# shz9/viprs

Hardware: AMD Instinct MI355X
Metric: SNP-updates/sec/E-step (1M SNPs, ~1700 LD blocks) (higher is better)
Workload: dtype f32

## Files before the change

### viprs_amd/csrc/abi_estep.hip

```cpp
#include "internal.h"

#include <type_traits>

using namespace viprs;

namespace {

__global__ void sweep_prologue_kernel(int32_t* counters, int n_counters, unsigned long long* skipped,
                                      unsigned long long* granules, int64_t n_granules) {
    const int64_t i = (int64_t)blockIdx.x * blockDim.x + threadIdx.x;
    if (i < n_counters) counters[i] = 0;
    if (i == 0) { skipped[0] = 0ull; skipped[1] = 0ull; }
    for (int64_t k = i; k < n_granules; k += (int64_t)gridDim.x * blockDim.x) granules[k] = 0ull;
}

hipError_t clear_stale_skip_count(viprs_plan* P) {
    if (!P->skip_count_in_place) return hipSuccess;
    P->skip_count_in_place = false;
    return hipMemsetAsync(P->d_skipped.p, 0, sizeof(unsigned long long), P->stream);
}

int sweep_prologue(viprs_plan* P, int n_models) {
    P->skip_count_in_place = true;
    const int64_t ng = P->n_granule_rows * kPanel * std::max(1, n_models);
    if (P->d_granules.n < (size_t)ng) {
        HIP_TRY(hipStreamSynchronize(P->stream));
        HIP_TRY(P->d_granules.alloc((size_t)ng));
    }
    const unsigned grid = (unsigned)std::max<int64_t>(1, std::min<int64_t>((ng + 255) / 256, 1024));
    sweep_prologue_kernel<<<grid, 256, 0, P->stream>>>(P->d_counters.p, kPlanCounters, P->d_skipped.p, P->d_granules.p, ng);
    HIP_TRY(hipGetLastError());
    return VIPRS_OK;
}

template <typename T>
EStepArgs<T> make_args(viprs_state* S, double dq) {
    viprs_plan* P = S->plan;
    EStepArgs<T> A{};
    A.skipped = P->d_skipped.p;
    A.lb = P->d_lb.p;
    A.rowstart = P->d_ip.p;
    A.rowlen = P->d_rowlen.p;
    A.ld_rows = P->d_ld_raw.p;
    A.ld_dense = P->d_ld_dense.p;
    A.ld_zero_off = P->dense_elems;
    A.std_beta = (const T*)S->f[VIPRS_FIELD_STD_BETA].p;
    A.u_logs = (const T*)S->f[VIPRS_FIELD_U_LOGS].p;
    A.shvt = (const T*)S->f[VIPRS_FIELD_SQRT_HALF_VAR_TAU].p;
    A.mu_mult = (const T*)S->f[VIPRS_FIELD_MU_MULT].p;
    A.log_null_pi = (const T*)S->f[VIPRS_FIELD_LOG_NULL_PI].p;
    A.var_gamma = (T*)S->f[VIPRS_FIELD_VAR_GAMMA].p;
    A.var_mu = (T*)S->f[VIPRS_FIELD_VAR_MU].p;
    A.eta = (T*)S->f[VIPRS_FIELD_ETA].p;
    A.q = (T*)S->f[VIPRS_FIELD_Q].p;
    A.eta_diff = (T*)S->f[VIPRS_FIELD_ETA_DIFF].p;
    A.eta_out = (T*)S->eta_out.p;
    A.q_out = (T*)S->q_out.p;
    A.granules = P->d_granules.p;
    A.granule_rows = P->n_granule_rows;
    A.error = P->d_error.p;
    A.dq = (T)dq;
    A.low_memory = P->low_memory;
    A.width = S->width;
    A.m = P->m;
    return A;
}

template <typename U> constexpr int ld_code();
template <> constexpr int ld_code<int8_t>() { return VIPRS_LD_I8; }
template <> constexpr int ld_code<int16_t>() { return VIPRS_LD_I16; }
template <> constexpr int ld_code<int32_t>() { return VIPRS_LD_I32; }
template <> constexpr int ld_code<int64_t>() { return VIPRS_LD_I64; }
template <> constexpr int ld_code<float>() { return VIPRS_LD_F32; }
template <> constexpr int ld_code<double>() { return VIPRS_LD_F64; }

template <typename... Us, typename F>
int for_ld_type(int ld_dtype, const char* otherwise, F&& f) {
    int rc = VIPRS_OK;
    const bool found = ((ld_dtype == ld_code<Us>() && ((rc = f(Us{})), true)) || ...);
    return found ? rc : fail(VIPRS_EINVAL, otherwise);
}

template <typename U>
int launch_grid_chunks(viprs_state* S, const EStepArgs<float>& A) {
    viprs_plan* P = S->plan;
    const int64_t lists_per_chunk = (int64_t)S->n_groups * kGroupListStride;
    for (int off = 0; off < A.n_active; off += kGridModels) {
        EStepArgs<float> Ac = A;
        Ac.active = A.active + off;
        Ac.n_active = std::min(kGridModels, A.n_active - off);
        if (A.group_cols) Ac.group_lists = S->d_group_lists.p + (off / kGridModels) * lists_per_chunk;
        int rc = off > 0 ? sweep_prologue(P, 1) : VIPRS_OK;
        if (rc == VIPRS_OK) rc = launch_grid_mfma<U>(P, Ac);
        if (rc != VIPRS_OK) return rc;
    }
    return VIPRS_OK;
}

template <typename T>
int launch_family(viprs_state* S, const EStepArgs<T>& A, int family, int model, bool dense) {
    viprs_plan* P = S->plan;
    if (family == kFamNone) return VIPRS_OK;
    if (family == kFamGeneric)
        return for_ld_type<int8_t, int16_t, int32_t, int64_t, float, double>(P->ld_dtype, "bad LD dtype", [&](auto u) {
            return launch_generic<T, decltype(u)>(P, A, model, dense); });
    if constexpr (std::is_same<T, double>::value) {
        if (family == kFamTileF64)
            return for_ld_type<int8_t, int16_t, int32_t, int64_t, float, double>(P->ld_dtype, "bad LD dtype", [&](auto u) {
                return launch_tile_f64<decltype(u)>(P, A, model, dense); });
    } else {
        if (family == kFamPanel)
            return for_ld_type<float, int8_t, int16_t>(P->ld_dtype, kDenseLdTypeError, [&](auto u) {
                return model == kPanelElasticNet ? launch_panel_enet<decltype(u)>(P, A) : launch_panel<decltype(u)>(P, A, model); });
        if (family == kFamBand)
            return for_ld_type<float, int8_t, int16_t>(P->ld_dtype, kBandLdTypeError, [&](auto u) {
                return model == kBandElasticNet ? launch_band_enet<decltype(u)>(P, A) : launch_band<decltype(u)>(P, A, model); });
        if (family == kFamGridBatched)
            return for_ld_type<float, int8_t, int16_t>(P->ld_dtype, kDenseLdTypeError, [&](auto u) {
                return launch_grid_chunks<decltype(u)>(S, A); });
    }
    return fail(VIPRS_EINVAL, "kernel family without an instantiation for the state precision");
}

template <typename T>
int launch_route(viprs_state* S, const SweepRoute& r, double dq, const int32_t* d_active, int n_active) {
    viprs_plan* P = S->plan;
    EStepArgs<T> A = make_args<T>(S, dq);
    A.active = d_active;
    A.n_active = n_active;
    if (S->model_kind == VIPRS_MODEL_GRID && !S->group_cols_h.empty()) {
        A.blk_group = S->d_blk_group.p;
        A.group_cols = S->d_group_cols.p;
    }
    int rc = launch_family<T>(S, A, r.dense_family, r.dense_model, true);
    if (rc != VIPRS_OK) return rc;
    rc = P->timing.dense_done();
    if (rc != VIPRS_OK) return rc;
    return launch_family<T>(S, A, r.ragged_family, r.ragged_model, false);
}

bool band_ok(const viprs_plan* P) {
    const char* f = getenv("VIPRS_BAND");
    if (f && !atoi(f)) return false;
    if (P->ld_dtype != VIPRS_LD_F32 && P->ld_dtype != VIPRS_LD_I8 && P->ld_dtype != VIPRS_LD_I16) return false;
    return band_ring_panels(P) <= kBandMaxRingPanels;
}

bool use_grid_mfma(const viprs_plan* P, int width) {
    if ((int64_t)P->m * std::max(1, width) >= (1LL << 31)) return false;
    if (P->grid_mfma >= 0) return P->grid_mfma != 0;
    return (int64_t)P->dense_h.size() * 8 >= (int64_t)P->n_cu * 3;
}

int run_route(viprs_state* S, const SweepRoute& r, double dq, const int32_t* d_active, int n_active) {
    viprs_plan* P = S->plan;
    int rc = VIPRS_OK;
    if (r.prologue) rc = sweep_prologue(P, r.prologue_per_model ? n_active : 1);
    else HIP_TRY(clear_stale_skip_count(P));
    if (rc != VIPRS_OK) return rc;
    P->math_used = 0;
    rc = P->timing.open(r.whole_sweep_events, r.dense_bracketed);
    if (rc != VIPRS_OK) return rc;
    if (r.dense_bracketed && r.start_event_by_launcher) P->timing.arm();
    else if (r.dense_bracketed) { rc = P->timing.start(); if (rc != VIPRS_OK) return rc; }
    rc = S->float_dtype == VIPRS_F32 ? launch_route<float>(S, r, dq, d_active, n_active)
                                     : launch_route<double>(S, r, dq, d_active, n_active);
    if (rc != VIPRS_OK) { P->timing.abandon(); return rc; }
    return P->timing.close();
}

int run_sweep(viprs_state* S, double dq, const int32_t* d_active, int n_active) {
    static_assert(kGenSpikeSlab == VIPRS_MODEL_SPIKE_SLAB && kGenMixture == VIPRS_MODEL_MIXTURE && kGenGrid == VIPRS_MODEL_GRID, "");
    viprs_plan* P = S->plan;
    HIP_TRY(hipSetDevice(P->device));
    const SweepConfig c{S->float_dtype, S->model_kind, S->width, P->ld_dtype, !P->dense_h.empty(), !P->ragged_h.empty(), band_ok(P),
                        use_grid_mfma(P, S->width), getenv("VIPRS_F64_ROW_BY_ROW") != nullptr};
    SweepRoute r;
    std::string err;
    const int rc = sweep_route(c, r, err);
    if (rc != VIPRS_OK) return fail(rc, err);
    return run_route(S, r, dq, d_active, n_active);
}

int group_mask_prepare(viprs_state* S, const int32_t* active, int n_active) {
    viprs_plan* P = S->plan;
    if (S->float_dtype != VIPRS_F32)
        return fail(VIPRS_EUNSUPPORTED, "grid state with a (group, column) mask: float64 states are not supported");
    if (!P->ragged_h.empty())
        return fail(VIPRS_EUNSUPPORTED, "grid state with a (group, column) mask: ragged / banded LD blocks are not supported "
                                        "(the generic and band kernels take no mask)");
    const int n_chunks = (n_active + kGridModels - 1) / kGridModels;
    std::vector<int32_t> lists((size_t)n_chunks * S->n_groups * kGroupListStride, 0);
    for (int k = 0; k < n_chunks; ++k) {
        const int lo = k * kGridModels, hi = std::min(n_active, lo + kGridModels);
        for (int g = 0; g < S->n_groups; ++g) {
            int32_t* l = lists.data() + ((size_t)k * S->n_groups + g) * kGroupListStride;
            int cnt = 0;
            for (int i = lo; i < hi; ++i)
                if (S->group_cols_h[(size_t)g * S->width + active[i]]) l[1 + cnt++] = active[i];
            l[0] = cnt;
            for (int t = cnt; t < kGridModels; ++t) l[1 + t] = cnt > 0 ? l[cnt] : active[lo];
        }
    }
    HIP_TRY(hipStreamSynchronize(P->stream));
    if (S->d_group_lists.n < lists.size()) HIP_TRY(S->d_group_lists.alloc(lists.size()));
    HIP_TRY(hipMemcpy(S->d_group_lists.p, lists.data(), lists.size() * sizeof(int32_t), hipMemcpyHostToDevice));
    if (S->blk_group_gen != P->dense_gen || S->d_blk_group.n < P->dense_h.size()) {
        std::vector<int32_t> map(std::max<size_t>(1, P->dense_h.size()), 0);
        for (size_t k = 0; k < P->dense_h.size(); ++k)
            map[k] = (int32_t)(std::upper_bound(S->group_start.begin(), S->group_start.end(), (int64_t)P->dense_h[k].start) -
                               S->group_start.begin()) - 1;
        HIP_TRY(S->d_blk_group.alloc(map.size()));
        HIP_TRY(hipMemcpy(S->d_blk_group.p, map.data(), map.size() * sizeof(int32_t), hipMemcpyHostToDevice));
        S->blk_group_gen = P->dense_gen;
    }
    return VIPRS_OK;
}

int active_list_check(const viprs_state* S, const int32_t*& active, int& n_active, std::vector<int32_t>& all) {
    if (!active) {
        all.resize((size_t)S->width);
        for (int g = 0; g < S->width; ++g) all[(size_t)g] = g;
        active = all.data();
        n_active = S->width;
    }
    for (int i = 0; i < n_active; ++i)
        if (active[i] < 0 || active[i] >= S->width) return fail(VIPRS_EINVAL, "active_model_idx out of range");
    return VIPRS_OK;
}

int active_list_upload(viprs_state* S, const int32_t* active, int n_active) {
    if (S->d_active.n < (size_t)n_active) HIP_TRY(S->d_active.alloc((size_t)std::max(n_active, S->width)));
    HIP_TRY(hipMemcpyAsync(S->d_active.p, active, sizeof(int32_t) * (size_t)n_active, hipMemcpyHostToDevice, S->plan->stream));
    HIP_TRY(hipStreamSynchronize(S->plan->stream));
    return VIPRS_OK;
}

void route_fields(const SweepRoute& r, int* route) {
    const int out[VIPRS_ROUTE_COUNT] = {r.dense_family, r.dense_model, r.ragged_family, r.ragged_model, r.prologue,
                                        r.prologue_per_model, r.start_event_by_launcher, r.whole_sweep_events, r.dense_bracketed};
    std::copy(out, out + VIPRS_ROUTE_COUNT, route);
}

}

extern "C" {

int viprs_state_e_step(viprs_state* S, double dq_scale, const int32_t* active, int n_active, int sync) {
    if (!S) return fail(VIPRS_EINVAL, "null state");
    int rc;
    switch (S->model_kind) {
        case VIPRS_MODEL_SPIKE_SLAB: case VIPRS_MODEL_MIXTURE: rc = run_sweep(S, dq_scale, nullptr, 0); break;
        case VIPRS_MODEL_GRID: {
            std::vector<int32_t> all;
            rc = active_list_check(S, active, n_active, all);
            if (rc != VIPRS_OK) return rc;
            if (n_active == 0) return VIPRS_OK;
            HIP_TRY(hipSetDevice(S->plan->device));
            if (!S->group_cols_h.empty()) {
                rc = group_mask_prepare(S, active, n_active);
                if (rc != VIPRS_OK) return rc;
            }
            rc = active_list_upload(S, active, n_active);
            if (rc != VIPRS_OK) return rc;
            rc = run_sweep(S, dq_scale, S->d_active.p, n_active);
            break;
        }
        default: return fail(VIPRS_EINVAL, "bad model kind");
    }
    if (rc != VIPRS_OK) return rc;
    if (sync) HIP_TRY(hipStreamSynchronize(S->plan->stream));
    return VIPRS_OK;
}

int viprs_state_enet_sweep(viprs_state* S, double dq_scale, const int32_t* active, int n_active, int sync) {
    if (!S) return fail(VIPRS_EINVAL, "null state");
    if (S->model_kind == VIPRS_MODEL_MIXTURE) return fail(VIPRS_EINVAL, "elastic-net sweep: not defined for a mixture state");
    if (S->model_kind != VIPRS_MODEL_SPIKE_SLAB && S->model_kind != VIPRS_MODEL_GRID) return fail(VIPRS_EINVAL, "bad model kind");
    if (S->float_dtype != VIPRS_F32)
        return fail(VIPRS_EUNSUPPORTED, "elastic-net sweep: float64 states are not supported (the kernels are float32)");
    const bool grid = S->model_kind == VIPRS_MODEL_GRID;
    if (grid && !S->group_cols_h.empty())
        return fail(VIPRS_EUNSUPPORTED, "elastic-net sweep: a grid state under a (group, column) mask is not supported");
    viprs_plan* P = S->plan;
    std::vector<int32_t> all;
    if (grid) {
        const int rc = active_list_check(S, active, n_active, all);
        if (rc != VIPRS_OK) return rc;
    } else {
        active = nullptr;
        n_active = 0;
    }
    SweepRoute r;
    std::string err;
    int rc = enet_route(grid, P->ld_dtype, !P->dense_h.empty(), !P->ragged_h.empty(), band_ok(P), r, err);
    if (rc != VIPRS_OK) return fail(rc, err);
    if (grid && n_active == 0) return VIPRS_OK;
    HIP_TRY(hipSetDevice(P->device));
    if (grid) {
        rc = active_list_upload(S, active, n_active);
        if (rc != VIPRS_OK) return rc;
    }
    rc = run_route(S, r, dq_scale, grid ? S->d_active.p : nullptr, n_active);
    if (rc != VIPRS_OK) return rc;
    if (sync) HIP_TRY(hipStreamSynchronize(P->stream));
    return VIPRS_OK;
}

int viprs_enet_route(int grid, int ld_dtype, int dense, int ragged, int band_ok, int* route) {
    if (!route) return fail(VIPRS_EINVAL, "null argument");
    SweepRoute r;
    std::string err;
    const int rc = enet_route(grid != 0, ld_dtype, dense != 0, ragged != 0, band_ok != 0, r, err);
    if (rc != VIPRS_OK) return fail(rc, err);
    route_fields(r, route);
    return VIPRS_OK;
}

static int one_shot(viprs_plan* P, int float_dtype, int model_kind, int width, const void* const (&host)[VIPRS_FIELD_COUNT],
                    double dq, const int32_t* active, int n_active) {
    viprs_state* S = P->scratch;
    if (!S || S->float_dtype != float_dtype || S->model_kind != model_kind || S->width != width) {
        delete P->scratch;
        P->scratch = nullptr;
        int rc = viprs_state_create(&P->scratch, P, float_dtype, model_kind, width);
        if (rc != VIPRS_OK) return rc;
        S = P->scratch;
    }
    const size_t fs = float_size(S->float_dtype);
    HIP_TRY(hipSetDevice(P->device));
    for (int f : {VIPRS_FIELD_STD_BETA, VIPRS_FIELD_LOG_NULL_PI, VIPRS_FIELD_U_LOGS, VIPRS_FIELD_SQRT_HALF_VAR_TAU, VIPRS_FIELD_MU_MULT,
                  VIPRS_FIELD_VAR_GAMMA, VIPRS_FIELD_VAR_MU, VIPRS_FIELD_ETA, VIPRS_FIELD_Q, VIPRS_FIELD_ETA_DIFF}) {
        const size_t bytes = S->field_elems(f) * fs;
        if (bytes == 0) continue;
        if (!host[f]) return fail(VIPRS_EINVAL, "null buffer");
        HIP_TRY(hipMemcpyAsync(S->f[f].p, host[f], bytes, hipMemcpyHostToDevice, P->stream));
    }
    int rc = viprs_state_e_step(S, dq, active, n_active, 0);
    if (rc != VIPRS_OK) return rc;
    for (int f : {VIPRS_FIELD_VAR_GAMMA, VIPRS_FIELD_VAR_MU, VIPRS_FIELD_ETA, VIPRS_FIELD_Q, VIPRS_FIELD_ETA_DIFF})
        HIP_TRY(hipMemcpyAsync(const_cast<void*>(host[f]), S->f[f].p, S->field_elems(f) * fs, hipMemcpyDeviceToHost, P->stream));
    HIP_TRY(hipStreamSynchronize(P->stream));
    return check_device_error(P);
}

int viprs_e_step(viprs_plan* P, int float_dtype, const void* std_beta, void* var_gamma, void* var_mu, void* eta,
                 void* q, void* eta_diff, const void* u_logs, const void* shvt, const void* mu_mult,
                 double dq_scale, int threads, int low_memory) {
    (void)threads;
    if (!P) return fail(VIPRS_EINVAL, "null plan");
    if ((low_memory != 0) != (P->low_memory != 0))
        return fail(VIPRS_EINVAL, "low_memory differs from the value the plan was created with");
    if (P->m == 0) return VIPRS_OK;
    const void* const host[] = {std_beta, u_logs, shvt, mu_mult, nullptr, var_gamma, var_mu, eta, q, eta_diff};
    return one_shot(P, float_dtype, VIPRS_MODEL_SPIKE_SLAB, 1, host, dq_scale, nullptr, 0);
}

int viprs_e_step_mixture(viprs_plan* P, int float_dtype, int K, const void* std_beta, void* var_gamma, void* var_mu,
                         void* eta, void* q, void* eta_diff, const void* log_null_pi, const void* u_logs,
                         const void* shvt, const void* mu_mult, double dq_scale, int threads, int low_memory) {
// ... 86 lines not shown
```

### viprs_amd/csrc/abi_plan.hip

```cpp
#include "internal.h"
#include <chrono>

using namespace viprs;

namespace {
thread_local std::string g_err;
viprs::BuildFlagsRegistrar tu_build_flags_(VIPRS_TU_BUILD_FLAGS);
}

namespace viprs {
int fail(int code, const std::string& msg) {
    g_err = msg;
    return code;
}
SchedConfig& sched_config() {
    static SchedConfig c;
    return c;
}
static std::string& build_flags_registry() {
    static std::string s;
    return s;
}
void register_build_flags(const char* flags) {
    std::string& all = build_flags_registry();
    const std::string f(flags ? flags : "");
    size_t i = 0;
    while (i < f.size()) {
        while (i < f.size() && f[i] == ' ') ++i;
        size_t j = i;
        while (j < f.size() && f[j] != ' ') ++j;
        if (j > i) {
            const std::string name = f.substr(i, j - i);
            if ((" " + all + " ").find(" " + name + " ") == std::string::npos) all += (all.empty() ? "" : " ") + name;
        }
        i = j;
    }
}
}

namespace {

template <typename U>
__global__ void repack_dense_kernel(const U* __restrict__ src, const int64_t* __restrict__ ip, U* __restrict__ dst,
                                    const BlockDesc* __restrict__ blocks, int upper) {
    const BlockDesc bd = blocks[blockIdx.y];
    const int b = bd.size;
    for (int r = blockIdx.x; r < b; r += gridDim.x) {
        const int64_t rs = ip[bd.start + r];
        U* __restrict__ drow = dst + bd.ld_off + (int64_t)r * bd.stride;
        if (upper) {
            for (int c = r + 1 + threadIdx.x; c < b; c += blockDim.x) drow[c] = src[rs + (c - r - 1)];
        } else {
            for (int c = threadIdx.x; c < b; c += blockDim.x) drow[c] = src[rs + c];
        }
    }
}

template <typename U>
__global__ __launch_bounds__(256) void mirror_lower_kernel(U* __restrict__ dense, const BlockDesc* __restrict__ blocks, int fill) {
    __shared__ U t[kPanel][kPanel + 1];
    const BlockDesc bd = blocks[blockIdx.y];
    const int b = bd.size, np = (b + kPanel - 1) / kPanel;
    U* __restrict__ base = dense + bd.ld_off;
    const int tx = threadIdx.x & 63, ty = threadIdx.x >> 6;
    const int n_pairs = np * (np + 1) / 2;
    for (int item = blockIdx.x; item < n_pairs; item += gridDim.x) {
        int I = 0, rem = item;
        while (rem >= np - I) { rem -= np - I; ++I; }
        const int J = I + rem;
        if (fill) {
            for (int r = ty; r < kPanel; r += 4) {
                const int row = I * kPanel + r, col = J * kPanel + tx;
                t[r][tx] = (row < b && col < b && col > row) ? base[(int64_t)row * bd.stride + col] : (U)0;
            }
        }
        __syncthreads();
        for (int r = ty; r < kPanel; r += 4) {
            const int row = J * kPanel + r, col = I * kPanel + tx;
            if (row < b && col < row) base[(int64_t)row * bd.stride + col] = fill ? t[tx][r] : (U)0;
        }
        __syncthreads();
    }
}

template <typename U>
__global__ void expand_symmetric_kernel(const U* __restrict__ up, const int64_t* __restrict__ ipu,
                                        const int32_t* __restrict__ lb, const int64_t* __restrict__ ip,
                                        U* __restrict__ out, int64_t m, U diag) {
    for (int64_t j = blockIdx.x; j < m; j += gridDim.x) {
        const int64_t o = ip[j];
        const int len = (int)(ip[j + 1] - o);
        const int64_t c0 = lb[j];
        const int64_t uj = ipu[j];
        for (int p = threadIdx.x; p < len; p += blockDim.x) {
            const int64_t c = c0 + p;
            U v = diag;
            if (c > j) v = up[uj + (c - j - 1)];
            else if (c < j) v = up[ipu[c] + (j - c - 1)];
            out[o + p] = v;
        }
    }
}

template <typename U>
static hipError_t launch_expand(const void* up, const int64_t* ipu, const int32_t* lb, const int64_t* ip, void* out,
                                int64_t m, double diag) {
    const unsigned grid = (unsigned)std::min<int64_t>(m, 1 << 16);
    expand_symmetric_kernel<U><<<grid, 256>>>((const U*)up, ipu, lb, ip, (U*)out, m, (U)diag);
    return hipGetLastError();
}

}

namespace viprs { void team_launch_forget(const viprs_plan* P); }
viprs_plan::~viprs_plan() {
    viprs::team_launch_forget(this);
    delete scratch;
    if (ev_fork) (void)hipEventDestroy(ev_fork);
    if (ev_join) (void)hipEventDestroy(ev_join);
    if (side_stream) (void)hipStreamDestroy(side_stream);
    if (stream) (void)hipStreamDestroy(stream);
}

struct ExpandSource {
    std::vector<int64_t> ip_upper;
    const void* data = nullptr;
    double diag = 1.0;
};

static int widen_indptr(int64_t m, const void* indptr, int indptr_dtype, std::vector<int64_t>& ip64) {
    ip64.assign((size_t)m + 1, 0);
    if (indptr_dtype == VIPRS_IP_I64) {
        if (m > 0) std::memcpy(ip64.data(), indptr, sizeof(int64_t) * ((size_t)m + 1));
    } else if (indptr_dtype == VIPRS_IP_I32) {
        const int32_t* p = static_cast<const int32_t*>(indptr);
        for (int64_t i = 0; i <= m && m > 0; ++i) ip64[(size_t)i] = p[i];
    } else {
        return fail(VIPRS_EINVAL, "bad indptr dtype code");
    }
    return VIPRS_OK;
}

static int plan_create_impl(viprs_plan** out, int64_t m, const int32_t* lb, const std::vector<int64_t>& ip64,
                            const void* ld_data, int ld_dtype, int low_memory, int device, const ExpandSource* ex,
                            const std::function<int(void*)>* fill = nullptr) {
    const size_t es = ld_elem_size(ld_dtype);
    std::unique_ptr<viprs_plan> P(new viprs_plan());
    P->m = m;
    if (const char* f = getenv("VIPRS_GRID_MFMA")) P->grid_mfma = atoi(f);
    {
        SchedConfig c;
        auto env = [](const char* name) -> const char* { const char* f = getenv(name); return (f && *f) ? f : nullptr; };
        if (const char* f = env("VIPRS_LARGE_BLOCK")) c.large_block = atoi(f);
        if (const char* f = env("VIPRS_MEDIUM_BLOCK")) c.medium_block = atoi(f);
        if (const char* f = env("VIPRS_TEAM0")) { c.class_team[0] = std::max(1, atoi(f)); c.team_env = true; }
        if (const char* f = env("VIPRS_TEAM1")) { c.class_team[1] = std::max(1, atoi(f)); c.team_env = true; }
        if (const char* f = getenv("VIPRS_BOTTOM_MOD")) c.bottom_mod = std::max(0, atoi(f));
        sched_config() = c;
    }
    P->low_memory = low_memory != 0;
    P->ld_dtype = ld_dtype;
    P->device = device;
    std::string err;
    int rc = plan_blocks(m, lb, ip64.data(), low_memory != 0, P->blocks, err);
    if (rc != VIPRS_OK) return fail(rc, err);
    P->nnz = m > 0 ? ip64[(size_t)m] : 0;
    if (P->nnz > 0 && !ld_data && !ex && !fill) return fail(VIPRS_EINVAL, "ld_data is null");

    HIP_TRY(hipSetDevice(device));
    (void)hipGetLastError();
    hipDeviceProp_t prop;
    HIP_TRY(hipGetDeviceProperties(&prop, device));
    P->n_cu = prop.multiProcessorCount;
    HIP_TRY(hipStreamCreateWithFlags(&P->stream, hipStreamNonBlocking));
    rc = P->timing.create(P->stream);
    if (rc != VIPRS_OK) return rc;

    bool panel_ld = (ld_dtype == VIPRS_LD_F32 || ld_dtype == VIPRS_LD_I8 || ld_dtype == VIPRS_LD_I16);
    if (const char* f = getenv("VIPRS_NO_DENSE")) panel_ld = panel_ld && !atoi(f);
    int64_t dense_off = 0;
    for (const Block& b : P->blocks) {
        BlockDesc d;
        d.start = (int32_t)b.start;
        d.size = (int32_t)(b.end - b.start);
        d.kind = b.kind;
        d.stride = 0;
        d.ld_off = 0;
        d.gr_off = 0;
        d.band_left = d.band_right = 0;
        constexpr int kMaxDenseBlock = 13184;
        static_assert(kMaxDenseBlock % kPanel == 0, "whole panels");
        static_assert(PanelLds(kMaxDenseBlock + 2 * kStrip, true, false).total_floats() <= 160 * 1024 / 4, "the symmetric form fits one workgroup");
        const bool dense = panel_ld && (b.kind == VIPRS_BLOCK_DENSE_SYM || b.kind == VIPRS_BLOCK_DENSE_UPPER) &&
                           d.size <= kMaxDenseBlock;
        if (dense) {
            d.stride = (d.size + kPanel - 1) / kPanel * kPanel;
            d.ld_off = dense_off;
            dense_off += (int64_t)d.size * d.stride;
            dense_off = (dense_off + 63) / 64 * 64;
            P->dense_h.push_back(d);
            P->max_dense = std::max(P->max_dense, d.size);
        } else {
            int64_t wl = 0, wr = 0;
            for (int64_t j = b.start; j < b.end; ++j) {
                const int64_t len = ip64[(size_t)j + 1] - ip64[(size_t)j];
                if (len <= 0) continue;
                wl = std::max<int64_t>(wl, j - lb[j]);
                wr = std::max<int64_t>(wr, lb[j] + len - 1 - j);
            }
            d.band_left = (int32_t)(wl / kPanel + 1);
            d.band_right = (int32_t)(wr / kPanel + 1);
            P->max_band_panels = std::max(P->max_band_panels, d.band_left + d.band_right + 2);
            P->ragged_h.push_back(d);
            P->max_ragged = std::max(P->max_ragged, d.size);
        }
    }
    P->dense_elems = dense_off;
    auto by_cost = [](const BlockDesc& a, const BlockDesc& b) {
        return a.size != b.size ? a.size > b.size : a.start < b.start;
    };
    std::sort(P->dense_h.begin(), P->dense_h.end(), by_cost);
    std::sort(P->ragged_h.begin(), P->ragged_h.end(), by_cost);
    {
        int i = 0, n = (int)P->dense_h.size();
        P->class_begin[0] = 0;
        while (i < n && P->dense_h[i].size >= sched_config().large_block) ++i;
        P->class_begin[1] = i;
        while (i < n && P->dense_h[i].size >= sched_config().medium_block) ++i;
        P->class_begin[2] = i;
        P->class_begin[3] = n;
        if (!sched_config().team_env && P->class_begin[1] > 0) {
            P->team0 = std::min(16, std::max(8, 4 * (int)(((int64_t)P->dense_h[0].size * (int64_t)es + 5999) / 6000)));
            const int64_t room = (int64_t)P->n_cu * 2 * 5 / 8;
            while (P->team0 > 4 && (int64_t)P->class_begin[1] * P->team0 > room) P->team0 -= 4;
        }
        int64_t rows = 0;
        for (int k = 0; k < P->class_begin[2]; ++k) {
            P->dense_h[(size_t)k].gr_off = rows;
            rows += (P->dense_h[(size_t)k].size + kPanel - 1) / kPanel;
        }
        P->n_granule_rows = rows;
    }

    HIP_TRY(P->d_counters.alloc(kPlanCounters));
    HIP_TRY(hipMemset(P->d_counters.p, 0, kPlanCounters * sizeof(int32_t)));
    HIP_TRY(hipDeviceSynchronize());
    HIP_TRY(P->d_error.alloc(1));
    HIP_TRY(hipMemset(P->d_error.p, 0, sizeof(int32_t)));
    HIP_TRY(P->d_skipped.alloc(2));
    HIP_TRY(hipMemset(P->d_skipped.p, 0, 2 * sizeof(unsigned long long)));
    if (m > 0) {
        HIP_TRY(P->d_lb.alloc((size_t)m));
        HIP_TRY(P->d_ip.alloc((size_t)m + 1));
        HIP_TRY(hipMemcpy(P->d_lb.p, lb, sizeof(int32_t) * (size_t)m, hipMemcpyHostToDevice));
        HIP_TRY(hipMemcpy(P->d_ip.p, ip64.data(), sizeof(int64_t) * ((size_t)m + 1), hipMemcpyHostToDevice));
        std::vector<int32_t> rowlen((size_t)m);
        for (int64_t j = 0; j < m; ++j) rowlen[(size_t)j] = (int32_t)(ip64[(size_t)j + 1] - ip64[(size_t)j]);
        HIP_TRY(P->d_rowlen.alloc((size_t)m));
        HIP_TRY(hipMemcpy(P->d_rowlen.p, rowlen.data(), sizeof(int32_t) * (size_t)m, hipMemcpyHostToDevice));
        if (!P->dense_h.empty()) {
            std::vector<int64_t> rs((size_t)m, 0);
            for (const BlockDesc& d : P->dense_h)
                for (int r = 0; r < d.size; ++r)
                    rs[(size_t)d.start + r] = d.ld_off + (int64_t)r * d.stride + (P->low_memory ? r + 1 : 0);
            HIP_TRY(P->d_rowstart_dense.alloc((size_t)m));
            HIP_TRY(hipMemcpy(P->d_rowstart_dense.p, rs.data(), sizeof(int64_t) * (size_t)m, hipMemcpyHostToDevice));
        }
    }
    if (P->nnz > 0) {
        HIP_TRY(P->d_ld_raw.alloc((size_t)P->nnz * es + 64));
        if (fill) {
            rc = (*fill)(P->d_ld_raw.p);
            if (rc != VIPRS_OK) return rc;
        } else if (!ex) {
            HIP_TRY(hipMemcpy(P->d_ld_raw.p, ld_data, (size_t)P->nnz * es, hipMemcpyHostToDevice));
        } else {
            const size_t nnz_u = (size_t)ex->ip_upper[(size_t)m];
            DevBuf<char> d_up;
            DevBuf<int64_t> d_ipu;
            HIP_TRY(d_up.alloc(std::max<size_t>(nnz_u, 1) * es));
            HIP_TRY(d_ipu.alloc((size_t)m + 1));
            if (nnz_u) HIP_TRY(hipMemcpy(d_up.p, ex->data, nnz_u * es, hipMemcpyHostToDevice));
            HIP_TRY(hipMemcpy(d_ipu.p, ex->ip_upper.data(), sizeof(int64_t) * ((size_t)m + 1), hipMemcpyHostToDevice));
            hipError_t e = hipSuccess;
            switch (ld_dtype) {
                case VIPRS_LD_I8:  e = launch_expand<int8_t>(d_up.p, d_ipu.p, P->d_lb.p, P->d_ip.p, P->d_ld_raw.p, m, ex->diag); break;
                case VIPRS_LD_I16: e = launch_expand<int16_t>(d_up.p, d_ipu.p, P->d_lb.p, P->d_ip.p, P->d_ld_raw.p, m, ex->diag); break;
                case VIPRS_LD_I32: e = launch_expand<int32_t>(d_up.p, d_ipu.p, P->d_lb.p, P->d_ip.p, P->d_ld_raw.p, m, ex->diag); break;
                case VIPRS_LD_I64: e = launch_expand<int64_t>(d_up.p, d_ipu.p, P->d_lb.p, P->d_ip.p, P->d_ld_raw.p, m, ex->diag); break;
                case VIPRS_LD_F32: e = launch_expand<float>(d_up.p, d_ipu.p, P->d_lb.p, P->d_ip.p, P->d_ld_raw.p, m, ex->diag); break;
                default:           e = launch_expand<double>(d_up.p, d_ipu.p, P->d_lb.p, P->d_ip.p, P->d_ld_raw.p, m, ex->diag); break;
            }
            HIP_TRY(e);
            HIP_TRY(hipDeviceSynchronize());
        }
    }
    if (P->n_granule_rows > 0) {
        HIP_TRY(P->d_granules.alloc((size_t)P->n_granule_rows * kPanel));
        HIP_TRY(hipMemset(P->d_granules.p, 0, sizeof(unsigned long long) * P->d_granules.n));
        HIP_TRY(hipDeviceSynchronize());
    }
    if (!P->dense_h.empty()) {
        HIP_TRY(P->d_dense.alloc(P->dense_h.size()));
        HIP_TRY(hipMemcpy(P->d_dense.p, P->dense_h.data(), sizeof(BlockDesc) * P->dense_h.size(), hipMemcpyHostToDevice));
        int max_stride = 0;
        for (const BlockDesc& d : P->dense_h) max_stride = std::max(max_stride, d.stride);
        const size_t bytes = ((size_t)P->dense_elems + 4 * kStrip + (size_t)kPanel * max_stride) * es;
        HIP_TRY(P->d_ld_dense.alloc(bytes));
        HIP_TRY(hipMemset(P->d_ld_dense.p, 0, bytes));
        dim3 grid(64, (unsigned)P->dense_h.size());
        const int upper = P->low_memory;
        switch (ld_dtype) {
            case VIPRS_LD_F32:
                repack_dense_kernel<float><<<grid, 256>>>((const float*)P->d_ld_raw.p, P->d_ip.p, (float*)P->d_ld_dense.p, P->d_dense.p, upper);
                break;
            case VIPRS_LD_I8:
                repack_dense_kernel<int8_t><<<grid, 256>>>((const int8_t*)P->d_ld_raw.p, P->d_ip.p, (int8_t*)P->d_ld_dense.p, P->d_dense.p, upper);
                break;
            case VIPRS_LD_I16:
                repack_dense_kernel<int16_t><<<grid, 256>>>((const int16_t*)P->d_ld_raw.p, P->d_ip.p, (int16_t*)P->d_ld_dense.p, P->d_dense.p, upper);
                break;
            default: break;
        }
        HIP_TRY(hipGetLastError());
        HIP_TRY(hipDeviceSynchronize());
    }
    if (!P->ragged_h.empty()) {
        HIP_TRY(P->d_ragged.alloc(P->ragged_h.size()));
        HIP_TRY(hipMemcpy(P->d_ragged.p, P->ragged_h.data(), sizeof(BlockDesc) * P->ragged_h.size(), hipMemcpyHostToDevice));
    } else {
        HIP_TRY(P->d_ld_raw.alloc(0));
    }
    P->dense_all_h = P->dense_h;
    P->ragged_all_h = P->ragged_h;
    std::copy(P->class_begin, P->class_begin + 4, P->class_begin_all);
    if (!P->dense_h.empty()) {
        HIP_TRY(P->d_dense_all.alloc(P->dense_h.size()));
        HIP_TRY(hipMemcpy(P->d_dense_all.p, P->dense_h.data(), sizeof(BlockDesc) * P->dense_h.size(), hipMemcpyHostToDevice));
    }
    HIP_TRY(hipDeviceSynchronize());
    *out = P.release();
    return VIPRS_OK;
}

namespace viprs {
int ensure_upper_storage(viprs_plan* P, bool mirrored) {
    P->unmirrored_wanted = !mirrored;
    if (!P->low_memory || P->dense_all_h.empty() || (P->mirror != 0) == mirrored) return VIPRS_OK;
    int max_np = 0;
    for (const BlockDesc& d : P->dense_all_h) max_np = std::max(max_np, (d.size + kPanel - 1) / kPanel);
    const dim3 grid((unsigned)std::min(max_np * (max_np + 1) / 2, 512), (unsigned)P->dense_all_h.size());
    switch (P->ld_dtype) {
        case VIPRS_LD_F32: mirror_lower_kernel<float><<<grid, 256, 0, P->stream>>>((float*)P->d_ld_dense.p, P->d_dense_all.p, mirrored ? 1 : 0); break;
        case VIPRS_LD_I8: mirror_lower_kernel<int8_t><<<grid, 256, 0, P->stream>>>((int8_t*)P->d_ld_dense.p, P->d_dense_all.p, mirrored ? 1 : 0); break;
        case VIPRS_LD_I16: mirror_lower_kernel<int16_t><<<grid, 256, 0, P->stream>>>((int16_t*)P->d_ld_dense.p, P->d_dense_all.p, mirrored ? 1 : 0); break;
        default: return fail(VIPRS_EINVAL, "dense blocks with unsupported LD dtype");
    }
    HIP_TRY(hipGetLastError());
    P->mirror = mirrored ? 1 : 0;
    return VIPRS_OK;
}

namespace {
std::mutex g_gate_mutex;
std::map<int, hipEvent_t> g_gate_event;
std::map<int, const viprs_plan*> g_gate_plan;
}
double host_clock_ms() {
    return std::chrono::duration<double, std::milli>(std::chrono::steady_clock::now().time_since_epoch()).count();
}
int team_launch_gate(viprs_plan* P) {
    std::lock_guard<std::mutex> lock(g_gate_mutex);
    auto it = g_gate_event.find(P->device);
    auto last = g_gate_plan.find(P->device);
    if (it != g_gate_event.end() && (last == g_gate_plan.end() || last->second != P))
        HIP_TRY(hipStreamWaitEvent(P->stream, it->second, 0));
    return VIPRS_OK;
}
void team_launch_forget(const viprs_plan* P) {
    std::lock_guard<std::mutex> lock(g_gate_mutex);
    auto last = g_gate_plan.find(P->device);
    if (last != g_gate_plan.end() && last->second == P) g_gate_plan.erase(last);
}
int team_launch_done(viprs_plan* P) {
    std::lock_guard<std::mutex> lock(g_gate_mutex);
    auto it = g_gate_event.find(P->device);
    if (it == g_gate_event.end()) {
        hipEvent_t e = nullptr;
        HIP_TRY(hipEventCreateWithFlags(&e, hipEventDisableTiming));
        it = g_gate_event.emplace(P->device, e).first;
    }
    HIP_TRY(hipEventRecord(it->second, P->stream));
    g_gate_plan[P->device] = P;
    return VIPRS_OK;
}
int plan_create_generated(viprs_plan** out, int64_t m, const int32_t* lb, const std::vector<int64_t>& ip64, int ld_dtype,
                          int low_memory, int device, const std::function<int(void*)>& fill) {
    return plan_create_impl(out, m, lb, ip64, nullptr, ld_dtype, low_memory, device, nullptr, &fill);
}
}

extern "C" {

const char* viprs_last_error(void) { return g_err.c_str(); }
const char* viprs_version(void) { return "viprs_amd 0.1.0 (gfx950)"; }
const char* viprs_build_flags(void) { return build_flags_registry().c_str(); }

int viprs_device_count(int* count) {
    if (!count) return fail(VIPRS_EINVAL, "count is null");
    int n = 0;
    hipError_t e = hipGetDeviceCount(&n);
    if (e != hipSuccess) { *count = 0; return fail(VIPRS_EDEVICE, hipGetErrorString(e)); }
    *count = n;
    return VIPRS_OK;
}

int viprs_host_fingerprint(const void* data, int64_t n_bytes, uint64_t* out) {
    if (!out || n_bytes < 0 || (n_bytes > 0 && !data)) return fail(VIPRS_EINVAL, "bad argument");
    const unsigned char* b = static_cast<const unsigned char*>(data);
    uint64_t h = 0x9e3779b97f4a7c15ull ^ (uint64_t)n_bytes;
    auto mix = [&](const unsigned char* p, int64_t n) {
        int64_t i = 0;
        for (; i + 8 <= n; i += 8) {
            uint64_t w;
            std::memcpy(&w, p + i, 8);
            h = (h ^ w) * 0xff51afd7ed558ccdull;
            h ^= h >> 32;
        }
        for (; i < n; ++i) { h = (h ^ p[i]) * 0x100000001b3ull; }
    };
    constexpr int64_t kEdge = 4096, kSamples = 256, kWin = 64;
    if (n_bytes <= 2 * kEdge + kSamples * kWin) {
        mix(b, n_bytes);
    } else {
        mix(b, kEdge);
        mix(b + n_bytes - kEdge, kEdge);
        const int64_t step = (n_bytes - kWin) / kSamples;
        for (int64_t k = 0; k < kSamples; ++k) mix(b + k * step, kWin);
    }
    *out = h;
    return VIPRS_OK;
}

int viprs_check_blas_support(void) { return 0; }
int viprs_check_omp_support(void) { return 0; }

int viprs_plan_blocks(int64_t m, const int32_t* lb, const void* indptr, int indptr_dtype, int low_memory,
                      int64_t* n_blocks, int64_t* block_start, int32_t* block_kind) {
    if (!n_blocks || !block_start) return fail(VIPRS_EINVAL, "null output");
    if (m > 0 && (!lb || !indptr)) return fail(VIPRS_EINVAL, "null LD index array");
    std::vector<int64_t> ip64;
    const int64_t* ip = nullptr;
    if (indptr_dtype == VIPRS_IP_I64) {
        ip = static_cast<const int64_t*>(indptr);
    } else if (indptr_dtype == VIPRS_IP_I32) {
        const int32_t* p = static_cast<const int32_t*>(indptr);
        ip64.assign(p, p + m + 1);
        ip = ip64.data();
    } else {
        return fail(VIPRS_EINVAL, "bad indptr dtype code");
    }
    std::vector<Block> blocks;
    std::string err;
    int rc = plan_blocks(m, lb, ip, low_memory != 0, blocks, err);
    if (rc != VIPRS_OK) return fail(rc, err);
    *n_blocks = (int64_t)blocks.size();
    for (size_t i = 0; i < blocks.size(); ++i) {
        block_start[i] = blocks[i].start;
        if (block_kind) block_kind[i] = blocks[i].kind;
    }
    block_start[blocks.size()] = m;
    return VIPRS_OK;
}

int viprs_plan_create(viprs_plan** out, int64_t m, const int32_t* lb, const void* indptr, int indptr_dtype,
                      const void* ld_data, int ld_dtype, int low_memory, int device) {
    if (!out) return fail(VIPRS_EINVAL, "plan output is null");
    *out = nullptr;
    if (ld_elem_size(ld_dtype) == 0) return fail(VIPRS_EINVAL, "bad LD dtype code");
    if (m < 0 || m > INT32_MAX) return fail(VIPRS_EINVAL, "m out of range");
    if (m > 0 && (!lb || !indptr)) return fail(VIPRS_EINVAL, "null LD index array");
    std::vector<int64_t> ip64;
    int rc = widen_indptr(m, indptr, indptr_dtype, ip64);
    if (rc != VIPRS_OK) return rc;
    return plan_create_impl(out, m, lb, ip64, ld_data, ld_dtype, low_memory, device, nullptr);
}

int viprs_plan_create_expanded(viprs_plan** out, int64_t m, const void* upper_indptr, int indptr_dtype,
                               const void* upper_data, int ld_dtype, double diag_value, int device) {
    if (!out) return fail(VIPRS_EINVAL, "plan output is null");
    *out = nullptr;
    if (ld_elem_size(ld_dtype) == 0) return fail(VIPRS_EINVAL, "bad LD dtype code");
    if (m < 0 || m > INT32_MAX) return fail(VIPRS_EINVAL, "m out of range");
    if (m > 0 && !upper_indptr) return fail(VIPRS_EINVAL, "null LD index array");
    ExpandSource ex;
    int rc = widen_indptr(m, upper_indptr, indptr_dtype, ex.ip_upper);
    if (rc != VIPRS_OK) return rc;
    ex.data = upper_data;
    ex.diag = diag_value;
    if (m > 0 && ex.ip_upper[(size_t)m] > 0 && !upper_data) return fail(VIPRS_EINVAL, "ld_data is null");
    std::vector<int32_t> lb((size_t)m, 0);
    std::vector<int64_t> ip((size_t)m + 1, 0);
    int64_t first = 0, prev_reach = -1;
    for (int64_t j = 0; j < m; ++j) {
        const int64_t len = ex.ip_upper[(size_t)j + 1] - ex.ip_upper[(size_t)j];
        if (len < 0) return fail(VIPRS_EINVAL, "ld_indptr is not non-decreasing");
        const int64_t reach = j + len;
        if (reach >= m) return fail(VIPRS_EINVAL, "an upper-triangular LD row runs past the last SNP");
        if (reach < prev_reach) return fail(VIPRS_EINVAL, "the upper-triangular windows do not mirror into contiguous symmetric windows");
        prev_reach = reach;
        while (first < j && first + (ex.ip_upper[(size_t)first + 1] - ex.ip_upper[(size_t)first]) < j) ++first;
        lb[(size_t)j] = (int32_t)first;
        ip[(size_t)j + 1] = ip[(size_t)j] + (j - first) + 1 + len;
    }
    return plan_create_impl(out, m, lb.data(), ip, nullptr, ld_dtype, 0, device, &ex);
}

int viprs_plan_get_windows(const viprs_plan* P, int32_t* left_bound, int64_t* indptr) {
    if (!P || !left_bound || !indptr) return fail(VIPRS_EINVAL, "null argument");
    HIP_TRY(hipSetDevice(P->device));
    indptr[0] = 0;
    if (P->m > 0) {
        HIP_TRY(hipMemcpy(left_bound, P->d_lb.p, sizeof(int32_t) * (size_t)P->m, hipMemcpyDeviceToHost));
        HIP_TRY(hipMemcpy(indptr, P->d_ip.p, sizeof(int64_t) * ((size_t)P->m + 1), hipMemcpyDeviceToHost));
    }
    return VIPRS_OK;
}
int viprs_plan_destroy(viprs_plan* plan) {
    if (!plan) return VIPRS_OK;
    (void)hipSetDevice(plan->device);
    delete plan;
    return VIPRS_OK;
}

int viprs_plan_info(const viprs_plan* P, int key, int64_t* value) {
// ... 82 lines not shown
```

### viprs_amd/csrc/abi_state.hip

```cpp
#include "internal.h"

using namespace viprs;

namespace {

template <typename T>
__global__ void reset_state_kernel(T* var_gamma, T* var_mu, int64_t n_wide, T* eta, T* q, T* eta_diff, int64_t n_vec,
                                   T pi) {
    const int64_t i = (int64_t)blockIdx.x * blockDim.x + threadIdx.x;
    if (i < n_wide) { var_gamma[i] = pi; var_mu[i] = (T)0; }
    if (i < n_vec) { eta[i] = (T)0; q[i] = (T)0; eta_diff[i] = (T)0; }
}


struct PrepRow {
    int64_t i0, i1, off;
    double logit_pi, log_tau_beta, sigma_eps, tau_beta, one_plus_lambda;
};

template <typename T, bool GRID>
__global__ void prep_kernel(const double* __restrict__ n, PrepRow one, const PrepRow* __restrict__ rows,
                            T* __restrict__ mu_mult, T* __restrict__ u_logs, T* __restrict__ shvt,
                            double* __restrict__ var_tau) {
    PrepRow r;
    if (rows) r = rows[blockIdx.y];
    else r = one;
    for (int64_t i = r.i0 + (int64_t)blockIdx.x * blockDim.x + threadIdx.x; i < r.i1; i += (int64_t)gridDim.x * blockDim.x) {
        const double vt = n[i] * r.one_plus_lambda / r.sigma_eps + r.tau_beta;
        mu_mult[r.off + i] = (T)(n[i] / (vt * r.sigma_eps));
        u_logs[r.off + i] = (T)(r.logit_pi + 0.5 * (r.log_tau_beta - log(vt)));
        if (GRID) {
            shvt[r.off + i] = (T)(0.5 * vt);
        } else {
            shvt[r.off + i] = (T)sqrt(0.5 * vt);
            var_tau[i] = vt;
        }
    }
}

constexpr int kMixResidentK = 8;
constexpr int kMixSums(int K) { return 7 + 6 * K; }
struct MixPrepRow {
    int64_t i0, i1;
    double log_null_pi, sigma_eps, one_plus_lambda;
    double logit_pi[kMixResidentK], log_tau[kMixResidentK], tau[kMixResidentK];
};

template <typename T>
__device__ __forceinline__ void prep_mixture_body(const double* __restrict__ n, int K, const MixPrepRow& r, T* __restrict__ mu_mult,
                                                  T* __restrict__ u_logs, T* __restrict__ shvt, T* __restrict__ lnp,
                                                  double* __restrict__ var_tau) {
    for (int64_t i = r.i0 + (int64_t)blockIdx.x * blockDim.x + threadIdx.x; i < r.i1; i += (int64_t)gridDim.x * blockDim.x) {
        lnp[i] = (T)r.log_null_pi;
        for (int k = 0; k < K; ++k) {
            const double vt = n[i] * r.one_plus_lambda / r.sigma_eps + r.tau[k];
            var_tau[i * K + k] = vt;
            mu_mult[i * K + k] = (T)(n[i] / (vt * r.sigma_eps));
            u_logs[i * K + k] = (T)(r.logit_pi[k] + 0.5 * (r.log_tau[k] - log(vt)));
            shvt[i * K + k] = (T)sqrt(0.5 * vt);
        }
    }
}
template <typename T>
__global__ void prep_mixture_kernel(const double* __restrict__ n, int K, MixPrepRow one, const MixPrepRow* __restrict__ rows,
                                    T* __restrict__ mu_mult, T* __restrict__ u_logs, T* __restrict__ shvt,
                                    T* __restrict__ lnp, double* __restrict__ var_tau) {
    if (rows) prep_mixture_body(n, K, rows[blockIdx.y], mu_mult, u_logs, shvt, lnp, var_tau);
    else prep_mixture_body(n, K, one, mu_mult, u_logs, shvt, lnp, var_tau);
}

constexpr int kSumsBlock = 256;
constexpr int kNSums = VIPRS_N_SUMS;
__host__ __device__ inline int sums_blocks(int64_t count) {
    const int64_t nb = (count + kSumsBlock - 1) / kSumsBlock;
    return (int)(nb < 1024 ? nb : 1024);
}
__host__ __device__ inline int grid_sums_blocks(int64_t count) {
    const int64_t nb = (count + kSumsBlock - 1) / kSumsBlock;
    return (int)(nb < 256 ? nb : 256);
}

struct SumsRow {
    int64_t i0, i1, off;
    int nb;
    int weighted;
    int form_vt;
    double vt[3];
    double one_plus_lambda;
};

template <typename T>
__device__ __forceinline__ void sums_body(int64_t i0, int64_t i1, int nb, int bx, const T* __restrict__ gam,
                                          const T* __restrict__ mu, const T* __restrict__ eta, const T* __restrict__ q,
                                          const T* __restrict__ ed, const T* __restrict__ beta,
                                          const double* __restrict__ var_tau, double one_plus_lambda,
                                          const double* __restrict__ weight, double* __restrict__ out,
                                          const double* __restrict__ n_snp = nullptr, double p_lam1 = 0.0, double p_sig = 1.0,
                                          double p_tau = 0.0) {
    __shared__ double red[kNSums][kSumsBlock];
    double acc[kNSums];
#pragma unroll
    for (int k = 0; k < kNSums; ++k) acc[k] = 0.0;
    const double lo = 1e-15, hi = 1.0 - 1e-15;
    for (int64_t i = i0 + (int64_t)bx * kSumsBlock + threadIdx.x; i < i1; i += (int64_t)nb * kSumsBlock) {
        const double g = (double)gam[i], mud = (double)mu[i];
        const double vt = n_snp ? n_snp[i] * p_lam1 / p_sig + p_tau : var_tau[i];
        const double zeta = g * (mud * mud + 1.0 / vt);
        acc[0] += weight ? g * weight[i] : g;
        acc[1] += zeta;
        acc[2] += one_plus_lambda * zeta + (double)(q[i] * eta[i]);
        acc[3] += (double)beta[i] * (double)eta[i];
        acc[4] += (double)eta[i] * (double)eta[i];
        const double gc = fmin(fmax(g, lo), hi), ng = fmin(fmax(1.0 - g, lo), hi);
        acc[5] += gc * log(gc);
        acc[6] += ng * log(ng);
        acc[7] += gc;
        acc[8] += ng;
        acc[9] += gc * log(vt);
        acc[10] = fmax(acc[10], fabs((double)ed[i]));
    }
#pragma unroll
    for (int k = 0; k < kNSums; ++k) red[k][threadIdx.x] = acc[k];
    __syncthreads();
    for (int s = kSumsBlock / 2; s > 0; s >>= 1) {
        if ((int)threadIdx.x < s) {
#pragma unroll
            for (int k = 0; k < kNSums - 1; ++k) red[k][threadIdx.x] += red[k][threadIdx.x + s];
            red[kNSums - 1][threadIdx.x] = fmax(red[kNSums - 1][threadIdx.x], red[kNSums - 1][threadIdx.x + s]);
        }
        __syncthreads();
    }
    if (threadIdx.x < kNSums) out[threadIdx.x] = red[threadIdx.x][0];
}

template <typename T>
__global__ __launch_bounds__(kSumsBlock) void sums_kernel(SumsRow one, const SumsRow* __restrict__ rows,
                                                          const T* __restrict__ gam, const T* __restrict__ mu,
                                                          const T* __restrict__ eta, const T* __restrict__ q,
                                                          const T* __restrict__ ed, const T* __restrict__ beta,
                                                          const double* __restrict__ var_tau, const double* __restrict__ n_snp,
                                                          const double* __restrict__ weight, double* __restrict__ partials) {
    SumsRow r;
    if (rows) r = rows[blockIdx.y];
    else r = one;
    if ((int)blockIdx.x >= r.nb) return;
    sums_body<T>(r.i0, r.i1, r.nb, (int)blockIdx.x, gam + r.off, mu + r.off, eta + r.off, q + r.off, ed + r.off, beta,
                 r.form_vt ? nullptr : var_tau, r.one_plus_lambda, r.weighted ? weight : nullptr,
                 partials + ((int64_t)blockIdx.y * gridDim.x + blockIdx.x) * kNSums, r.form_vt ? n_snp : nullptr, r.vt[0],
                 r.vt[1], r.vt[2]);
}

template <typename T>
__device__ __forceinline__ void sums_mixture_body(int64_t i0, int64_t i1, int nb, int bx, int K, const T* __restrict__ gam,
                                                  const T* __restrict__ mu, const T* __restrict__ eta,
                                                  const T* __restrict__ q, const T* __restrict__ ed,
                                                  const T* __restrict__ beta, const double* __restrict__ var_tau,
                                                  const double* __restrict__ log_var_tau0, double one_plus_lambda,
                                                  double* __restrict__ partials) {
    constexpr int NMAX = kMixSums(kMixResidentK);
    const int N = kMixSums(K);
    double acc[NMAX];
#pragma unroll
    for (int k = 0; k < NMAX; ++k) acc[k] = 0.0;
    const double lo = 1e-15, hi = 1.0 - 1e-15;
    for (int64_t i = i0 + (int64_t)bx * kSumsBlock + threadIdx.x; i < i1; i += (int64_t)nb * kSumsBlock) {
        double zeta = 0.0, gsum = 0.0;
#pragma unroll
        for (int k = 0; k < kMixResidentK; ++k) {
            if (k < K) {
                const double g = (double)gam[i * K + k], mud = (double)mu[i * K + k], vt = var_tau[i * K + k];
                const double z = g * (mud * mud + 1.0 / vt);
                zeta += z;
                gsum += g;
                const double gc = fmin(fmax(g, lo), hi);
                acc[6 + 0 * kMixResidentK + k] += g;
                acc[6 + 1 * kMixResidentK + k] += z;
                acc[6 + 2 * kMixResidentK + k] += gc * log(gc);
                acc[6 + 3 * kMixResidentK + k] += gc;
                acc[6 + 4 * kMixResidentK + k] += gc * log_var_tau0[i * K + k];
                acc[6 + 5 * kMixResidentK + k] += gc * (mud * mud + 1.0 / vt);
            }
        }
        acc[0] += zeta;
        acc[1] += one_plus_lambda * zeta + (double)(q[i] * eta[i]);
        acc[2] += (double)beta[i] * (double)eta[i];
        acc[3] += (double)eta[i] * (double)eta[i];
        const double ng = fmin(fmax(1.0 - gsum, lo), hi);
        acc[4] += ng * log(ng);
        acc[5] += ng;
        acc[NMAX - 1] = fmax(acc[NMAX - 1], fabs((double)ed[i]));
    }
    __shared__ double red[NMAX][kSumsBlock / 64];
    const int lane = threadIdx.x & 63, wave = threadIdx.x >> 6;
#pragma unroll
    for (int k = 0; k < NMAX; ++k) {
        double a = acc[k];
        for (int off = 32; off > 0; off >>= 1) {
            const double o = __shfl_xor(a, off, 64);
            a = (k == NMAX - 1) ? fmax(a, o) : a + o;
        }
        if (lane == 0) red[k][wave] = a;
    }
    __syncthreads();
    if ((int)threadIdx.x < N) {
        const int nidx = threadIdx.x;
        int src;
        if (nidx < 6) src = nidx;
        else if (nidx == N - 1) src = NMAX - 1;
        else src = 6 + ((nidx - 6) / K) * kMixResidentK + (nidx - 6) % K;
        double a = red[src][0];
        for (int w = 1; w < kSumsBlock / 64; ++w) a = (src == NMAX - 1) ? fmax(a, red[src][w]) : a + red[src][w];
        partials[nidx] = a;
    }
}

template <typename T>
__global__ __launch_bounds__(kSumsBlock) void sums_mixture_kernel(int K, SumsRow one, const SumsRow* __restrict__ rows,
                                                                  const T* __restrict__ gam, const T* __restrict__ mu,
                                                                  const T* __restrict__ eta, const T* __restrict__ q,
                                                                  const T* __restrict__ ed, const T* __restrict__ beta,
                                                                  const double* __restrict__ var_tau,
                                                                  const double* __restrict__ log_var_tau0,
                                                                  double* __restrict__ partials) {
    SumsRow r;
    if (rows) r = rows[blockIdx.y];
    else r = one;
    if ((int)blockIdx.x >= r.nb) return;
    sums_mixture_body<T>(r.i0, r.i1, r.nb, (int)blockIdx.x, K, gam, mu, eta, q, ed, beta, var_tau, log_var_tau0,
                         r.one_plus_lambda, partials + ((int64_t)blockIdx.y * gridDim.x + blockIdx.x) * kMixSums(K));
}

constexpr int kNEnetSums = VIPRS_N_ENET_SUMS;
__global__ __launch_bounds__(kSumsBlock) void enet_sums_kernel(SumsRow one, const SumsRow* __restrict__ rows,
                                                               const float* __restrict__ eta, const float* __restrict__ q,
                                                               const float* __restrict__ ed, const float* __restrict__ beta,
                                                               const float* __restrict__ pen, double* __restrict__ partials) {
    SumsRow r;
    if (rows) r = rows[blockIdx.y];
    else r = one;
    if ((int)blockIdx.x >= r.nb) return;
    __shared__ double red[kNEnetSums][kSumsBlock];
    double acc[kNEnetSums];
#pragma unroll
    for (int k = 0; k < kNEnetSums; ++k) acc[k] = 0.0;
    for (int64_t i = r.i0 + (int64_t)blockIdx.x * kSumsBlock + threadIdx.x; i < r.i1; i += (int64_t)r.nb * kSumsBlock) {
        const double e = (double)eta[r.off + i];
        acc[0] += (double)beta[i] * e;
        acc[1] += (double)q[r.off + i] * e;
        acc[2] += e * e;
        acc[3] += (double)pen[r.off + i] * fabs(e);
        acc[4] += e != 0.0 ? 1.0 : 0.0;
        acc[5] = fmax(acc[5], fabs((double)ed[r.off + i]));
    }
#pragma unroll
    for (int k = 0; k < kNEnetSums; ++k) red[k][threadIdx.x] = acc[k];
    __syncthreads();
    for (int s = kSumsBlock / 2; s > 0; s >>= 1) {
        if ((int)threadIdx.x < s) {
#pragma unroll
            for (int k = 0; k < kNEnetSums - 1; ++k) red[k][threadIdx.x] += red[k][threadIdx.x + s];
            red[kNEnetSums - 1][threadIdx.x] = fmax(red[kNEnetSums - 1][threadIdx.x], red[kNEnetSums - 1][threadIdx.x + s]);
        }
        __syncthreads();
    }
    if (threadIdx.x < kNEnetSums)
        partials[((int64_t)blockIdx.y * gridDim.x + blockIdx.x) * kNEnetSums + threadIdx.x] = red[threadIdx.x][0];
}

__global__ void sums_final_kernel(const double* __restrict__ partials, int stride, int n_sums, SumsRow one,
                                  const SumsRow* __restrict__ rows, double* __restrict__ out) {
    int nb;
    if (rows) nb = rows[blockIdx.y].nb;
    else nb = one.nb;
    partials += (int64_t)blockIdx.y * stride * n_sums;
    const int k = blockIdx.x, lane = threadIdx.x;
    const bool is_max = (k == n_sums - 1);
    double a = 0.0;
    for (int b = lane; b < nb; b += 64) {
        const double v = partials[(int64_t)b * n_sums + k];
        a = is_max ? fmax(a, v) : a + v;
    }
    for (int off = 32; off > 0; off >>= 1) {
        const double o = __shfl_xor(a, off, 64);
        a = is_max ? fmax(a, o) : a + o;
    }
    if (lane == 0) out[(int64_t)blockIdx.y * n_sums + k] = a;
}

}

extern "C" {

int viprs_state_create(viprs_state** out, viprs_plan* plan, int float_dtype, int model_kind, int width) {
    if (!out || !plan) return fail(VIPRS_EINVAL, "null argument");
    *out = nullptr;
    if (float_size(float_dtype) == 0) return fail(VIPRS_EINVAL, "bad float dtype code");
    if (model_kind < VIPRS_MODEL_SPIKE_SLAB || model_kind > VIPRS_MODEL_GRID) return fail(VIPRS_EINVAL, "bad model kind");
    if (model_kind == VIPRS_MODEL_SPIKE_SLAB) width = 1;
    if (width < 1) return fail(VIPRS_EINVAL, "width must be >= 1");
    HIP_TRY(hipSetDevice(plan->device));
    (void)hipGetLastError();
    std::unique_ptr<viprs_state> S(new viprs_state());
    S->plan = plan;
    S->device = plan->device;
    S->float_dtype = float_dtype;
    S->model_kind = model_kind;
    S->width = width;
    if (plan->n_granule_rows > 0) {
        HIP_TRY(S->eta_out.alloc(S->field_elems(VIPRS_FIELD_ETA) * float_size(float_dtype)));
        HIP_TRY(S->q_out.alloc(S->field_elems(VIPRS_FIELD_ETA) * float_size(float_dtype)));
    }
    for (int k = 0; k < VIPRS_FIELD_COUNT; ++k) {
        const size_t bytes = S->field_elems(k) * float_size(float_dtype);
        HIP_TRY(S->f[k].alloc(bytes));
        if (bytes) HIP_TRY(hipMemsetAsync(S->f[k].p, 0, bytes, plan->stream));
    }
    HIP_TRY(hipStreamSynchronize(plan->stream));
    *out = S.release();
    return VIPRS_OK;
}

int viprs_state_destroy(viprs_state* S) {
    if (!S) return VIPRS_OK;
    (void)hipSetDevice(S->device);
    delete S;
    return VIPRS_OK;
}

int viprs_state_upload(viprs_state* S, int field, const void* host) {
    if (!S || field < 0 || field >= VIPRS_FIELD_COUNT) return fail(VIPRS_EINVAL, "bad state/field");
    const size_t bytes = S->field_elems(field) * float_size(S->float_dtype);
    if (bytes == 0) return VIPRS_OK;
    if (!host) return fail(VIPRS_EINVAL, "host buffer is null");
    HIP_TRY(hipSetDevice(S->plan->device));
    HIP_TRY(hipMemcpyAsync(S->f[field].p, host, bytes, hipMemcpyHostToDevice, S->plan->stream));
    HIP_TRY(hipStreamSynchronize(S->plan->stream));
    return VIPRS_OK;
}

int viprs_state_download(viprs_state* S, int field, void* host) {
    if (!S || field < 0 || field >= VIPRS_FIELD_COUNT) return fail(VIPRS_EINVAL, "bad state/field");
    const size_t bytes = S->field_elems(field) * float_size(S->float_dtype);
    if (bytes == 0) return VIPRS_OK;
    if (!host) return fail(VIPRS_EINVAL, "host buffer is null");
    HIP_TRY(hipSetDevice(S->plan->device));
    HIP_TRY(hipMemcpyAsync(host, S->f[field].p, bytes, hipMemcpyDeviceToHost, S->plan->stream));
    HIP_TRY(hipStreamSynchronize(S->plan->stream));
    return check_device_error(S->plan);
}

int viprs_state_reset(viprs_state* S, double pi) {
    if (!S) return fail(VIPRS_EINVAL, "null state");
    viprs_plan* P = S->plan;
    HIP_TRY(hipSetDevice(P->device));
    const int64_t n_wide = (int64_t)S->field_elems(VIPRS_FIELD_VAR_GAMMA);
    const int64_t n_vec = (int64_t)S->field_elems(VIPRS_FIELD_ETA);
    const int64_t n = std::max(n_wide, n_vec);
    if (n == 0) return VIPRS_OK;
    const unsigned grid = (unsigned)((n + 255) / 256);
    if (S->float_dtype == VIPRS_F32)
        reset_state_kernel<float><<<grid, 256, 0, P->stream>>>(
            (float*)S->f[VIPRS_FIELD_VAR_GAMMA].p, (float*)S->f[VIPRS_FIELD_VAR_MU].p, n_wide,
            (float*)S->f[VIPRS_FIELD_ETA].p, (float*)S->f[VIPRS_FIELD_Q].p, (float*)S->f[VIPRS_FIELD_ETA_DIFF].p, n_vec,
            (float)pi);
    else
        reset_state_kernel<double><<<grid, 256, 0, P->stream>>>(
            (double*)S->f[VIPRS_FIELD_VAR_GAMMA].p, (double*)S->f[VIPRS_FIELD_VAR_MU].p, n_wide,
            (double*)S->f[VIPRS_FIELD_ETA].p, (double*)S->f[VIPRS_FIELD_Q].p, (double*)S->f[VIPRS_FIELD_ETA_DIFF].p, n_vec,
            pi);
    HIP_TRY(hipGetLastError());
    return VIPRS_OK;
}

}

namespace viprs {
int check_device_error(viprs_plan* P) {
    int32_t e = 0;
    HIP_TRY(hipMemcpy(&e, P->d_error.p, sizeof(e), hipMemcpyDeviceToHost));
    if (e != 0) {
        HIP_TRY(hipMemsetAsync(P->d_error.p, 0, sizeof(e), P->stream));
        HIP_TRY(hipStreamSynchronize(P->stream));
        return fail(VIPRS_EDEVICE, "E-step kernel: a team hand-off timed out (results of this sweep are invalid)");
    }
    return VIPRS_OK;
}
}

static size_t prep_row_bytes(const viprs_state* S) {
    return S->model_kind == VIPRS_MODEL_MIXTURE ? sizeof(MixPrepRow) : sizeof(PrepRow);
}
static SumsRow* sums_staging(const viprs_state* S) {
    return reinterpret_cast<SumsRow*>(S->h_rows + S->rows_cap * prep_row_bytes(S));
}

static int row_buffers(viprs_state* S, int n) {
    if ((size_t)n <= S->rows_cap) return VIPRS_OK;
    viprs_plan* P = S->plan;
    const size_t cap = std::max<size_t>((size_t)n, (size_t)std::max(1, S->n_groups) *
                                                       (S->model_kind == VIPRS_MODEL_GRID ? S->width : 1));
    HIP_TRY(hipStreamSynchronize(P->stream));
    HIP_TRY(S->d_prep_rows.alloc(cap * prep_row_bytes(S)));
    HIP_TRY(S->d_sum_rows.alloc(cap * sizeof(SumsRow)));
    if (S->h_rows) HIP_TRY(hipHostFree(S->h_rows));
    S->h_rows = nullptr;
    S->rows_cap = 0;
    HIP_TRY(hipHostMalloc(reinterpret_cast<void**>(&S->h_rows), cap * (prep_row_bytes(S) + sizeof(SumsRow)),
                          hipHostMallocDefault));
    S->rows_cap = cap;
    return VIPRS_OK;
}

template <typename Row>
static int prep_staging(viprs_state* S, int n, Row** h) {
    const int rc = row_buffers(S, n);
    if (rc != VIPRS_OK) return rc;
    if (!S->ev_prep) HIP_TRY(hipEventCreateWithFlags(&S->ev_prep, hipEventDisableTiming));
    else HIP_TRY(hipEventSynchronize(S->ev_prep));
    *h = reinterpret_cast<Row*>(S->h_rows);
    return VIPRS_OK;
}

template <typename Row>
static dim3 prep_grid(int n, const Row* rows) {
    int64_t longest = 0;
    for (int i = 0; i < n; ++i) longest = std::max(longest, rows[i].i1 - rows[i].i0);
    return dim3((unsigned)std::max<int64_t>(1, (longest + 255) / 256), (unsigned)n);
}

static int prep_launch(viprs_state* S, int n, const PrepRow* one) {
    viprs_plan* P = S->plan;
    const PrepRow* h = one ? one : reinterpret_cast<const PrepRow*>(S->h_rows);
    const PrepRow* rows = one ? nullptr : reinterpret_cast<const PrepRow*>(S->d_prep_rows.p);
    if (!one) HIP_TRY(hipMemcpyAsync(S->d_prep_rows.p, h, n * sizeof(PrepRow), hipMemcpyHostToDevice, P->stream));
    const dim3 grid = prep_grid(n, h);
    const bool g = S->model_kind == VIPRS_MODEL_GRID;
#define VIPRS_PREP_ARGS(T)                                                                                                    \
    S->d_n.p, *h, rows, (T*)S->f[VIPRS_FIELD_MU_MULT].p, (T*)S->f[VIPRS_FIELD_U_LOGS].p,                                     \
        (T*)S->f[VIPRS_FIELD_SQRT_HALF_VAR_TAU].p, S->d_var_tau.p
    if (S->float_dtype == VIPRS_F32 && g) prep_kernel<float, true><<<grid, 256, 0, P->stream>>>(VIPRS_PREP_ARGS(float));
    else if (S->float_dtype == VIPRS_F32) prep_kernel<float, false><<<grid, 256, 0, P->stream>>>(VIPRS_PREP_ARGS(float));
    else if (g) prep_kernel<double, true><<<grid, 256, 0, P->stream>>>(VIPRS_PREP_ARGS(double));
    else prep_kernel<double, false><<<grid, 256, 0, P->stream>>>(VIPRS_PREP_ARGS(double));
#undef VIPRS_PREP_ARGS
    HIP_TRY(hipGetLastError());
    if (!one) HIP_TRY(hipEventRecord(S->ev_prep, P->stream));
    return VIPRS_OK;
}

static int prep_mixture_launch(viprs_state* S, int n, const MixPrepRow* one) {
    viprs_plan* P = S->plan;
    const int K = S->width;
    if (S->d_var_tau.n < (size_t)P->m * K) {
        HIP_TRY(hipStreamSynchronize(P->stream));
        HIP_TRY(S->d_var_tau.alloc((size_t)P->m * K));
    }
    const MixPrepRow* h = one ? one : reinterpret_cast<const MixPrepRow*>(S->h_rows);
    const MixPrepRow* rows = one ? nullptr : reinterpret_cast<const MixPrepRow*>(S->d_prep_rows.p);
    if (!one) HIP_TRY(hipMemcpyAsync(S->d_prep_rows.p, h, n * sizeof(MixPrepRow), hipMemcpyHostToDevice, P->stream));
    const dim3 grid = prep_grid(n, h);
    if (S->float_dtype == VIPRS_F32)
        prep_mixture_kernel<float><<<grid, 256, 0, P->stream>>>(
            S->d_n.p, K, *h, rows, (float*)S->f[VIPRS_FIELD_MU_MULT].p, (float*)S->f[VIPRS_FIELD_U_LOGS].p,
            (float*)S->f[VIPRS_FIELD_SQRT_HALF_VAR_TAU].p, (float*)S->f[VIPRS_FIELD_LOG_NULL_PI].p, S->d_var_tau.p);
    else
        prep_mixture_kernel<double><<<grid, 256, 0, P->stream>>>(
            S->d_n.p, K, *h, rows, (double*)S->f[VIPRS_FIELD_MU_MULT].p, (double*)S->f[VIPRS_FIELD_U_LOGS].p,
            (double*)S->f[VIPRS_FIELD_SQRT_HALF_VAR_TAU].p, (double*)S->f[VIPRS_FIELD_LOG_NULL_PI].p, S->d_var_tau.p);
    HIP_TRY(hipGetLastError());
    if (!one) HIP_TRY(hipEventRecord(S->ev_prep, P->stream));
    return VIPRS_OK;
}

static SumsRow sums_row(const viprs_state* S, int64_t i0, int64_t i1, int64_t col, double one_plus_lambda, bool weighted,
                        const double* vt) {
    SumsRow r{};
    r.i0 = i0;
    r.i1 = i1;
    r.off = col * S->plan->m;
    r.nb = vt ? grid_sums_blocks(i1 - i0) : sums_blocks(i1 - i0);
    r.weighted = weighted;
    r.one_plus_lambda = one_plus_lambda;
    if (vt) {
        r.form_vt = 1;
        for (int k = 0; k < 3; ++k) r.vt[k] = vt[k];
    }
    return r;
}

static int sums_buffers(viprs_state* S, size_t partials, size_t total) {
    if (S->d_partials.n < partials) HIP_TRY(S->d_partials.alloc(partials));
    if (S->d_sums.n < total) HIP_TRY(S->d_sums.alloc(total));
    if (S->h_sums_cap < total + 1) {
        if (S->h_sums) HIP_TRY(hipHostFree(S->h_sums));
        S->h_sums = nullptr;
        S->h_sums_cap = 0;
        HIP_TRY(hipHostMalloc(reinterpret_cast<void**>(&S->h_sums), (total + 1) * sizeof(double), hipHostMallocDefault));
        S->h_sums_cap = total + 1;
    }
    return VIPRS_OK;
}

enum { kSumsSpikeSlabOrGrid = 0, kSumsMixture = 1, kSumsElasticNet = 2 };

static int sums_enqueue(viprs_state* S, int family, int n, int n_sums, const SumsRow* one) {
    const bool mixture = family == kSumsMixture;
    viprs_plan* P = S->plan;
    HIP_TRY(hipSetDevice(P->device));
    const size_t total = (size_t)n * n_sums;
    const SumsRow* h = one ? one : sums_staging(S);
    int nb = 1;
    for (int i = 0; P->m > 0 && i < n; ++i) nb = std::max(nb, h[i].nb);
    int rc = sums_buffers(S, (size_t)nb * total, total);
    if (rc != VIPRS_OK) return rc;
    if (P->m == 0) {
        HIP_TRY(hipMemsetAsync(S->d_sums.p, 0, total * sizeof(double), P->stream));
    } else {
        const SumsRow* rows = one ? nullptr : reinterpret_cast<const SumsRow*>(S->d_sum_rows.p);
        if (!one) HIP_TRY(hipMemcpyAsync(S->d_sum_rows.p, h, n * sizeof(SumsRow), hipMemcpyHostToDevice, P->stream));
        const dim3 grid((unsigned)nb, (unsigned)n);
#define VIPRS_SUMS_ARGS(T)                                                                                                     \
    *h, rows, (const T*)S->f[VIPRS_FIELD_VAR_GAMMA].p, (const T*)S->f[VIPRS_FIELD_VAR_MU].p, (const T*)S->f[VIPRS_FIELD_ETA].p, \
        (const T*)S->f[VIPRS_FIELD_Q].p, (const T*)S->f[VIPRS_FIELD_ETA_DIFF].p, (const T*)S->f[VIPRS_FIELD_STD_BETA].p,       \
        S->d_var_tau.p
        if (family == kSumsElasticNet)
            enet_sums_kernel<<<grid, kSumsBlock, 0, P->stream>>>(
                *h, rows, (const float*)S->f[VIPRS_FIELD_ETA].p, (const float*)S->f[VIPRS_FIELD_Q].p,
                (const float*)S->f[VIPRS_FIELD_ETA_DIFF].p, (const float*)S->f[VIPRS_FIELD_STD_BETA].p,
                (const float*)S->f[VIPRS_FIELD_ENET_PENALTY].p, S->d_partials.p);
        else if (mixture && S->float_dtype == VIPRS_F32)
            sums_mixture_kernel<float><<<grid, kSumsBlock, 0, P->stream>>>(S->width, VIPRS_SUMS_ARGS(float), S->d_log_var_tau0.p,
                                                                           S->d_partials.p);
        else if (mixture)
            sums_mixture_kernel<double><<<grid, kSumsBlock, 0, P->stream>>>(S->width, VIPRS_SUMS_ARGS(double),
                                                                            S->d_log_var_tau0.p, S->d_partials.p);
        else if (S->float_dtype == VIPRS_F32)
            sums_kernel<float><<<grid, kSumsBlock, 0, P->stream>>>(VIPRS_SUMS_ARGS(float), S->d_n.p, S->d_weight.p,
                                                                   S->d_partials.p);
        else
            sums_kernel<double><<<grid, kSumsBlock, 0, P->stream>>>(VIPRS_SUMS_ARGS(double), S->d_n.p, S->d_weight.p,
                                                                    S->d_partials.p);
#undef VIPRS_SUMS_ARGS
        HIP_TRY(hipGetLastError());
        sums_final_kernel<<<dim3((unsigned)n_sums, (unsigned)n), 64, 0, P->stream>>>(S->d_partials.p, nb, n_sums, *h, rows,
                                                                                     S->d_sums.p);
        HIP_TRY(hipGetLastError());
    }
    if (S->comm) {
        rc = comm_reduce_on_stream(S->comm, S->d_sums.p, (int)total, n_sums, P->stream);
        if (rc != VIPRS_OK) return rc;
    }
    HIP_TRY(hipMemcpyAsync(S->h_sums, S->d_sums.p, total * sizeof(double), hipMemcpyDeviceToHost, P->stream));
    HIP_TRY(hipMemcpyAsync(S->h_sums + total, P->d_error.p, sizeof(int32_t), hipMemcpyDeviceToHost, P->stream));
    S->sums_total = total;
    S->sums_pending = true;
    S->sums_empty = false;
    return VIPRS_OK;
}

static int sums_nothing(viprs_state* S, bool mixture, int n, int n_sums) {
    if (S->plan->m == 0 && n > 0 && S->comm) return sums_enqueue(S, mixture, n, n_sums, nullptr);
    S->sums_total = (size_t)n * n_sums;
    S->sums_pending = false;
    S->sums_empty = true;
    return VIPRS_OK;
}

static int sums_collect(viprs_state* S, double* out, const char* begin, size_t room = SIZE_MAX) {
    const size_t n = std::min(S->sums_total, room);
    if (S->sums_empty) {
        for (size_t k = 0; k < n; ++k) out[k] = 0.0;
        return VIPRS_OK;
    }
    if (!S->sums_pending) return fail(VIPRS_EINVAL, std::string("no device sums in flight (") + begin + ")");
    viprs_plan* P = S->plan;
    HIP_TRY(hipSetDevice(P->device));
    HIP_TRY(hipStreamSynchronize(P->stream));
    S->sums_pending = false;
    for (size_t k = 0; k < n; ++k) out[k] = S->h_sums[k];
    int32_t e = 0;
    memcpy(&e, S->h_sums + S->sums_total, sizeof(e));
    return e != 0 ? check_device_error(P) : VIPRS_OK;
}

extern "C" {

int viprs_state_synchronize(viprs_state* S) {
    if (!S) return fail(VIPRS_EINVAL, "null state");
    HIP_TRY(hipSetDevice(S->plan->device));
    HIP_TRY(hipStreamSynchronize(S->plan->stream));
    return check_device_error(S->plan);
}

int viprs_state_set_n_per_snp(viprs_state* S, const double* n) {
    if (!S || !n) return fail(VIPRS_EINVAL, "null argument");
    viprs_plan* P = S->plan;
    HIP_TRY(hipSetDevice(P->device));
    const size_t m = (size_t)P->m;
    if (m == 0) return VIPRS_OK;
    HIP_TRY(S->d_n.alloc(m));
    HIP_TRY(S->d_var_tau.alloc(m));
    HIP_TRY(hipMemcpyAsync(S->d_n.p, n, m * sizeof(double), hipMemcpyHostToDevice, P->stream));
    HIP_TRY(hipMemsetAsync(S->d_var_tau.p, 0, m * sizeof(double), P->stream));
    HIP_TRY(hipStreamSynchronize(P->stream));
    return VIPRS_OK;
}

int viprs_state_set_snp_weights(viprs_state* S, const double* w) {
    if (!S) return fail(VIPRS_EINVAL, "null argument");
    viprs_plan* P = S->plan;
    HIP_TRY(hipSetDevice(P->device));
    const size_t m = (size_t)P->m;
    if (!w || m == 0) { HIP_TRY(S->d_weight.alloc(0)); return VIPRS_OK; }
    HIP_TRY(S->d_weight.alloc(m));
// ... 562 lines not shown
```

### viprs_amd/csrc/estep_band.h

```cpp
#pragma once
#include "panel_loads.h"
#include "panel_models.h"

namespace viprs {

constexpr int kBandWaves = 8;
constexpr int kBandStagers = 2;
constexpr int kBandIdleWave = 4;
constexpr int kBandUpdaters = kBandWaves - 2 - kBandStagers;
constexpr int kBandTargets = 2;

__host__ __device__ constexpr int band_lds_floats(int ring_panels) {
    return ring_panels * kPanel + 2 * kPanel + 4 * kPanel * kPanel;
}

struct BandRows {
    int rs_lo, rs_hi, lb, len;
};
__device__ __forceinline__ BandRows band_rows(const EStepArgs<float>& A, int64_t s0, int b, int panel, int lane) {
    const int row = panel * kPanel + lane;
    const bool ok = row < b;
    const int64_t rs = ok ? A.rowstart[s0 + row] : 0;
    BandRows d;
    d.rs_lo = (int)(unsigned)(rs & 0xffffffffll);
    d.rs_hi = (int)(rs >> 32);
    d.lb = ok ? A.lb[s0 + row] - (int)s0 : 0;
    d.len = ok ? A.rowlen[s0 + row] : 0;
    return d;
}
__device__ __forceinline__ int64_t band_rowstart(const BandRows& d, int r) {
    return ((int64_t)__builtin_amdgcn_readlane(d.rs_hi, r) << 32) | (int64_t)(unsigned)__builtin_amdgcn_readlane(d.rs_lo, r);
}

template <typename U>
__device__ __forceinline__ void band_stage_tiles(const U* __restrict__ ld, const BandRows& dT, const BandRows& dD, int cp,
                                                 float* __restrict__ dstT, float* __restrict__ dstD, int sw, int lane) {
    constexpr int RPW = (2 * kPanel + kBandStagers - 1) / kBandStagers;
    const int c = cp * kPanel + lane;
    float v[RPW];
    unsigned long long okm = 0;
#pragma unroll
    for (int i = 0; i < RPW; ++i) {
        const int t = min(sw + i * kBandStagers, 2 * kPanel - 1);
        const bool inT = t < kPanel;
        const int r = t & (kPanel - 1);
        const int len = inT ? __builtin_amdgcn_readlane(dT.len, r) : __builtin_amdgcn_readlane(dD.len, r);
        const int off = c - (inT ? __builtin_amdgcn_readlane(dT.lb, r) : __builtin_amdgcn_readlane(dD.lb, r));
        const int64_t rs = inT ? band_rowstart(dT, r) : band_rowstart(dD, r);
        v[i] = static_cast<float>(ld[rs + max(0, min(off, len - 1))]);
        okm |= (off >= 0 && off < len) ? (1ull << i) : 0ull;
    }
    asm volatile("" ::: "memory");
#pragma unroll
    for (int i = 0; i < RPW; ++i) {
        const int t = sw + i * kBandStagers;
        if (t < 2 * kPanel) {
            float* __restrict__ dst = (t < kPanel) ? dstT : dstD;
            dst[(t & (kPanel - 1)) * kPanel + lane] = ((okm >> i) & 1ull) ? v[i] : 0.0f;
        }
    }
}

template <typename U, int NT>
__device__ __forceinline__ void band_strip(const U* __restrict__ ld, const BandRows& d, const int (&c)[NT], float avec,
                                           float (&qv)[NT]) {
    constexpr int DEPTH = 64 / NT;
#pragma unroll
    for (int g = 0; g < kPanel / DEPTH; ++g) {
        float x[NT][DEPTH];
        unsigned okm[NT];
#pragma unroll
        for (int n = 0; n < NT; ++n) okm[n] = 0;
#pragma unroll
        for (int k = 0; k < DEPTH; ++k) {
            const int r = g * DEPTH + k;
            const int len = __builtin_amdgcn_readlane(d.len, r);
            const int lb = __builtin_amdgcn_readlane(d.lb, r);
            const U* __restrict__ row = ld + band_rowstart(d, r);
#pragma unroll
            for (int n = 0; n < NT; ++n) {
                const int off = c[n] - lb;
                x[n][k] = static_cast<float>(row[max(0, min(off, len - 1))]);
                okm[n] |= (off >= 0 && off < len) ? (1u << k) : 0u;
            }
        }
        asm volatile("" ::: "memory");
#pragma unroll
        for (int k = 0; k < DEPTH; ++k) {
            const float a = rl(avec, g * DEPTH + k);
#pragma unroll
            for (int n = 0; n < NT; ++n) qv[n] = __builtin_fmaf(((okm[n] >> k) & 1u) ? x[n][k] : 0.0f, a, qv[n]);
        }
    }
}

template <bool EXACT = true>
struct MixtureSerialModel : MixtureModel<EXACT> {
    static constexpr bool kLaneParallel = false;
};

template <typename U, typename MODEL, bool SYM>
__global__ __launch_bounds__(64 * kBandWaves) void estep_band_kernel(EStepArgs<float> A0, int ring_panels) {
    static_assert(!MODEL::kLaneParallel, "band kernel: lane-per-SNP model policies only");
    extern __shared__ __attribute__((aligned(16))) float band_smem[];
    __shared__ int s_blk;
    ExpTab tab;
    tab.init();
    const int tid = threadIdx.x, lane = tid & 63;
    const int wave = __builtin_amdgcn_readfirstlane(tid >> 6);
    const int RM = ring_panels - 1;
    float* __restrict__ lq = band_smem;
    float* __restrict__ la = lq + ring_panels * kPanel;
    float* __restrict__ lT = la + 2 * kPanel;
    float* __restrict__ lD = lT + 2 * kPanel * kPanel;
    const U* __restrict__ ld = static_cast<const U*>(A0.ld_rows);
    const int n_models = max(A0.n_active, 1);
    const float dq = A0.dq;
    unsigned long long my_skipped = 0;

    for (;;) {
        if (tid == 0) s_blk = atomicAdd(A0.counter, 1);
        __syncthreads();
        const int item = s_blk;
        __syncthreads();
        if (item >= A0.n_blocks * n_models) break;
        const int blk = item / n_models, model_slot = item - blk * n_models;
        const EStepArgs<float> A = select_model(A0, model_slot);
        const BlockDesc bd = A.blocks[blk];
        const int64_t s0 = bd.start;
        const int b = bd.size;
        const int WL = bd.band_left, WR = bd.band_right;
        const int np = (b + kPanel - 1) / kPanel;

        for (int i = tid; i < min(WR, np) * kPanel; i += 64 * kBandWaves)
            lq[((i >> 6) & RM) * kPanel + (i & 63)] = (i < b) ? A.q[s0 + i] : 0.0f;
        BandRows d_prev{}, d_cur{}, d_next{};
        if (wave > 0) {
            d_cur = band_rows(A, s0, b, 0, lane);
            d_next = band_rows(A, s0, b, 1, lane);
            if (wave <= kBandStagers) band_stage_tiles<U>(ld, d_cur, d_cur, 0, lT, lD, wave - 1, lane);
        }
        __syncthreads();

        float a_prev = 0.0f;
        typename MODEL::In nxt_in{};
        if (wave == 0) nxt_in = MODEL::load(A, s0 + (lane < b ? lane : 0), lane < b);

        for (int p = 0; p < np + (SYM ? 1 : 0); ++p) {
            if (wave == 0) {
                if (p < np) {
                    const int r0 = p * kPanel;
                    const int nrows = min(kPanel, b - r0);
                    const int64_t j = s0 + r0 + lane;
                    const bool live = lane < nrows;
                    const typename MODEL::In in = nxt_in;
                    {
                        const int rn = r0 + kPanel + lane;
                        const bool ln = rn < b;
                        nxt_in = MODEL::load(A, s0 + (ln ? rn : 0), ln);
                    }
                    float* __restrict__ slot = lq + (p & RM) * kPanel + lane;
                    float qc = *slot;
                    const float* __restrict__ Dt = lD + (p & 1) * kPanel * kPanel + lane;
                    float drow[kPanel];
#pragma unroll
                    for (int k = 0; k < kChainPrefetch; ++k) drow[k] = Dt[k * kPanel];
                    if (p > 0) {
                        const float* __restrict__ T = lT + (p & 1) * kPanel * kPanel;
#pragma unroll
                        for (int k = 0; k < kPanel; ++k) qc = __builtin_fmaf(T[k * kPanel + lane], rl(a_prev, k), qc);
                    }
                    float qcap_v = 0.0f;
#pragma unroll
                    for (int jj = 0; jj < kPanel; ++jj) {
                        if (jj + kChainPrefetch < kPanel) drow[jj + kChainPrefetch] = Dt[(jj + kChainPrefetch) * kPanel];
                        float d;
                        const bool upd = MODEL::template update<kLookupLane>(in, qc, tab, d, jj) && live;
                        const float a_lane = upd ? dq * d : 0.0f;
                        int l = lane;
                        asm volatile("" : "+v"(l));
                        const bool me = (l == jj);
                        qcap_v = me ? qc : qcap_v;
                        qc = __builtin_fmaf(drow[jj], rl(a_lane, jj), qc);
                        if (SYM) qc = (me && upd) ? qc - d : qc;
                    }
                    bool skipped_lane;
                    a_prev = MODEL::template finish<false>(A, j, in, qcap_v, tab, live, true, skipped_lane);
                    my_skipped += __popcll(__ballot(skipped_lane));
                    la[(p & 1) * kPanel + lane] = a_prev;
                    *slot = qc;
                    if (!SYM && live) A.q[j] = qc;
                }
            } else {
                const BandRows d_fetch = band_rows(A, s0, b, p + 2, lane);
                if (wave <= kBandStagers) {
                    if (p + 1 < np)
                        band_stage_tiles<U>(ld, d_cur, d_next, p + 1, lT + ((p + 1) & 1) * kPanel * kPanel,
                                            lD + ((p + 1) & 1) * kPanel * kPanel, wave - 1, lane);
                } else if (p > 0) {
                    const int uw = (wave == kBandIdleWave) ? kBandUpdaters : wave - 1 - kBandStagers - (wave > kBandIdleWave ? 1 : 0);
                    const int pp = p - 1;
                    const float avec = la[(pp & 1) * kPanel + lane];
                    const bool any_a = __ballot(avec != 0.0f) != 0;
                    const int first = SYM ? max(0, pp - WL) : p + 1;
                    const int last = min(np - 1, pp + WR);
                    const int n_targets = last - first + 1 - ((SYM && p < np) ? 2 : (SYM ? 1 : 0));
                    const int n_upd = (n_targets > kBandUpdaters * kBandTargets) ? kBandUpdaters + 1 : kBandUpdaters;
                    for (int t0 = uw * kBandTargets; t0 < n_targets && uw < n_upd; t0 += n_upd * kBandTargets) {
                        int cp[kBandTargets], c[kBandTargets];
                        float qv[kBandTargets];
#pragma unroll
                        for (int n = 0; n < kBandTargets; ++n) {
                            int x = first + t0 + n;
                            if (SYM && x >= pp) x += 2;
                            cp[n] = (t0 + n < n_targets) ? x : -1;
                            c[n] = (cp[n] >= 0) ? cp[n] * kPanel + lane : -(1 << 28);
                            qv[n] = (cp[n] >= 0) ? lq[(cp[n] & RM) * kPanel + lane] : 0.0f;
                        }
                        if (any_a) band_strip<U, kBandTargets>(ld, d_prev, c, avec, qv);
#pragma unroll
                        for (int n = 0; n < kBandTargets; ++n) {
                            if (cp[n] < 0) continue;
                            lq[(cp[n] & RM) * kPanel + lane] = qv[n];
                            if (SYM && p == min(cp[n] + WL + 1, np) && c[n] < b) A.q[s0 + c[n]] = qv[n];
                        }
                    }
                    if (SYM && p == np && uw == 0 && pp * kPanel + lane < b)
                        A.q[s0 + pp * kPanel + lane] = lq[(pp & RM) * kPanel + lane];
                }
                d_prev = d_cur;
                d_cur = d_next;
                d_next = d_fetch;
                if (wave == 1) {
                    const int cn = p + WR;
                    if (cn < np) {
                        const int c = cn * kPanel + lane;
                        lq[(cn & RM) * kPanel + lane] = (c < b) ? A.q[s0 + c] : 0.0f;
                    }
                }
            }
            __syncthreads();
        }

    }
    if (lane == 0 && my_skipped) atomicAdd(A0.skipped, my_skipped);
}

template <typename U>
__global__ __launch_bounds__(256) void band_upper_epilogue_kernel(EStepArgs<float> A0) {
    const int n_models = max(A0.n_active, 1);
    const int blk = blockIdx.y / n_models, model_slot = blockIdx.y - blk * n_models;
    const EStepArgs<float> A = select_model(A0, model_slot);
    const BlockDesc bd = A.blocks[blk];
    const U* __restrict__ ld = static_cast<const U*>(A.ld_rows);
    for (int jj = blockIdx.x * 256 + threadIdx.x; jj < bd.size; jj += gridDim.x * 256) {
        const int64_t j = (int64_t)bd.start + jj;
        const U* __restrict__ row = ld + A.rowstart[j];
        const float* __restrict__ ed = A.eta_diff + A.lb[j];
        const int len = A.rowlen[j];
        float s = 0.0f;
        for (int i = 0; i < len; ++i) s = __builtin_fmaf(static_cast<float>(row[i]), ed[i], s);
        A.q[j] += A.dq * s;
    }
}

}
```

### viprs_amd/csrc/estep_panel.h

```cpp
#pragma once
#include <type_traits>

#include "device_math.h"
#include "kernels_common.h"
#include "panel_loads.h"
#include "panel_models.h"

#ifndef PANEL_MIN_WAVES
#define PANEL_MIN_WAVES 2
#endif

namespace viprs {

#ifdef VIPRS_SWEEP_TRACE
__device__ unsigned long long g_sweep_trace[1 << 15][4];
__device__ unsigned int g_sweep_trace_n;
#endif

#ifdef VIPRS_PANEL_PROFILE
#define PPROF(slot, cond) do { if (TEAM && item == 0 && member < 2 && lane == 0 && p < 64 && (cond)) s_pprof[p][slot] = (unsigned)wall_clock64(); } while (0)
#else
#define PPROF(slot, cond) do { } while (0)
#endif

template <typename U> __host__ __device__ constexpr int panel_cols() { return sizeof(U) == 4 ? 4 : 8; }
template <typename U> __host__ __device__ constexpr int panel_team_cols() {
#ifdef PANEL_TEAM_CPL_F32
    return sizeof(U) == 4 ? PANEL_TEAM_CPL_F32 : 4;
#else
    return sizeof(U) == 4 ? 2 : 4;
#endif
}

constexpr int kFormSym = 1, kFormMirror = 2;

template <typename U, typename MODEL, int FORM, int NW, bool TEAM, int CPL>
__device__ __forceinline__ void panel_role(const EStepArgs<float>& A0, const int qcap, float* __restrict__ smem, const int wg) {
    constexpr bool MIR = FORM == kFormMirror;
    constexpr bool SUMS = FORM != kFormSym;
    const PanelLds lds(qcap, MODEL::kLaneParallel && !is_wide_mixture<MODEL>::value, MIR);
    float* lq = smem + lds.q();
    float* la = smem + lds.a();
    float* lT = smem + lds.diag_tiles();
    float* lTo = smem + lds.offdiag_tile();
    float* lmx = smem + lds.mix();
    float* led = smem + lds.ed();
    float* ls = smem + lds.s();
#ifdef PANEL_TEAM_STRIP_DEPTH
    constexpr int kDepth = TEAM ? PANEL_TEAM_STRIP_DEPTH : kStripRowsInFlight;
#else
    constexpr int kDepth = TEAM ? (kPanel / RawRow<U, CPL>::kWords < kPanel ? kPanel / RawRow<U, CPL>::kWords : kPanel) : kStripRowsInFlight;
#endif
    __shared__ int s_blk;
    __shared__ int s_tdone;
    __shared__ int s_ddone;

    const int tid = threadIdx.x;
    const int wave = __builtin_amdgcn_readfirstlane(tid >> 6);
    const int lane = tid & 63;
    const U* __restrict__ ldd = static_cast<const U*>(A0.ld_dense);
    ExpTab tab;
    tab.init();
    unsigned long long my_skipped = 0;
    const float dq = A0.dq;
    const int n_models = max(1, A0.n_active);

    constexpr int kSW = kPanel * CPL;
    const int TS = TEAM ? A0.team_size : 1;
    const int team = TEAM ? wg / TS : 0;
    const int member = TEAM ? wg % TS : 0;
    int team_iter = 0;

    for (;;) {
        int item;
        if (TEAM) {
            item = team + team_iter * A0.n_teams;
            ++team_iter;
        } else {
            if (tid == 0) {
                int it = atomicAdd(A0.counter, 1);
                if (A0.bottom_mod > 0 && it < A0.n_blocks * n_models) {
                    const bool bottom = (wg % A0.bottom_mod) == A0.bottom_mod - 1;
                    it = bottom ? A0.n_blocks * n_models - 1 - atomicAdd(A0.counter + 2, 1) : atomicAdd(A0.counter + 1, 1);
                }
                s_blk = it;
            }
            __syncthreads();
            item = s_blk;
            __syncthreads();
        }
        if (item >= A0.n_blocks * n_models) break;
        const int blk = item / n_models, model_slot = item - blk * n_models;
        if constexpr (IsGridColumn<MODEL>::value) {
            if (A0.group_cols) {
                const int on = A0.group_cols[(int64_t)A0.blk_group[blk] * A0.width + A0.active[model_slot]];
                if (__builtin_amdgcn_readfirstlane(on) == 0) continue;
            }
        }
        const EStepArgs<float> A = select_model(A0, model_slot);

        const BlockDesc bd = A.blocks[blk];
        const int64_t s0 = bd.start;
        const int b = bd.size;
#ifdef VIPRS_SWEEP_TRACE
        const unsigned long long trace_t0 = wall_clock64();
#endif
        unsigned long long* __restrict__ gran =
            TEAM ? A.granules + ((int64_t)model_slot * A.granule_rows + bd.gr_off) * kPanel : nullptr;
        const int stride = bd.stride;
        const U* __restrict__ base = ldd + bd.ld_off;
        const int np = (b + kPanel - 1) / kPanel;
        const int bpad = np * kPanel;
        const int nstrips_all = (bpad + kSW - 1) / kSW;
        const int n_own = TEAM ? (nstrips_all - member + TS - 1) / TS : nstrips_all;
        auto own = [&](int c) { return !TEAM || ((c / kSW) % TS) == member; };
        auto loc = [&](int c) { return TEAM ? ((c / kSW) / TS) * kSW + (c % kSW) : c; };
        auto glob = [&](int li) { return TEAM ? ((li / kSW) * TS + member) * kSW + (li % kSW) : li; };

        for (int li = tid; li < (TEAM ? n_own * kSW : bpad) + kStrip; li += NW * 64) {
            const int c = glob(li);
            const bool in = (!TEAM || li < n_own * kSW) && c < b;
            lq[li] = in ? A.q[s0 + c] : 0.0f;
            if (SUMS) ls[li] = 0.0f;
        }
        if (tid == 0) { s_tdone = 0; s_ddone = 0; }
        for (int i = tid; i < kPanel * kPanel / 4; i += NW * 64) {
            const int row = i >> 4, tcol = (i & 15) * 4;
            *reinterpret_cast<float4*>(lT + row * kPanel + tcol) = load4<U>(base + (int64_t)min(row, b - 1) * stride + tcol);
        }
        __syncthreads();

        float a_prev = 0.0f;

        typename MODEL::In nxt_in{};
        if (wave == 0) {
            const bool live0 = lane < b;
            nxt_in = MODEL::load(A, s0 + (live0 ? lane : 0), live0);
        }

#ifdef VIPRS_PANEL_PROFILE
        __shared__ unsigned s_pprof[64][8];
#endif
        if (wave == 0) {
#ifdef PANEL_CHAIN_PRIO
        __builtin_amdgcn_s_setprio(PANEL_CHAIN_PRIO);
#endif
        for (int p = 0; p < np + 1; ++p) {
            PPROF(0, true);
            {
                if (p < np) {
                    const int r0 = p * kPanel;
                    const int nrows = min(kPanel, b - r0);
                    const int64_t j = s0 + r0 + lane;
                    const bool live = lane < nrows;
                    const typename MODEL::In in = nxt_in;
                    {
                        const int rn = r0 + kPanel + lane;
                        const bool ln = rn < b;
                        nxt_in = MODEL::load(A, s0 + (ln ? rn : 0), ln);
                    }

                    float qc;
                    float q_own = 0.0f;
                    if (own(r0)) qc = lq[loc(r0 + lane)];
                    else qc = (r0 + lane < b) ? A.q[s0 + r0 + lane] : 0.0f;
                    if (TEAM && p >= 2 && (((p * kPanel) / kSW) % TS) != member) {
                        unsigned long long g = 0;
#ifdef PANEL_TIMING_NO_HANDOFF_WAIT
                        if (false)
#endif
                        for (unsigned spins = 0;; ++spins) {
                            g = __hip_atomic_load(gran + (int64_t)p * kPanel + lane, __ATOMIC_RELAXED,
                                                  __HIP_MEMORY_SCOPE_AGENT);
                            if (__all((unsigned)(g >> 32) == A.tag_base + (unsigned)(p + 1))) break;
                            if (spins > (1u << 22)) {
                                if (lane == 0) atomicExch(A.error, 1);
                                break;
                            }
                            if ((spins & 1023u) == 1023u &&
                                __hip_atomic_load(A.error, __ATOMIC_RELAXED, __HIP_MEMORY_SCOPE_AGENT) != 0) break;
                            __builtin_amdgcn_s_sleep(8);
                        }
                        qc = __uint_as_float((unsigned)g);
                    }
                    PPROF(1, true);
                    if (p > 0) {
                        {
                            float trow[kPanel];
#pragma unroll
                            for (int k = 0; k < kPanel; ++k) trow[k] = lTo[k * kPanel + lane];
                            if constexpr (sizeof(U) < 4 || MODEL::kLaneParallel) {
                                const float4* __restrict__ av4 = reinterpret_cast<const float4*>(la + ((p - 1) & 1) * kPanel);
                                float4 av[kPanel / 4];
#pragma unroll
                                for (int i = 0; i < kPanel / 4; ++i) av[i] = av4[i];
#pragma unroll
                                for (int k = 0; k < kPanel; ++k) {
                                    const float4 t = av[k >> 2];
                                    const float ak = (k & 3) == 0 ? t.x : (k & 3) == 1 ? t.y : (k & 3) == 2 ? t.z : t.w;
                                    qc = __builtin_fmaf(trow[k], ak, qc);
                                }
                            } else {
#pragma unroll
                                for (int k = 0; k < kPanel; ++k) qc = __builtin_fmaf(trow[k], rl(a_prev, k), qc);
                            }
                        }
                    }

                    {
                        if (lane == 0) *reinterpret_cast<volatile int*>(&s_tdone) = p + 1;
                    }
                    PPROF(2, true);
                    if constexpr (is_wide_mixture<MODEL>::value) {
                        constexpr int KMAX = MODEL::kMax;
                        const int K = in.K;
                        const int kc = min(lane, K - 1);
                        const bool comp = lane < K;
                        float dvec = 0.0f, avec = 0.0f;
                        const int64_t jlast = s0 + b - 1;
                        auto cptr = [&](const float* __restrict__ arr, int jj) {
                            return arr + min(s0 + r0 + jj, jlast) * K + kc;
                        };
                        static_assert(kChainPrefetch == 16 && kPanel == 64, "window indexing");
                        float rmm[kChainPrefetch], rsv[kChainPrefetch], rul[kChainPrefetch];
                        float rvec = in.beta - qc;
                        const float* __restrict__ DtW = lT + (p & 1) * kPanel * kPanel + lane;
#pragma unroll
                        for (int k = 0; k < kChainPrefetch; ++k) {
                            rmm[k] = *cptr(A.mu_mult, k);
                            rsv[k] = *cptr(A.shvt, k);
                            rul[k] = *cptr(A.u_logs, k);
                        }
#pragma unroll 1
                        for (int g = 0; g < kPanel / kChainPrefetch; ++g) {
#pragma unroll
                        for (int k = 0; k < kChainPrefetch; ++k) {
                            const int jj = kChainPrefetch * g + k;
                            const float drow_jj = DtW[jj * kPanel];
                            const float cmm = rmm[k], csv = rsv[k], cul = rul[k];
                            {
                                rmm[k] = *cptr(A.mu_mult, jj + kChainPrefetch);
                                rsv[k] = *cptr(A.shvt, jj + kChainPrefetch);
                                rul[k] = *cptr(A.u_logs, jj + kChainPrefetch);
                            }
                            const float lnp = rl(in.lnp, jj), eta_old = rl(in.eta_old, jj);
                            const float r = rl(rvec, jj);
                            const float mu = cmm * r;
                            const float t = csv * mu;
                            float u = __builtin_fmaf(t, t, cul);
                            u = (lane == K) ? lnp : u;
                            float mx = dpp_max_shr<1>(u);
                            mx = dpp_max_shr<2>(mx);
                            mx = dpp_max_shr<4>(mx);
                            mx = dpp_max_shr<8>(mx);
                            const float m_lo = rl(mx, 15), m_hi = rl(mx, K);
                            mx = (K >= 16) ? fmaxf(m_lo, m_hi) : m_hi;
                            float e = expf_glibc_nonpos<kLookupPerLane>(u - mx, tab);
                            e = (lane <= K) ? e : 0.0f;
                            static_assert((KMAX + 1) % 8 == 0, "chunks of 8 terms");
                            float ssum = 0.0f;
#pragma unroll
                            for (int c = 0; c < (KMAX + 1) / 8; ++c) {
                                int et[8];
#pragma unroll
                                for (int i = 0; i < 8; ++i) et[i] = __builtin_amdgcn_readlane(__float_as_int(e), 8 * c + i);
                                pin_sgprs(et);
#pragma unroll
                                for (int i = 0; i < 8; ++i) ssum = (c == 0 && i == 0) ? __int_as_float(et[0]) : ssum + __int_as_float(et[i]);
                            }
                            const float gam = comp ? e / ssum : 0.0f;
                            float d = -eta_old;
#pragma unroll
                            for (int c = 0; c < (KMAX + 1) / 8; ++c) {
                                int gt[8];
                                float mb[8];
#pragma unroll
                                for (int i = 0; i < 8; ++i) {
                                    gt[i] = __builtin_amdgcn_readlane(__float_as_int(gam), 8 * c + i);
                                    mb[i] = rl(mu, 8 * c + i);
                                }
                                pin_sgprs(gt);
#pragma unroll
                                for (int i = 0; i < 8; ++i) d = __builtin_fmaf(__int_as_float(gt[i]), mb[i], d);
                            }
                            const bool livej = jj < nrows;
                            const float a = livej ? dq * d : 0.0f;
                            if (comp && livej && member == 0) {
                                const int64_t o = (s0 + r0 + jj) * K + lane;
                                A.var_mu[o] = mu;
                                A.var_gamma[o] = gam;
                            }
                            int l = lane;
                            asm volatile("" : "+v"(l));
                            const bool me = (l == jj);
                            dvec = me ? d : dvec;
                            avec = me ? a : avec;
                            if (MIR) q_own = me ? qc : q_own;
                            qc = __builtin_fmaf(drow_jj, a, qc);
                            rvec = in.beta - qc;
                            if (!MIR) qc = (me && livej) ? qc - d : qc;
                        }
                        }
                        if (member == 0 && live) {
                            A.eta_diff[j] = dvec;
                            if (TEAM) stage_store(A.eta_out + j, in.eta_old + dvec); else A.eta[j] = in.eta_old + dvec;
                        }
                        a_prev = avec;
                        if (SUMS) led[(p & 1) * kPanel + lane] = live ? dvec : 0.0f;
                    } else if constexpr (MODEL::kLaneParallel) {
                        const int K = in.K;
                        float* __restrict__ Lmm = lmx;
                        float* __restrict__ Lsv = lmx + kPanel * kPanelMaxK;
                        float* __restrict__ Lul = lmx + 2 * kPanel * kPanelMaxK;
                        float* __restrict__ Lmu = lmx + 3 * kPanel * kPanelMaxK;
                        float* __restrict__ Lga = lmx + 4 * kPanel * kPanelMaxK;
#pragma unroll
                        for (int k = 0; k < kPanelMaxK; ++k) {
                            if (k < K) {
                                Lmm[lane * K + k] = in.mm[k];
                                Lsv[lane * K + k] = in.sv[k];
                                Lul[lane * K + k] = in.ulog[k];
                            }
                        }
                        __builtin_amdgcn_wave_barrier();
                        const int kc = min(lane, K - 1);
                        float cmm = Lmm[kc], csv = Lsv[kc], cul = Lul[kc];
                        float dvec = 0.0f, avec = 0.0f;
                        auto run_panel = [&](auto rounds_c, auto k4_c) {
                        constexpr int ROUNDS = decltype(rounds_c)::value;
                        constexpr bool K4 = decltype(k4_c)::value;
                        float rvec = in.beta - qc;
                        static_assert(kChainPrefetch == 16 && kPanel == 64, "group indexing");
                        const float* __restrict__ Dt = lT + (p & 1) * kPanel * kPanel + lane;
#pragma unroll 1
                        for (int g = 0; g < kPanel / kChainPrefetch; ++g) {
#pragma unroll
                        for (int k = 0; k < kChainPrefetch; ++k) {
                            const int jj = kChainPrefetch * g + k;
                            const float drow_jj = Dt[jj * kPanel];
                            const int jn = (jj + 1 < kPanel) ? jj + 1 : jj;
                            const float nmm = Lmm[jn * K + kc], nsv = Lsv[jn * K + kc], nul = Lul[jn * K + kc];
                            const float lnp = rl(in.lnp, jj), eta_old = rl(in.eta_old, jj);
                            const float r = rl(rvec, jj);
                            const float mu = cmm * r;
                            const float t = csv * mu;
                            float u = __builtin_fmaf(t, t, cul);
                            u = (lane == K) ? lnp : u;
                            float mub[ROUNDS];
#pragma unroll
                            for (int i = 0; i < ROUNDS; ++i) mub[i] = rl(mu, i);
                            float mx;
                            if constexpr (K4) {
                                int ut[5];
#pragma unroll
                                for (int i = 0; i < 5; ++i) ut[i] = __builtin_amdgcn_readlane(__float_as_int(u), i);
                                pin_sgprs(ut);
                                mx = __int_as_float(ut[0]);
#pragma unroll
                                for (int i = 1; i <= 4; ++i) mx = fmaxf(mx, __int_as_float(ut[i]));
                            } else {
                                mx = dpp_max_shr<1>(u);
                                mx = dpp_max_shr<2>(mx);
                                mx = dpp_max_shr<4>(mx);
                                mx = dpp_max_shr<8>(mx);
                                mx = rl(mx, K);
                            }
                            const float e = softmax_exp<MODEL::kExact, kLookupPerLane>(u - mx, tab);
                            const float e_t = (K4 || lane <= K) ? e : 0.0f;
                            int et[ROUNDS + 1];
#pragma unroll
                            for (int i = 0; i <= ROUNDS; ++i) et[i] = __builtin_amdgcn_readlane(__float_as_int(e_t), i);
                            pin_sgprs(et);
                            float ssum = __int_as_float(et[0]);
#pragma unroll
                            for (int i = 1; i <= ROUNDS; ++i) ssum += __int_as_float(et[i]);
                            const float gam = softmax_div<MODEL::kExact>(e, ssum);
                            const float gam_t = (K4 || lane < K) ? gam : 0.0f;
                            int gt[ROUNDS];
#pragma unroll
                            for (int i = 0; i < ROUNDS; ++i) gt[i] = __builtin_amdgcn_readlane(__float_as_int(gam_t), i);
                            pin_sgprs(gt);
                            float d = -eta_old;
#pragma unroll
                            for (int i = 0; i < ROUNDS; ++i) d = __builtin_fmaf(__int_as_float(gt[i]), mub[i], d);
                            const bool livej = jj < nrows;
                            const float a = livej ? dq * d : 0.0f;
                            if (lane < K) {
                                Lmu[jj * K + lane] = mu;
                                Lga[jj * K + lane] = gam;
                            }
                            int l = lane;
                            asm volatile("" : "+v"(l));
                            const bool me = (l == jj);
                            dvec = me ? d : dvec;
                            avec = me ? a : avec;
                            if (MIR) q_own = me ? qc : q_own;
                            qc = __builtin_fmaf(drow_jj, a, qc);
                            rvec = in.beta - qc;
                            if (!MIR) qc = (me && livej) ? qc - d : qc;
                            cmm = nmm; csv = nsv; cul = nul;
                        }
                        }
                        };
                        if (K == 4) run_panel(std::integral_constant<int, 4>{}, std::true_type{});
                        else if (K < 4) run_panel(std::integral_constant<int, 4>{}, std::false_type{});
                        else run_panel(std::integral_constant<int, kPanelMaxK>{}, std::false_type{});
                        __builtin_amdgcn_wave_barrier();
                        if (member == 0) {
                            const int64_t o = (s0 + r0) * K;
                            for (int i = lane; i < nrows * K; i += 64) {
                                A.var_mu[o + i] = Lmu[i];
                                A.var_gamma[o + i] = Lga[i];
                            }
                            if (live) {
                                A.eta_diff[j] = dvec;
                                if (TEAM) stage_store(A.eta_out + j, in.eta_old + dvec); else A.eta[j] = in.eta_old + dvec;
                            }
                        }
                        a_prev = avec;
                        if (SUMS) led[(p & 1) * kPanel + lane] = live ? dvec : 0.0f;
                    } else {
                        float qcap_v = 0.0f;
                        const float* __restrict__ Dt = lT + (p & 1) * kPanel * kPanel + lane;
                        unsigned long long lane_bit = 1ull;
                        float qf = qc;
    #pragma unroll
                        for (int jj = 0; jj < kPanel; ++jj) {
                            const float dr = Dt[jj * kPanel];
                            const float d = MODEL::template delta<kLookupLane>(in, qf, tab, jj);
                            const float dz = (MODEL::kHasSkip && fabsf(d) < Eps<float>::value) ? 0.0f : d;
                            const float az = dq * dz;
                            const float sa = rl(az, jj);
                            const float sdz = rl(dz, jj);
                            qcap_v = sel_mask(qcap_v, qc, lane_bit);
                            qf = __builtin_fmaf(dr, sa, qc);
                            qc = !MIR ? sel_mask(qf, qf - sdz, lane_bit) : qf;
                            asm volatile("s_lshl_b64 %0, %0, 1" : "+s"(lane_bit) : : "scc");
                        }
                        q_own = qcap_v;

                        PPROF(3, true);
                        bool skipped_lane;
                        float d_lane = 0.0f;
                        a_prev = MODEL::template finish<TEAM>(A, j, in, qcap_v, tab, live, member == 0, skipped_lane, &d_lane);
                        my_skipped += __popcll(__ballot(skipped_lane));
                        if (SUMS) led[(p & 1) * kPanel + lane] = d_lane;
                    }
                    la[(p & 1) * kPanel + lane] = a_prev;
                    if (own(r0)) lq[loc(r0 + lane)] = MIR ? q_own : qc;
                    PPROF(4, true);
                }
            }
            __syncthreads();
        }
        } else {
        for (int p = 0; p < np + 1; ++p) {
            {
                const int uw = wave - 1;
                auto stage_tiles = [&]() {
                if (p + 1 < np) {
                    float* __restrict__ T = lT + ((p + 1) & 1) * kPanel * kPanel;
                    const int trow = lane >> 4, tcol = (lane & 15) * 4;
                    const int row_base = (p + 1) * kPanel;
                    constexpr int kGroups = (kPanel / 4 + NW - 2) / (NW - 1);
                    float4 v[kGroups];
#pragma unroll
                    for (int g = 0; g < kGroups; ++g) {
                        const int row = 4 * min(uw + g * (NW - 1), kPanel / 4 - 1) + trow;
                        v[g] = load4<U>(base + (int64_t)min(row_base + row, b - 1) * stride + (p + 1) * kPanel + tcol);
                    }
                    float4 w[kGroups];
                    {
#pragma unroll
                        for (int g = 0; g < kGroups; ++g) {
                            const int row = 4 * min(uw + g * (NW - 1), kPanel / 4 - 1) + trow;
                            w[g] = load4<U>(base + (int64_t)min(p * kPanel + row, b - 1) * stride + (p + 1) * kPanel + tcol);
                        }
                    }
                    if (MIR && p > 0) {
                        while (*reinterpret_cast<volatile int*>(&s_ddone) < p) __builtin_amdgcn_s_sleep(1);
                    }
#pragma unroll
                    for (int g = 0; g < kGroups; ++g) {
                        const int i = uw + g * (NW - 1);
                        if (i < kPanel / 4) *reinterpret_cast<float4*>(T + (4 * i + trow) * kPanel + tcol) = v[g];
                    }
                    {
                        while (*reinterpret_cast<volatile int*>(&s_tdone) < p + 1) __builtin_amdgcn_s_sleep(1);
#pragma unroll
                        for (int g = 0; g < kGroups; ++g) {
                            const int i = uw + g * (NW - 1);
                            if (i < kPanel / 4) *reinterpret_cast<float4*>(lTo + (4 * i + trow) * kPanel + tcol) = w[g];
                        }
                    }
                }
                };
                const int pp = p - 1;
                const int rr0 = pp * kPanel;
                const int last_row = min(kPanel, b - rr0) - 1;
                const float avec = p > 0 ? la[(pp & 1) * kPanel + lane] : 0.0f;
                const int nstrips = (bpad + kSW - 1) / kSW;
                const bool any_a = __ballot(avec != 0.0f) != 0;
                const float edvec = (MIR && p > 0) ? led[(pp & 1) * kPanel + lane] : 0.0f;
                const bool any_ed = MIR && __ballot(edvec != 0.0f) != 0;
                const int s_pri = ((p + 1) * kPanel) / kSW;
                const int n_mine = (nstrips - member + TS - 1) / TS;
                auto do_strip = [&](int k) {
                    int st = member + k * TS, kl = k;
                    if (TEAM) {
                        const int k_pri = (s_pri % TS == member) ? (s_pri - member) / TS : 0;
                        kl = (k + k_pri) % n_mine;
                        st = member + kl * TS;
                    }
                    const int c = st * kSW + CPL * lane;
                    float* __restrict__ lq_c = lq + (TEAM ? kl * kSW + CPL * lane : c);
                    const int cp = c >> 6;
#if defined(PANEL_TIMING_NO_SECOND_PASS) && PANEL_TIMING_NO_SECOND_PASS + 0 >= 2
                    const bool active = (c < b) && cp > p;
#else
                    const bool active = (c < b) && cp != pp && cp != p;
#endif
                    auto hand_off = [&]() {
                        if (TEAM && st == s_pri && p + 1 < np && p + 1 >= 2) {
                            __builtin_amdgcn_wave_barrier();
                            const float v = lq[loc((p + 1) * kPanel + lane)];
                            const unsigned long long g =
                                ((unsigned long long)(A.tag_base + (unsigned)(p + 2)) << 32) | (unsigned long long)__float_as_uint(v);
                            __hip_atomic_store(gran + (int64_t)(p + 1) * kPanel + lane, g, __ATOMIC_RELAXED,
                                               __HIP_MEMORY_SCOPE_AGENT);
                        }
                    };
                    if constexpr (MIR) {
                        const bool left = cp < pp;
                        float* __restrict__ tgt = left ? ls + (TEAM ? kl * kSW + CPL * lane : c) : lq_c;
                        const bool any_l = __ballot(active && left) != 0, any_r = __ballot(active && !left) != 0;
                        if (any_l && any_r) {
                            const float fvec = left ? 1.0f : dq;
                            if (any_ed && active) {
                                if (last_row == kPanel - 1)
                                    strip_update<U, CPL, true, kDepth, true>(base + (int64_t)rr0 * stride + c, stride, last_row, edvec, tgt, fvec);
                                else
                                    strip_update<U, CPL, false, kDepth, true>(base + (int64_t)rr0 * stride + c, stride, last_row, edvec, tgt, fvec);
                            }
                        } else {
                            float mvec = any_l ? edvec : avec;
                            asm volatile("" : "+v"(mvec));
                            if ((any_l ? any_ed : any_a) && active) {
                                if (last_row == kPanel - 1)
                                    strip_update<U, CPL, true, kDepth>(base + (int64_t)rr0 * stride + c, stride, last_row, mvec, tgt);
                                else
                                    strip_update<U, CPL, false, kDepth>(base + (int64_t)rr0 * stride + c, stride, last_row, mvec, tgt);
                            }
                        }
                        if (k == uw) PPROF(6, wave == 1);
                        hand_off();
                    } else {
                        if (any_a && active) {
                            if (last_row == kPanel - 1)
                                strip_update<U, CPL, true, kDepth>(base + (int64_t)rr0 * stride + c, stride, last_row, avec, lq_c);
                            else
                                strip_update<U, CPL, false, kDepth>(base + (int64_t)rr0 * stride + c, stride, last_row, avec, lq_c);
                        }
                        if (k == uw) PPROF(6, wave == 1);
                        hand_off();
                    }
                };
                if (MIR && p > 0 && uw == NW - 2) {
#ifdef PANEL_TIMING_NO_SECOND_PASS
                    if (false) {
#else
                    if (any_ed && own(rr0)) {
#endif
                        float* __restrict__ sp = ls + loc(rr0 + lane);
                        *sp = diag_lower_update(lT + (pp & 1) * kPanel * kPanel, edvec, *sp, lane);
                    }
                    if (lane == 0) *reinterpret_cast<volatile int*>(&s_ddone) = p;
                }
                stage_tiles();
                PPROF(5, wave == 1);
                if (p > 0) {
                    for (int k = uw; k < n_mine; k += NW - 1) do_strip(k);
                }
            }
            PPROF(7, wave == 1);
            __syncthreads();
        }
        }
#ifdef VIPRS_PANEL_PROFILE
        if (TEAM && item == 0 && member < 2 && tid == 0) {
            for (int p = 0; p < np && p < 64; p += (p < 4 || p > np - 4) ? 1 : 8) {
                const unsigned t = s_pprof[p][0];
                printf("m%d phase %2d @%7u: granule %4d T-apply %4d loop %5d replay %5d end %5d | upd: staged %5d pri %5d all %5d (x10ns)\n",
                       member, p, t - s_pprof[0][0], (int)(s_pprof[p][1] - t), (int)(s_pprof[p][2] - t), (int)(s_pprof[p][3] - t),
                       (int)(s_pprof[p][4] - t), (int)(s_pprof[p][4] - t), (int)(s_pprof[p][5] - t), (int)(s_pprof[p][6] - t),
                       (int)(s_pprof[p][7] - t));
            }
        }
#endif
        {
            for (int li = tid; li < (TEAM ? n_own * kSW : b); li += NW * 64) {
                const int i = glob(li);
                if (i < b) {
                    const float v = SUMS ? lq[li] + A.dq * ls[li] : lq[li];
                    if (TEAM) stage_store(A.q_out + s0 + i, v); else A.q[s0 + i] = v;
                }
            }
        }
        if (TEAM) {
            asm volatile("s_waitcnt vmcnt(0)" ::: "memory");
            __syncthreads();
            if (tid == 0) s_blk = (atomicAdd(A.arrive + item, 1) == TS - 1) ? 1 : 0;
            __syncthreads();
            const bool last = s_blk != 0;
            if (last) {
                for (int i = tid; i < b; i += NW * 64) {
                    A.eta[s0 + i] = __hip_atomic_load(A.eta_out + s0 + i, __ATOMIC_RELAXED, __HIP_MEMORY_SCOPE_AGENT);
                    A.q[s0 + i] = __hip_atomic_load(A.q_out + s0 + i, __ATOMIC_RELAXED, __HIP_MEMORY_SCOPE_AGENT);
                }
                if (tid == 0) atomicExch(A.arrive + item, 0);
            }
        }
        __syncthreads();
#ifdef VIPRS_SWEEP_TRACE
        if (tid == 0) {
            const unsigned k = atomicAdd(&g_sweep_trace_n, 1u);
            if (k < (1u << 15)) {
                g_sweep_trace[k][0] = ((unsigned long long)blockIdx.x << 32) | (unsigned)(TEAM ? 1 : 0);
                g_sweep_trace[k][1] = (unsigned long long)b;
                g_sweep_trace[k][2] = trace_t0;
                g_sweep_trace[k][3] = wall_clock64();
            }
        }
#endif
    }
    if (lane == 0 && my_skipped && member == 0) atomicAdd(A0.skipped, my_skipped);
}

struct SweepArgs {
    EStepArgs<float> cls[3];
    int32_t qcap[3];
    int32_t n_wg[2];
    int32_t narrow0;
    int32_t* done;
    unsigned long long* skipped_last;
};

template <typename U, typename MODEL, int FORM, int NW, int CPL>
__global__ __launch_bounds__(NW * 64, PANEL_MIN_WAVES) void estep_sweep_kernel(SweepArgs S) {
    extern __shared__ __attribute__((aligned(16))) float smem[];
    const int wg = blockIdx.x;
    const int team_cls = wg < S.n_wg[0] ? 0 : (wg < S.n_wg[0] + S.n_wg[1] ? 1 : 2);
    if (team_cls < 2) {
        constexpr bool kNarrowForm = FORM == kFormMirror && sizeof(U) < 4;
        constexpr int CPL_N = (MODEL::kLaneParallel || !kNarrowForm) ? CPL : panel_team_cols<U>();
        const int wg_t = wg - (team_cls ? S.n_wg[0] : 0);
        if (CPL_N != CPL && team_cls == 0 && S.narrow0)
            panel_role<U, MODEL, FORM, NW, true, CPL_N>(S.cls[0], S.qcap[0], smem, wg_t);
        else
            panel_role<U, MODEL, FORM, NW, true, CPL>(S.cls[team_cls], S.qcap[team_cls], smem, wg_t);
        __syncthreads();
    }
    if (S.cls[2].n_blocks > 0) panel_role<U, MODEL, FORM, NW, false, CPL>(S.cls[2], S.qcap[2], smem, wg);
    __syncthreads();
    if (threadIdx.x == 0) {
        if (atomicAdd(S.done, 1) == (int)gridDim.x - 1) {
            S.cls[2].counter[0] = 0; S.cls[2].counter[1] = 0; S.cls[2].counter[2] = 0;
            atomicExch(S.skipped_last, atomicExch(S.cls[2].skipped, 0ull));
            atomicExch(S.done, 0);
        }
    }
}

}
```

### viprs_amd/csrc/internal.h

```cpp
#pragma once
#include <hip/hip_runtime.h>

#include <algorithm>
#include <array>
#include <cstdlib>
#include <cstring>
#include <functional>
#include <map>
#include <memory>
#include <mutex>
#include <string>
#include <vector>

#include "../../include/viprs_hip.h"
#include "dev_buf.h"
#include "kernels_common.h"
#include "planner.h"
#include "sweep_route.h"

namespace viprs {

int fail(int code, const std::string& msg);

#define HIP_TRY(expr)                                                                        \
    do {                                                                                     \
        hipError_t _e = (expr);                                                              \
        if (_e != hipSuccess)                                                                \
            return ::viprs::fail(VIPRS_EDEVICE, std::string(#expr) + ": " + hipGetErrorString(_e)); \
    } while (0)

inline size_t ld_elem_size(int ld_dtype) {
    switch (ld_dtype) {
        case VIPRS_LD_I8: return 1;
        case VIPRS_LD_I16: return 2;
        case VIPRS_LD_I32: return 4;
        case VIPRS_LD_I64: return 8;
        case VIPRS_LD_F32: return 4;
        case VIPRS_LD_F64: return 8;
        default: return 0;
    }
}
inline size_t float_size(int t) { return t == VIPRS_F32 ? 4 : (t == VIPRS_F64 ? 8 : 0); }

struct SchedConfig {
    int large_block = 2304, medium_block = 1600;
    int class_team[3] = {8, 4, 1};
    int class_team_mix[3] = {8, 4, 1};
    bool team_env = false;
    int bottom_mod = 0;
};
SchedConfig& sched_config();
constexpr int kClassWaves[3] = {4, 4, 4};
constexpr int kPlanCounters = 32;

struct DevEvent {
    hipEvent_t e = nullptr;
    ~DevEvent() { if (e) (void)hipEventDestroy(e); }
};

struct EventBracket {
    DevEvent ev[2];
    bool timed = false;
    int start(hipStream_t s) {
        for (auto& e : ev)
            if (!e.e) HIP_TRY(hipEventCreate(&e.e));
        HIP_TRY(hipEventRecord(ev[0].e, s));
        return VIPRS_OK;
    }
    int stop(hipStream_t s) {
        HIP_TRY(hipEventRecord(ev[1].e, s));
        timed = true;
        return VIPRS_OK;
    }
    int elapsed(int device, double* ms, const char* nothing) {
        if (!timed) return fail(VIPRS_EINVAL, nothing);
        HIP_TRY(hipSetDevice(device));
        HIP_TRY(hipEventSynchronize(ev[1].e));
        float t = 0.f;
        HIP_TRY(hipEventElapsedTime(&t, ev[0].e, ev[1].e));
        *ms = (double)t;
        return VIPRS_OK;
    }
};

double host_clock_ms();

struct SweepTiming {
    static constexpr int kRing = 256;
    struct Slot {
        DevEvent ev[4];
        bool whole = false;
        bool dense = false;
        double t0 = 0.0, t1 = 0.0;
    };
    Slot ring[kRing];
    hipStream_t stream = nullptr;
    int64_t sweeps = 0;
    bool armed = false;

    Slot& slot(int64_t sweep) { return ring[sweep % kRing]; }
    int create(hipStream_t s) {
        stream = s;
        for (Slot& sl : ring)
            for (DevEvent& e : sl.ev) HIP_TRY(hipEventCreate(&e.e));
        return VIPRS_OK;
    }
    int open(bool whole_sweep_events, bool dense_bracketed) {
        Slot& s = slot(sweeps);
        s.whole = whole_sweep_events;
        s.dense = dense_bracketed;
        s.t0 = s.t1 = 0.0;
        armed = false;
        if (s.whole) HIP_TRY(hipEventRecord(s.ev[0].e, stream));
        return VIPRS_OK;
    }
    void arm() { armed = true; }
    int start() {
        armed = false;
        slot(sweeps).t0 = host_clock_ms();
        HIP_TRY(hipEventRecord(slot(sweeps).ev[2].e, stream));
        return VIPRS_OK;
    }
    int launcher_start() { return armed ? start() : VIPRS_OK; }
    int stop() {
        HIP_TRY(hipEventRecord(slot(sweeps).ev[3].e, stream));
        slot(sweeps).t1 = host_clock_ms();
        return VIPRS_OK;
    }
    int dense_done() { return slot(sweeps).whole && slot(sweeps).dense ? stop() : VIPRS_OK; }
    int close() {
        if (slot(sweeps).whole) HIP_TRY(hipEventRecord(slot(sweeps).ev[1].e, stream));
        else { const int rc = stop(); if (rc != VIPRS_OK) return rc; }
        sweeps++;
        return VIPRS_OK;
    }
    void abandon() { armed = false; }
    void reset() { sweeps = 0; armed = false; }
    int elapsed(int64_t sweep, int which, double* ms) {
        Slot& s = slot(sweep);
        *ms = 0.0;
        if (which == 2) { *ms = std::max(0.0, s.t1 - s.t0); return VIPRS_OK; }
        const bool bracket = which == 1 || !s.whole;
        if (bracket && !s.dense) return VIPRS_OK;
        float t = 0.f;
        HIP_TRY(hipEventSynchronize(s.ev[bracket ? 3 : 1].e));
        HIP_TRY(hipEventElapsedTime(&t, s.ev[bracket ? 2 : 0].e, s.ev[bracket ? 3 : 1].e));
        *ms = t;
        return VIPRS_OK;
    }
};

struct RidgeBlock;

struct RidgeWork {
    bool built = false;
    DevBuf<char> d_rec;
    DevBuf<int32_t> d_live;
    size_t vec_bytes = 0;
    DevBuf<char> d_vec[9];
    DevBuf<char> d_shift;
    EventBracket time;
    int iterations = 0;
};

struct SpectrumWork {
    bool built = false;
    DevBuf<double> d_beta;
    DevBuf<int32_t> d_status, d_iters;
    DevBuf<int32_t> d_live;
    size_t vec_bytes = 0;
    DevBuf<char> d_vec[3];
    size_t coef_cap = 0;
    DevBuf<double> d_alpha, d_betas;
    EventBracket time;
    int iterations = 0;
    double host_ms = 0.0;
};

}

struct viprs_state;
struct viprs_comm;
struct viprs_plan {
    int64_t m = 0;
    int64_t nnz = 0;
    int low_memory = 0;
    int mirror = 0;
    int ld_dtype = 0;
    int device = 0;
    int n_cu = 0;
    int math_mode = VIPRS_MATH_EXACT;
    int math_used = 0;
    hipStream_t stream = nullptr;
    hipStream_t side_stream = nullptr;
    hipEvent_t ev_fork = nullptr, ev_join = nullptr;
    std::vector<viprs::Block> blocks;
    std::vector<viprs::BlockDesc> dense_h, ragged_h;
    int class_begin[4] = {0, 0, 0, 0};
    int team0 = 0;
    viprs::DevBuf<viprs::BlockDesc> d_dense, d_ragged;
    std::vector<viprs::BlockDesc> dense_all_h, ragged_all_h;
    int class_begin_all[4] = {0, 0, 0, 0};
    viprs::DevBuf<viprs::BlockDesc> d_dense_all;
    bool filtered = false;
    uint64_t dense_gen = 0;
    viprs::DevBuf<unsigned long long> d_granules;
    int64_t n_granule_rows = 0;
    viprs::DevBuf<int32_t> d_error;
    int grid_mfma = -1;
    viprs::DevBuf<int32_t> d_lb;
    viprs::DevBuf<int64_t> d_ip;
    viprs::DevBuf<int32_t> d_rowlen;
    viprs::DevBuf<int64_t> d_rowlist_dense, d_rowlist_ragged;
    viprs::DevBuf<int64_t> d_rowstart_dense;
    viprs::DevBuf<char> d_ld_raw;
    viprs::DevBuf<char> d_ld_dense;
    int64_t dense_elems = 0;
    int max_dense = 0, max_ragged = 0;
    int max_band_panels = 0;
    viprs::DevBuf<int32_t> d_counters;
    viprs::DevBuf<unsigned long long> d_skipped;
    bool skip_count_in_place = false;
    viprs::DevBuf<int32_t> d_arrive;
    uint32_t granule_gen = 0;
    struct TeamSplit { int64_t key[6] = {-1, -1, -1, -1, -1, -1}; int best[2] = {0, 0}; } team_split;
    bool grid_teams_built = false;
    int grid_team_blocks = 0, grid_team_wgs = 0;
    std::vector<int> grid_team_ts;
    viprs::DevBuf<int32_t> d_grid_team_block, d_grid_team_member, d_grid_team_size;
    viprs::DevBuf<int64_t> d_grid_team_goff;
    viprs::DevBuf<unsigned long long> d_grid_gran;
    uint32_t grid_gen = 0;
    viprs::SweepTiming timing;
    viprs_state* scratch = nullptr;
    bool dot_built = false;
    viprs::DevBuf<viprs::BlockDesc> d_dot_blocks;
    viprs::DevBuf<int64_t> d_dot_rows_dense[3], d_dot_rows_ragged;
    viprs::DevBuf<int32_t> d_dot_first;
    viprs::DevBuf<char> d_dot_b, d_dot_y;
    viprs::EventBracket time_dot;
    bool unmirrored_wanted = false;
    viprs::DevBuf<char> d_score_a, d_score_y;
    viprs::DevBuf<double> d_score_corr;
    viprs::EventBracket time_score;
    std::vector<int32_t> clump_block_of;
    viprs::DevBuf<int32_t> d_clump_order;
    viprs::DevBuf<int64_t> d_clump_off;
    viprs::DevBuf<double> d_clump_thr;
    viprs::DevBuf<uint32_t> d_clump_mask;
    viprs::DevBuf<int32_t> d_clump_index;
    viprs::EventBracket time_clump;
    viprs::DevBuf<viprs::RidgeBlock> d_solver_blocks;
    viprs::RidgeWork ridge;
    viprs::SpectrumWork spectrum;

    ~viprs_plan();
};

struct viprs_state {
    viprs_plan* plan = nullptr;
    int device = 0;
    int float_dtype = VIPRS_F32;
    int model_kind = VIPRS_MODEL_SPIKE_SLAB;
    int width = 1;
    viprs::DevBuf<char> f[VIPRS_FIELD_COUNT];
    viprs::DevBuf<int32_t> d_active;
    viprs::DevBuf<char> eta_out, q_out;
    viprs::DevBuf<double> d_n, d_var_tau, d_partials, d_sums;
    viprs::DevBuf<double> d_weight;
    viprs::DevBuf<double> d_log_var_tau0;
    std::vector<double> col_prep;
    int n_groups = 0;
    std::vector<int64_t> group_start;
    std::vector<double> pair_prep;
    std::vector<uint8_t> group_cols_h;
    viprs::DevBuf<uint8_t> d_group_cols;
    viprs::DevBuf<int32_t> d_blk_group;
    uint64_t blk_group_gen = ~0ull;
    viprs::DevBuf<int32_t> d_group_lists;
    viprs::DevBuf<char> d_prep_rows;
    viprs::DevBuf<char> d_sum_rows;
    char* h_rows = nullptr;
    size_t rows_cap = 0;
    hipEvent_t ev_prep = nullptr;
    size_t h_sums_cap = 0;
    double* h_sums = nullptr;
    size_t sums_total = 0;
    bool sums_pending = false, sums_empty = false;
    viprs_comm* comm = nullptr;
    ~viprs_state() {
        if (h_sums) (void)hipHostFree(h_sums);
        if (h_rows) (void)hipHostFree(h_rows);
        if (ev_prep) (void)hipEventDestroy(ev_prep);
    }
    size_t field_elems(int field) const {
        const size_t m = (size_t)plan->m;
        switch (field) {
            case VIPRS_FIELD_STD_BETA: return m;
            case VIPRS_FIELD_LOG_NULL_PI: return model_kind == VIPRS_MODEL_MIXTURE ? m : 0;
            case VIPRS_FIELD_ETA: case VIPRS_FIELD_Q: case VIPRS_FIELD_ETA_DIFF:
                return model_kind == VIPRS_MODEL_GRID ? m * width : m;
            default: return m * width;
        }
    }
};

namespace viprs {

int plan_create_generated(viprs_plan** out, int64_t m, const int32_t* lb, const std::vector<int64_t>& ip64, int ld_dtype,
                          int low_memory, int device, const std::function<int(void*)>& fill);

int ensure_upper_storage(viprs_plan* P, bool mirrored);
int team_launch_gate(viprs_plan* P);
int team_launch_done(viprs_plan* P);

int check_device_error(viprs_plan* P);

int prepare_ld_rows(viprs_plan* P);
int ensure_solver_blocks(viprs_plan* P);
int enqueue_dot(viprs_plan* P, int float_dtype, int n_cols, const void* dB, void* dY, double dq_scale, int include_diagonal);

int comm_reduce_on_stream(viprs_comm* C, double* d_vec, int n, int group, hipStream_t stream);


template <typename T, typename U> int launch_generic(viprs_plan* P, EStepArgs<T> A, int model, bool dense);
template <typename U> int launch_tile_f64(viprs_plan* P, EStepArgs<double> A, int model, bool dense);
template <typename U> int launch_panel(viprs_plan* P, EStepArgs<float> A, int model);
template <typename U> int launch_band(viprs_plan* P, EStepArgs<float> A, int model);
int band_ring_panels(const viprs_plan* P);
#ifdef PANEL_NW
constexpr int kPanelWaves = PANEL_NW;
#else
constexpr int kPanelWaves = kClassWaves[0];
#endif
using BandKernelFn = void (*)(EStepArgs<float>, int);
template <typename U> int launch_panel_kernel(viprs_plan* P, EStepArgs<float> A, int model, const void* kfn, int nw, int math_bit);
template <typename U> int launch_band_kernel(viprs_plan* P, EStepArgs<float> A, BandKernelFn kfn, int math_bit);
template <typename U> int launch_panel_enet(viprs_plan* P, EStepArgs<float> A);
template <typename U> int launch_band_enet(viprs_plan* P, EStepArgs<float> A);
template <typename U> int launch_grid_mfma(viprs_plan* P, EStepArgs<float> A);
template <typename U> int launch_ld_dot(viprs_plan* P, int float_dtype, int n_cols, const void* dB, void* dY, double dq_scale,
                                        int include_diagonal);
template <typename U> int launch_ld_score(viprs_plan* P, int float_dtype, int n_cols, const void* dA, const double* dCorr,
                                          void* dY, double dq_scale);
template <typename U> int launch_ld_clump(viprs_plan* P, int n_cols);

}
```

### viprs_amd/csrc/kernels_common.h

```cpp
#pragma once
#include <hip/hip_runtime.h>
#include <stdint.h>

#if (defined(PANEL_TIMING_NO_HANDOFF_WAIT) || \
    defined(PANEL_TIMING_NO_SECOND_PASS) || \
    defined(PANEL_NW) || \
    defined(PANEL_STRIP_DEPTH) || \
    defined(PANEL_MIN_WAVES) || \
    defined(PANEL_TEAM_STRIP_DEPTH) || \
    defined(PANEL_TEAM_CPL_F32) || \
    defined(PANEL_CHAIN_PRIO) || \
    defined(VIPRS_GRID_MFMA_CHAIN) || \
    defined(VIPRS_GRID_PROFILE) || \
    defined(VIPRS_TILE_PROFILE) || \
    defined(VIPRS_SWEEP_TRACE) || \
    defined(VIPRS_PANEL_PROFILE)) && \
    !defined(VIPRS_EXPERIMENTAL)
#error "experiment switch defined without -DVIPRS_EXPERIMENTAL (see kernels_common.h)"
#endif
#ifdef VIPRS_EXPERIMENTAL
#define VIPRS_BF_VIPRS_EXPERIMENTAL " VIPRS_EXPERIMENTAL"
#else
#define VIPRS_BF_VIPRS_EXPERIMENTAL ""
#endif
#ifdef PANEL_TIMING_NO_HANDOFF_WAIT
#define VIPRS_BF_PANEL_TIMING_NO_HANDOFF_WAIT " PANEL_TIMING_NO_HANDOFF_WAIT"
#else
#define VIPRS_BF_PANEL_TIMING_NO_HANDOFF_WAIT ""
#endif
#ifdef PANEL_TIMING_NO_SECOND_PASS
#define VIPRS_BF_PANEL_TIMING_NO_SECOND_PASS " PANEL_TIMING_NO_SECOND_PASS"
#else
#define VIPRS_BF_PANEL_TIMING_NO_SECOND_PASS ""
#endif
#ifdef PANEL_NW
#define VIPRS_BF_PANEL_NW " PANEL_NW"
#else
#define VIPRS_BF_PANEL_NW ""
#endif
#ifdef PANEL_STRIP_DEPTH
#define VIPRS_BF_PANEL_STRIP_DEPTH " PANEL_STRIP_DEPTH"
#else
#define VIPRS_BF_PANEL_STRIP_DEPTH ""
#endif
#ifdef PANEL_MIN_WAVES
#define VIPRS_BF_PANEL_MIN_WAVES " PANEL_MIN_WAVES"
#else
#define VIPRS_BF_PANEL_MIN_WAVES ""
#endif
#ifdef PANEL_TEAM_STRIP_DEPTH
#define VIPRS_BF_PANEL_TEAM_STRIP_DEPTH " PANEL_TEAM_STRIP_DEPTH"
#else
#define VIPRS_BF_PANEL_TEAM_STRIP_DEPTH ""
#endif
#ifdef PANEL_TEAM_CPL_F32
#define VIPRS_BF_PANEL_TEAM_CPL_F32 " PANEL_TEAM_CPL_F32"
#else
#define VIPRS_BF_PANEL_TEAM_CPL_F32 ""
#endif
#ifdef PANEL_CHAIN_PRIO
#define VIPRS_BF_PANEL_CHAIN_PRIO " PANEL_CHAIN_PRIO"
#else
#define VIPRS_BF_PANEL_CHAIN_PRIO ""
#endif
#ifdef VIPRS_GRID_MFMA_CHAIN
#define VIPRS_BF_VIPRS_GRID_MFMA_CHAIN " VIPRS_GRID_MFMA_CHAIN"
#else
#define VIPRS_BF_VIPRS_GRID_MFMA_CHAIN ""
#endif
#ifdef VIPRS_GRID_PROFILE
#define VIPRS_BF_VIPRS_GRID_PROFILE " VIPRS_GRID_PROFILE"
#else
#define VIPRS_BF_VIPRS_GRID_PROFILE ""
#endif
#ifdef VIPRS_TILE_PROFILE
#define VIPRS_BF_VIPRS_TILE_PROFILE " VIPRS_TILE_PROFILE"
#else
#define VIPRS_BF_VIPRS_TILE_PROFILE ""
#endif
#ifdef VIPRS_SWEEP_TRACE
#define VIPRS_BF_VIPRS_SWEEP_TRACE " VIPRS_SWEEP_TRACE"
#else
#define VIPRS_BF_VIPRS_SWEEP_TRACE ""
#endif
#ifdef VIPRS_PANEL_PROFILE
#define VIPRS_BF_VIPRS_PANEL_PROFILE " VIPRS_PANEL_PROFILE"
#else
#define VIPRS_BF_VIPRS_PANEL_PROFILE ""
#endif
#define VIPRS_TU_BUILD_FLAGS VIPRS_BF_VIPRS_EXPERIMENTAL VIPRS_BF_PANEL_TIMING_NO_HANDOFF_WAIT VIPRS_BF_PANEL_TIMING_NO_SECOND_PASS VIPRS_BF_PANEL_NW VIPRS_BF_PANEL_STRIP_DEPTH VIPRS_BF_PANEL_MIN_WAVES VIPRS_BF_PANEL_TEAM_STRIP_DEPTH VIPRS_BF_PANEL_TEAM_CPL_F32 VIPRS_BF_PANEL_CHAIN_PRIO VIPRS_BF_VIPRS_GRID_MFMA_CHAIN VIPRS_BF_VIPRS_GRID_PROFILE VIPRS_BF_VIPRS_TILE_PROFILE VIPRS_BF_VIPRS_SWEEP_TRACE VIPRS_BF_VIPRS_PANEL_PROFILE

namespace viprs {
void register_build_flags(const char* flags);
struct BuildFlagsRegistrar { explicit BuildFlagsRegistrar(const char* f) { register_build_flags(f); } };
}

namespace viprs {

constexpr int kPanel = 64;
constexpr int kStrip = 256;

constexpr int kPanelMaxK = 8;
constexpr int kPanelWideMaxK = 31;
constexpr int kMixLdsFloats = 5 * kPanel * kPanelMaxK;
struct PanelLds {
    int qcap;
    bool mix_scratch, mirror;
    __host__ __device__ constexpr PanelLds(int qcap_, bool mix_scratch_, bool mirror_)
        : qcap(qcap_), mix_scratch(mix_scratch_), mirror(mirror_) {}
    __host__ __device__ constexpr int q() const { return 0; }
    __host__ __device__ constexpr int a() const { return qcap; }
    __host__ __device__ constexpr int diag_tiles() const { return a() + 2 * kPanel; }
    __host__ __device__ constexpr int offdiag_tile() const { return diag_tiles() + 2 * kPanel * kPanel; }
    __host__ __device__ constexpr int mix() const { return offdiag_tile() + kPanel * kPanel; }
    __host__ __device__ constexpr int ed() const { return mix() + (mix_scratch ? kMixLdsFloats : 0); }
    __host__ __device__ constexpr int s() const { return ed() + 2 * kPanel; }
    __host__ __device__ constexpr int total_floats() const { return mirror ? s() + qcap : ed(); }
};
constexpr int kMaxMixtureK = 64;
constexpr int kGridModels = 32;
constexpr int kGridResOwners = 6, kGridResSlots = 2;
constexpr int kGridResMaxCols = kGridResOwners * kGridResSlots * 2 * kPanel;
constexpr int kBandMaxRingPanels = 256;

struct BlockDesc {
    int32_t start;
    int32_t size;
    int32_t stride;
    int32_t kind;
    int64_t ld_off;
    int64_t gr_off;
    int32_t band_left;
    int32_t band_right;
};

template <typename T>
struct EStepArgs {
    const BlockDesc* blocks;
    int32_t n_blocks;
    int32_t* counter;
    int32_t bottom_mod;
    unsigned long long* granules;
    uint32_t tag_base;
    int32_t* arrive;
    int32_t* error;
    int32_t n_teams;
    int32_t team_size;
    int64_t granule_rows;
    unsigned long long* skipped;
    const int32_t* lb;
    const int64_t* rowstart;
    const int32_t* rowlen;
    const void* ld_rows;
    const void* ld_dense;
    int64_t ld_zero_off;
    const T* std_beta;
    const T* u_logs;
    const T* shvt;
    const T* mu_mult;
    const T* log_null_pi;
    T* var_gamma;
    T* var_mu;
    T* eta;
    T* q;
    T* eta_diff;
    T* eta_out;
    T* q_out;
    T dq;
    int32_t low_memory;
    int32_t width;
    int64_t m;
    const int32_t* active;
    int32_t n_active;
    const int32_t* blk_group;
    const uint8_t* group_cols;
    const int32_t* group_lists;
};
constexpr int kGroupListStride = 1 + kGridModels;

template <typename T>
__device__ __forceinline__ EStepArgs<T> select_model(const EStepArgs<T>& A0, int model_slot) {
    EStepArgs<T> A = A0;
    if (A0.n_active > 0) {
        const int64_t off = (int64_t)A0.active[model_slot] * A0.m;
        A.var_gamma += off; A.var_mu += off; A.eta += off; A.q += off; A.eta_diff += off;
        A.u_logs += off; A.shvt += off; A.mu_mult += off;
        if (A.eta_out) { A.eta_out += off; A.q_out += off; }
    }
    return A;
}

}
```

### viprs_amd/csrc/launch_panel.inc

```
#include "internal.h"
#include "estep_panel.h"

static viprs::BuildFlagsRegistrar viprs_tu_build_flags_(VIPRS_TU_BUILD_FLAGS);

namespace viprs {

template <typename U>
int launch_panel_kernel(viprs_plan* P, EStepArgs<float> A, int model, const void* kfn, int nw, int math_bit) {
    constexpr int CPL = panel_cols<U>();
    const bool upper = P->low_memory != 0;
    const bool mirror = upper;
    if (upper) { const int rc = ensure_upper_storage(P, true); if (rc != VIPRS_OK) return rc; }
    const int n_models = std::max(1, A.n_active);
    const int* team_of = ((model == kPanelMixture || model == kPanelMixtureWide) && !sched_config().team_env) ? sched_config().class_team_mix
                                                                             : sched_config().class_team;
    P->math_used |= math_bit;

    const int n_team_blocks = P->class_begin[2];
    const int64_t ng = P->n_granule_rows * kPanel * (int64_t)n_models;
    if (P->d_granules.n < (size_t)ng) {
        HIP_TRY(hipStreamSynchronize(P->stream));
        HIP_TRY(P->d_granules.alloc((size_t)ng));
        HIP_TRY(hipMemsetAsync(P->d_granules.p, 0, sizeof(unsigned long long) * (size_t)ng, P->stream));
    }
    const size_t n_arrive = (size_t)n_team_blocks * (size_t)n_models + 1;
    if (P->d_arrive.n < n_arrive) {
        HIP_TRY(hipStreamSynchronize(P->stream));
        HIP_TRY(P->d_arrive.alloc(n_arrive));
        HIP_TRY(hipMemsetAsync(P->d_arrive.p, 0, sizeof(int32_t) * n_arrive, P->stream));
    }
    P->granule_gen = (P->granule_gen + 1) & 0xFFFFFu;
    if (P->granule_gen == 0) {
        if (P->d_granules.n) HIP_TRY(hipMemsetAsync(P->d_granules.p, 0, sizeof(unsigned long long) * P->d_granules.n, P->stream));
        P->granule_gen = 1;
    }
    A.granules = P->d_granules.p;
    A.tag_base = P->granule_gen << 12;

    SweepArgs S{};
    S.done = P->d_arrive.p + (n_arrive - 1);
    S.skipped_last = P->d_skipped.p + 1;
    size_t shmem = 0;
    for (int c = 0; c < 3; ++c) {
        EStepArgs<float>& C = S.cls[c];
        C = A;
        const int begin = P->class_begin[c], end = P->class_begin[c + 1];
        C.blocks = P->d_dense.p + begin;
        C.n_blocks = end - begin;
        if (A.blk_group) C.blk_group = A.blk_group + begin;
        C.counter = c < 2 ? P->d_counters.p + 4 + c : P->d_counters.p + 16;
        C.arrive = P->d_arrive.p + (c == 1 ? (size_t)(P->class_begin[1] - P->class_begin[0]) * (size_t)n_models : 0);
        C.bottom_mod = 0;
        C.team_size = c < 2 ? team_of[c] : 1;
        if (c == 0 && P->team0 > 0 && team_of == sched_config().class_team) C.team_size = P->team0;
        if (c == 0 && team_of == sched_config().class_team_mix) {
            const int64_t room = (int64_t)P->n_cu * 2 * 5 / 8;
            while (C.team_size > 4 && (int64_t)(end - begin) * n_models * C.team_size > room) C.team_size -= 4;
        }
        C.n_teams = 0;
        S.qcap[c] = 0;
        if (end > begin) {
            const int max_b = P->dense_h[begin].size;
            auto lds_bytes = [&](int qcap) {
                return (size_t)PanelLds(qcap, model == kPanelMixture, mirror).total_floats() * sizeof(float);
            };
            for (;;) {
                S.qcap[c] = (max_b + kPanel - 1) / kPanel * kPanel + kStrip;
                if (c < 2) {
                    const bool narrow = upper && sizeof(U) < 4 && c == 0 && C.team_size >= 8 && model != kPanelMixture && model != kPanelMixtureWide;
                    if (c == 0) S.narrow0 = narrow ? 1 : 0;
                    const int kSW = kPanel * (narrow ? panel_team_cols<U>() : CPL);
                    const int n_strips = ((max_b + kPanel - 1) / kPanel * kPanel + kSW - 1) / kSW;
                    S.qcap[c] = (n_strips + C.team_size - 1) / C.team_size * kSW + kStrip;
                }
                if (c < 2 && lds_bytes(S.qcap[c]) > 160 * 1024 && C.team_size < 16) { ++C.team_size; continue; }
                break;
            }
            shmem = std::max(shmem, lds_bytes(S.qcap[c]));
        }
    }
    if (shmem == 0) return P->timing.launcher_start();
    if (shmem > 160 * 1024) return fail(VIPRS_EUNSUPPORTED, "LD block too large for the LDS-resident panel kernel");
    if (shmem > 48 * 1024)
        HIP_TRY(hipFuncSetAttribute(kfn, hipFuncAttributeMaxDynamicSharedMemorySize, (int)shmem));
    int per_cu = 0;
    HIP_TRY(hipOccupancyMaxActiveBlocksPerMultiprocessor(&per_cu, kfn, nw * 64, shmem));
    per_cu = std::max(1, per_cu);
    if (const char* f = getenv("VIPRS_MAX_WG_PER_CU")) per_cu = std::max(1, std::min(per_cu, atoi(f)));
    const int capacity = P->n_cu * per_cu;

    const int64_t n_small = (int64_t)S.cls[2].n_blocks * n_models;
    const int team_budget = n_small > 0 ? capacity * 5 / 8 : capacity;
    int team_wgs = 0;
    {
        const double es = (double)sizeof(U);
        auto class_time = [&](int c, int n_teams) {
            const EStepArgs<float>& C = S.cls[c];
            const int64_t n_items = (int64_t)C.n_blocks * n_models;
            double t = 0.0;
            for (int64_t i = 0; i < n_items; i += n_teams) {
                const double sz = (double)P->dense_h[(size_t)(P->class_begin[c] + i / n_models)].size;
                t += std::max(sz * 135e-9, sz * sz * es / (C.team_size * 16e9));
            }
            return t;
        };
        const int64_t items[2] = {(int64_t)S.cls[0].n_blocks * n_models, (int64_t)S.cls[1].n_blocks * n_models};
        const int TS0 = S.cls[0].team_size, TS1 = S.cls[1].team_size;
        int best[2] = {0, 0};
        const int64_t key[6] = {items[0], items[1], TS0, TS1, team_budget, (int64_t)sizeof(U)};
        if (std::equal(key, key + 6, P->team_split.key)) {
            best[0] = P->team_split.best[0];
            best[1] = P->team_split.best[1];
        } else if (items[0] > 0 && items[1] > 0) {
            double best_t = 1e30;
            const int max0 = (int)std::min<int64_t>(items[0], std::max(1, (team_budget - TS1) / TS0));
            for (int n0 = 1; n0 <= max0; ++n0) {
                const int n1 = (int)std::min<int64_t>(items[1], std::max(1, (team_budget - n0 * TS0) / TS1));
                const double t = std::max(class_time(0, n0), class_time(1, n1));
                if (t < best_t * (1.0 - 1e-9)) { best_t = t; best[0] = n0; best[1] = n1; }
            }
        } else if (items[0] > 0) {
            best[0] = (int)std::min<int64_t>(items[0], std::max(1, team_budget / TS0));
        } else if (items[1] > 0) {
            best[1] = (int)std::min<int64_t>(items[1], std::max(1, team_budget / TS1));
        }
        std::copy(key, key + 6, P->team_split.key);
        P->team_split.best[0] = best[0];
        P->team_split.best[1] = best[1];
        for (int c = 0; c < 2; ++c) {
            EStepArgs<float>& C = S.cls[c];
            C.n_teams = best[c];
            S.n_wg[c] = C.n_teams * C.team_size;
            team_wgs += S.n_wg[c];
        }
    }
    if (team_wgs > capacity) return fail(VIPRS_EUNSUPPORTED, "team size exceeds the resident workgroups of the device");
    int grid = (int)std::min<int64_t>(capacity, (int64_t)team_wgs + n_small);
    grid = std::max(grid, team_wgs);
    if (n_small >= 4 * (int64_t)P->n_cu) S.cls[2].bottom_mod = sched_config().bottom_mod;

    void* params[] = {(void*)&S};
    if (team_wgs > 0) { const int rc = team_launch_gate(P); if (rc != VIPRS_OK) return rc; }
    { const int rc = P->timing.launcher_start(); if (rc != VIPRS_OK) return rc; }
    HIP_TRY(hipLaunchKernel(kfn, dim3(grid), dim3(nw * 64), params, shmem, P->stream));
    if (team_wgs > 0) { const int rc = team_launch_done(P); if (rc != VIPRS_OK) return rc; }
    return VIPRS_OK;
}

template <typename U>
int launch_panel(viprs_plan* P, EStepArgs<float> A, int model) {
    constexpr int NW = kPanelWaves, CPL = panel_cols<U>();
    const bool exact = P->math_mode == VIPRS_MATH_EXACT;
    const bool upper = P->low_memory != 0;
    const void* kfn = nullptr;
#define PK(MODEL) (upper ? (const void*)estep_sweep_kernel<U, MODEL, kFormMirror, NW, CPL>       \
                          : (const void*)estep_sweep_kernel<U, MODEL, kFormSym, NW, CPL>)
    if (model == kPanelGridColumn) kfn = exact ? PK(GridColumnModel<true>) : PK(GridColumnModel<false>);
    else if (model == kPanelMixture) kfn = exact ? PK(MixtureModel<true>) : PK(MixtureModel<false>);
    else if (model == kPanelMixtureWide) kfn = A.width <= 15 ? PK(MixtureWideModel<15>) : PK(MixtureWideModel<31>);
    else kfn = exact ? PK(SpikeSlabModel<true>) : PK(SpikeSlabModel<false>);
#undef PK
    return launch_panel_kernel<U>(P, A, model, kfn, NW, (exact || model == kPanelMixtureWide) ? 1 : 2);
}

template int launch_panel_kernel<PANEL_U>(viprs_plan*, EStepArgs<float>, int, const void*, int, int);
template int launch_panel<PANEL_U>(viprs_plan*, EStepArgs<float>, int);

#if defined(VIPRS_SWEEP_TRACE)
#define PANEL_TRACE_FN2(tag) viprs_debug_sweep_trace_##tag
#define PANEL_TRACE_FN(tag) PANEL_TRACE_FN2(tag)
extern "C" int PANEL_TRACE_FN(PANEL_TAG)(unsigned long long* out, int capacity) {
    unsigned n = 0;
    if (hipDeviceSynchronize() != hipSuccess) return -1;
    if (hipMemcpyFromSymbol(&n, HIP_SYMBOL(g_sweep_trace_n), sizeof(n)) != hipSuccess) return -1;
    n = std::min<unsigned>(n, std::min<unsigned>(1u << 15, (unsigned)capacity));
    if (n && hipMemcpyFromSymbol(out, HIP_SYMBOL(g_sweep_trace), (size_t)n * 32) != hipSuccess) return -1;
    const unsigned zero = 0;
    (void)hipMemcpyToSymbol(HIP_SYMBOL(g_sweep_trace_n), &zero, sizeof(zero));
    return (int)n;
}
#endif

}
```

### viprs_amd/csrc/panel_enet.h

```cpp
#pragma once
#include "panel_models.h"

namespace viprs {

struct ElasticNetModel {
    static constexpr bool kLaneParallel = false;
    static constexpr bool kHasSkip = false;
    struct In { float c, beta, pen, eta_old; };
    static __device__ __forceinline__ In load(const EStepArgs<float>& A, int64_t j, bool live) {
        In in;
        in.c = live ? A.mu_mult[j] : 0.0f;
        in.beta = live ? A.std_beta[j] : 0.0f;
        in.pen = live ? A.shvt[j] : 0.0f;
        in.eta_old = live ? A.eta[j] : 0.0f;
        return in;
    }
    static __device__ __forceinline__ void core(const In& in, float q, float& u, float& b, float& d) {
        const float t = in.c * q;
        u = in.beta - t;
        const float a = fabsf(u) - in.pen;
        b = a > 0.0f ? copysignf(a, u) : 0.0f;
        d = b - in.eta_old;
    }
    template <int LOOKUP>
    static __device__ __forceinline__ float delta(const In& in, float q, const ExpTab&, int) {
        float u, b, d;
        core(in, q, u, b, d);
        return d;
    }
    template <int LOOKUP>
    static __device__ __forceinline__ bool update(const In& in, float q, const ExpTab& tab, float& d, int sel) {
        d = delta<LOOKUP>(in, q, tab, sel);
        return true;
    }
    template <bool TEAM>
    static __device__ __forceinline__ float finish(const EStepArgs<float>& A, int64_t j, const In& in, float q,
                                                   const ExpTab&, bool live, bool writer, bool& skipped,
                                                   float* d_out = nullptr) {
        float u, b, d;
        core(in, q, u, b, d);
        if (d_out) *d_out = live ? d : 0.0f;
        if (live && writer) {
            A.var_mu[j] = u;
            A.var_gamma[j] = b != 0.0f ? 1.0f : 0.0f;
            A.eta_diff[j] = d;
            if (TEAM) stage_store(A.eta_out + j, in.eta_old + d); else A.eta[j] = in.eta_old + d;
        }
        skipped = false;
        return live ? A.dq * d : 0.0f;
    }
};

}
```

### viprs_amd/csrc/panel_loads.h

```cpp
#pragma once
#include "kernels_common.h"

namespace viprs {

template <typename U> __device__ __forceinline__ float4 load4(const U* p);
template <> __device__ __forceinline__ float4 load4<float>(const float* p) {
    return *reinterpret_cast<const float4*>(p);
}
template <> __device__ __forceinline__ float4 load4<int8_t>(const int8_t* p) {
    const int w = *reinterpret_cast<const int*>(p);
    return make_float4((float)(int8_t)(w), (float)(int8_t)(w >> 8), (float)(int8_t)(w >> 16),
                       (float)(int8_t)(w >> 24));
}
template <> __device__ __forceinline__ float4 load4<int16_t>(const int16_t* p) {
    const int2 w = *reinterpret_cast<const int2*>(p);
    return make_float4((float)(int16_t)(w.x), (float)(int16_t)(w.x >> 16), (float)(int16_t)(w.y),
                       (float)(int16_t)(w.y >> 16));
}

template <int N> __device__ __forceinline__ void pin_sgprs(int (&v)[N]) {
    static_assert(N == 4 || N == 5 || N == 8 || N == 9, "chain lengths of the K <= 8 mixture step");
    if constexpr (N == 4) asm volatile("" : "+s"(v[0]), "+s"(v[1]), "+s"(v[2]), "+s"(v[3]));
    if constexpr (N == 5) asm volatile("" : "+s"(v[0]), "+s"(v[1]), "+s"(v[2]), "+s"(v[3]), "+s"(v[4]));
    if constexpr (N == 8) asm volatile("" : "+s"(v[0]), "+s"(v[1]), "+s"(v[2]), "+s"(v[3]), "+s"(v[4]), "+s"(v[5]), "+s"(v[6]), "+s"(v[7]));
    if constexpr (N == 9) asm volatile("" : "+s"(v[0]), "+s"(v[1]), "+s"(v[2]), "+s"(v[3]), "+s"(v[4]), "+s"(v[5]), "+s"(v[6]), "+s"(v[7]),
                                       "+s"(v[8]));
}
template <int N> __device__ __forceinline__ float dpp_max_shr(float x) {
    float r;
    if (N == 1) asm("s_nop 1\n\tv_max_f32_dpp %0, %1, %1 row_shr:1 row_mask:0xf bank_mask:0xf" : "=v"(r) : "v"(x), "0"(x));
    if (N == 2) asm("s_nop 1\n\tv_max_f32_dpp %0, %1, %1 row_shr:2 row_mask:0xf bank_mask:0xf" : "=v"(r) : "v"(x), "0"(x));
    if (N == 4) asm("s_nop 1\n\tv_max_f32_dpp %0, %1, %1 row_shr:4 row_mask:0xf bank_mask:0xf" : "=v"(r) : "v"(x), "0"(x));
    if (N == 8) asm("s_nop 1\n\tv_max_f32_dpp %0, %1, %1 row_shr:8 row_mask:0xf bank_mask:0xf" : "=v"(r) : "v"(x), "0"(x));
    return r;
}

__device__ __forceinline__ float sel_mask(float a, float b, unsigned long long m) {
    float r;
    asm("v_cndmask_b32_e64 %0, %1, %2, %3" : "=v"(r) : "v"(a), "v"(b), "s"(m));
    return r;
}

__device__ __forceinline__ void stage_store(float* p, float v) {
    __hip_atomic_store(p, v, __ATOMIC_RELAXED, __HIP_MEMORY_SCOPE_AGENT);
}

__device__ __forceinline__ float rl(float v, int lane) {
    return __int_as_float(__builtin_amdgcn_readlane(__float_as_int(v), lane));
}

template <typename U, int CPL> struct RawRow {
    static constexpr int kWords = CPL * (int)sizeof(U) / 4;
    static_assert(CPL * sizeof(U) % 4 == 0 && (kWords == 1 || kWords == 2 || kWords == 4), "1, 2 or 4 dwords per lane and row");
    unsigned w[kWords];
    __device__ __forceinline__ float get(int i) const {
        if constexpr (sizeof(U) == 4) return __uint_as_float(w[i]);
        else if constexpr (sizeof(U) == 1) return static_cast<float>(static_cast<int8_t>(w[i >> 2] >> (8 * (i & 3))));
        else return static_cast<float>(static_cast<int16_t>(w[i >> 1] >> (16 * (i & 1))));
    }
};
template <typename U, int CPL> __device__ __forceinline__ RawRow<U, CPL> load_raw(const U* p) {
    RawRow<U, CPL> r;
    if constexpr (RawRow<U, CPL>::kWords == 1) {
        r.w[0] = *reinterpret_cast<const unsigned*>(p);
    } else if constexpr (RawRow<U, CPL>::kWords == 2) {
        const uint2 t = *reinterpret_cast<const uint2*>(p);
        r.w[0] = t.x; r.w[1] = t.y;
    } else {
        const uint4 t = *reinterpret_cast<const uint4*>(p);
        r.w[0] = t.x; r.w[1] = t.y; r.w[2] = t.z; r.w[3] = t.w;
    }
    return r;
}

constexpr int kChainPrefetch = 16;
#ifndef PANEL_STRIP_DEPTH
#define PANEL_STRIP_DEPTH 16
#endif
constexpr int kStripRowsInFlight = PANEL_STRIP_DEPTH;


template <typename U, int CPL, bool FULL, int DEPTH = kStripRowsInFlight, bool MIXED = false>
__device__ __forceinline__ void strip_update(const U* __restrict__ rowp, int stride, int last_row, float avec,
                                             float* __restrict__ lq_c, float fvec = 1.0f) {
    static_assert(kPanel % DEPTH == 0, "panel must be a whole number of prefetch groups");
    float qv[CPL];
#pragma unroll
    for (int i = 0; i < CPL; ++i) qv[i] = lq_c[i];
    RawRow<U, CPL> buf[DEPTH];
#pragma unroll
    for (int k = 0; k < DEPTH; ++k)
        buf[k] = load_raw<U, CPL>(rowp + (int64_t)(FULL ? k : min(k, last_row)) * stride);
#pragma unroll 1
    for (int g = 0; g < kPanel / DEPTH - 1; ++g) {
#pragma unroll
        for (int k = 0; k < DEPTH; ++k) {
            const RawRow<U, CPL> v = buf[k];
            const int rn = DEPTH * (g + 1) + k;
            buf[k] = load_raw<U, CPL>(rowp + (int64_t)(FULL ? rn : min(rn, last_row)) * stride);
            const float a = MIXED ? fvec * rl(avec, DEPTH * g + k) : rl(avec, DEPTH * g + k);
#pragma unroll
            for (int i = 0; i < CPL; ++i) qv[i] = __builtin_fmaf(v.get(i), a, qv[i]);
            __builtin_amdgcn_sched_barrier(0);
        }
    }
#pragma unroll
    for (int k = 0; k < DEPTH; ++k) {
        const RawRow<U, CPL> v = buf[k];
        const float a = MIXED ? fvec * rl(avec, kPanel - DEPTH + k) : rl(avec, kPanel - DEPTH + k);
#pragma unroll
        for (int i = 0; i < CPL; ++i) qv[i] = __builtin_fmaf(v.get(i), a, qv[i]);
    }
#pragma unroll
    for (int i = 0; i < CPL; ++i) lq_c[i] = qv[i];
}

__device__ __forceinline__ float diag_lower_update(const float* __restrict__ tile, float edvec, float sv, int lane) {
#pragma unroll 16
    for (int jr = 0; jr < kPanel; ++jr) {
        const float t = __builtin_fmaf(tile[jr * kPanel + lane], rl(edvec, jr), sv);
        sv = lane < jr ? t : sv;
    }
    return sv;
}

}
```

### viprs_amd/csrc/panel_models.h

```cpp
#pragma once
#include <type_traits>

#include "device_math.h"
#include "kernels_common.h"
#include "panel_loads.h"

namespace viprs {

template <bool EXACT>
struct SpikeSlabModel {
    static constexpr bool kLaneParallel = false;
    struct In { float mm, beta, sv, ulog, eta_old; };
    static __device__ __forceinline__ In load(const EStepArgs<float>& A, int64_t j, bool live) {
        In in;
        in.mm = live ? A.mu_mult[j] : 0.0f;
        in.beta = live ? A.std_beta[j] : 0.0f;
        in.sv = live ? A.shvt[j] : 0.0f;
        in.ulog = live ? A.u_logs[j] : 0.0f;
        in.eta_old = live ? A.eta[j] : 0.0f;
        return in;
    }
    static constexpr bool kHasSkip = true;
    template <int LOOKUP>
    static __device__ __forceinline__ float delta(const In& in, float q, const ExpTab& tab, int sel) {
        float mu, gamma, d;
        snp_update<EXACT, LOOKUP>(in.mm, in.beta, in.sv, in.ulog, in.eta_old, q, tab, mu, gamma, d, sel);
        return d;
    }
    template <int LOOKUP>
    static __device__ __forceinline__ bool update(const In& in, float q, const ExpTab& tab, float& d, int sel) {
        d = delta<LOOKUP>(in, q, tab, sel);
        return !(fabsf(d) < Eps<float>::value);
    }
    template <bool TEAM>
    static __device__ __forceinline__ float finish(const EStepArgs<float>& A, int64_t j, const In& in, float q,
                                                   const ExpTab& tab, bool live, bool writer, bool& skipped,
                                                   float* d_out = nullptr) {
        float mu, gamma, d;
        snp_update<EXACT, kLookupPerLane>(in.mm, in.beta, in.sv, in.ulog, in.eta_old, q, tab, mu, gamma, d);
        const bool skip = fabsf(d) < Eps<float>::value;
        if (live && writer) {
            if (!skip) {
                A.var_mu[j] = mu;
                A.var_gamma[j] = gamma;
                A.eta_diff[j] = d;
                if (!TEAM) A.eta[j] = in.eta_old + d;
            } else {
                A.eta_diff[j] = 0.0f;
            }
            if (TEAM) stage_store(A.eta_out + j, skip ? in.eta_old : in.eta_old + d);
        }
        skipped = live && skip;
        if (d_out) *d_out = (live && !skip) ? d : 0.0f;
        return (live && !skip) ? A.dq * d : 0.0f;
    }
};

template <bool EXACT = true>
struct GridColumnModel {
    static constexpr bool kLaneParallel = false;
    struct In { float mm, beta, hvt, ulog, eta_old; };
    static __device__ __forceinline__ In load(const EStepArgs<float>& A, int64_t j, bool live) {
        In in;
        in.mm = live ? A.mu_mult[j] : 0.0f;
        in.beta = live ? A.std_beta[j] : 0.0f;
        in.hvt = live ? A.shvt[j] : 0.0f;
        in.ulog = live ? A.u_logs[j] : 0.0f;
        in.eta_old = live ? A.eta[j] : 0.0f;
        return in;
    }
    template <int LOOKUP>
    static __device__ __forceinline__ void core(const In& in, float q, const ExpTab& tab, float& mu, float& gamma,
                                                float& d, int sel) {
        mu = in.mm * (in.beta - q);
        const float u = in.ulog + in.hvt * mu * mu;
        gamma = EXACT ? sigmoid_exact<LOOKUP>(u, tab, sel) : sigmoid_fast(u);
        d = gamma * mu - in.eta_old;
    }
    static constexpr bool kHasSkip = false;
    template <int LOOKUP>
    static __device__ __forceinline__ float delta(const In& in, float q, const ExpTab& tab, int sel) {
        float mu, gamma, d;
        core<LOOKUP>(in, q, tab, mu, gamma, d, sel);
        return d;
    }
    template <int LOOKUP>
    static __device__ __forceinline__ bool update(const In& in, float q, const ExpTab& tab, float& d, int sel) {
        d = delta<LOOKUP>(in, q, tab, sel);
        return true;
    }
    template <bool TEAM>
    static __device__ __forceinline__ float finish(const EStepArgs<float>& A, int64_t j, const In& in, float q,
                                                   const ExpTab& tab, bool live, bool writer, bool& skipped,
                                                   float* d_out = nullptr) {
        float mu, gamma, d;
        core<kLookupPerLane>(in, q, tab, mu, gamma, d, 0);
        if (d_out) *d_out = live ? d : 0.0f;
        if (live && writer) {
            A.var_mu[j] = mu;
            A.var_gamma[j] = gamma;
            A.eta_diff[j] = d;
            if (TEAM) stage_store(A.eta_out + j, in.eta_old + d); else A.eta[j] = in.eta_old + d;
        }
        skipped = false;
        return live ? A.dq * d : 0.0f;
    }
};

template <typename MODEL> struct IsGridColumn : std::false_type {};
template <bool EXACT> struct IsGridColumn<GridColumnModel<EXACT>> : std::true_type {};

template <bool EXACT, int LOOKUP>
__device__ __forceinline__ float softmax_exp(float x, const ExpTab& tab, int sel = 0) {
    if constexpr (EXACT) return expf_glibc_nonpos<LOOKUP>(x, tab, sel);
    else return expf_fast_nonpos(x);
}
template <bool EXACT>
__device__ __forceinline__ float softmax_div(float e, float ssum) {
    if constexpr (EXACT) return e / ssum;
    else return e * __builtin_amdgcn_rcpf(ssum);
}

template <bool EXACT = true>
struct MixtureModel {
    static constexpr bool kExact = EXACT;
    static constexpr bool kLaneParallel = true;
    struct In { float mm[kPanelMaxK], sv[kPanelMaxK], ulog[kPanelMaxK]; float lnp, beta, eta_old; int K; };
    static __device__ __forceinline__ In load(const EStepArgs<float>& A, int64_t j, bool live) {
        In in;
        in.K = A.width;
#pragma unroll
        for (int k = 0; k < kPanelMaxK; ++k) {
            const bool on = live && k < in.K;
            const int64_t idx = on ? j * in.K + k : 0;
            in.mm[k] = on ? A.mu_mult[idx] : 0.0f;
            in.sv[k] = on ? A.shvt[idx] : 0.0f;
            in.ulog[k] = on ? A.u_logs[idx] : 0.0f;
        }
        in.lnp = live ? A.log_null_pi[j] : 0.0f;
        in.beta = live ? A.std_beta[j] : 0.0f;
        in.eta_old = live ? A.eta[j] : 0.0f;
        return in;
    }
    template <int LOOKUP>
    static __device__ __forceinline__ void core(const In& in, float q, const ExpTab& tab, float (&mu)[kPanelMaxK],
                                                float (&gam)[kPanelMaxK], float& d, int sel) {
        const float r = in.beta - q;
        float u[kPanelMaxK];
        float mx = in.lnp;
#pragma unroll
        for (int k = 0; k < kPanelMaxK; ++k) {
            mu[k] = in.mm[k] * r;
            const float t = in.sv[k] * mu[k];
            u[k] = __builtin_fmaf(t, t, in.ulog[k]);
            if (k < in.K) mx = fmaxf(mx, u[k]);
        }
        float ssum = 0.0f;
#pragma unroll
        for (int k = 0; k < kPanelMaxK; ++k) {
            if (k < in.K) {
                u[k] = softmax_exp<EXACT, LOOKUP>(u[k] - mx, tab, sel);
                ssum += u[k];
            }
        }
        ssum += softmax_exp<EXACT, LOOKUP>(in.lnp - mx, tab, sel);
        d = -in.eta_old;
#pragma unroll
        for (int k = 0; k < kPanelMaxK; ++k) {
            if (k < in.K) {
                gam[k] = softmax_div<EXACT>(u[k], ssum);
                d = __builtin_fmaf(gam[k], mu[k], d);
            }
        }
    }
    template <int LOOKUP>
    static __device__ __forceinline__ bool update(const In& in, float q, const ExpTab& tab, float& d, int sel) {
        float mu[kPanelMaxK], gam[kPanelMaxK];
        core<LOOKUP>(in, q, tab, mu, gam, d, sel);
        return true;
    }
    template <bool TEAM>
    static __device__ __forceinline__ float finish(const EStepArgs<float>& A, int64_t j, const In& in, float q,
                                                   const ExpTab& tab, bool live, bool writer, bool& skipped) {
        float mu[kPanelMaxK], gam[kPanelMaxK], d;
        core<kLookupPerLane>(in, q, tab, mu, gam, d, 0);
        if (live && writer) {
#pragma unroll
            for (int k = 0; k < kPanelMaxK; ++k) {
                if (k < in.K) {
                    A.var_mu[j * in.K + k] = mu[k];
                    A.var_gamma[j * in.K + k] = gam[k];
                }
            }
            A.eta_diff[j] = d;
            if (TEAM) stage_store(A.eta_out + j, in.eta_old + d); else A.eta[j] = in.eta_old + d;
        }
        skipped = false;
        return live ? A.dq * d : 0.0f;
    }
};

template <int KMAX>
struct MixtureWideModel {
    static constexpr bool kLaneParallel = true;
    static constexpr bool kWide = true;
    static constexpr int kMax = KMAX;
    struct In { float lnp, beta, eta_old; int K; };
    static __device__ __forceinline__ In load(const EStepArgs<float>& A, int64_t j, bool live) {
        In in;
        in.K = A.width;
        in.lnp = live ? A.log_null_pi[j] : 0.0f;
        in.beta = live ? A.std_beta[j] : 0.0f;
        in.eta_old = live ? A.eta[j] : 0.0f;
        return in;
    }
};
template <typename M, typename = void> struct is_wide_mixture { static constexpr bool value = false; };
template <typename M> struct is_wide_mixture<M, std::enable_if_t<M::kWide>> { static constexpr bool value = true; };

}
```

Measured before the change: 1.567 billion.

## Split team panel work by contiguous panel ranges instead of interleaved strips

```diff
diff --git a/viprs_amd/csrc/abi_estep.hip b/viprs_amd/csrc/abi_estep.hip
--- a/viprs_amd/csrc/abi_estep.hip
+++ b/viprs_amd/csrc/abi_estep.hip
@@ -54,8 +54,6 @@
     A.eta = (T*)S->f[VIPRS_FIELD_ETA].p;
     A.q = (T*)S->f[VIPRS_FIELD_Q].p;
     A.eta_diff = (T*)S->f[VIPRS_FIELD_ETA_DIFF].p;
-    A.eta_out = (T*)S->eta_out.p;
-    A.q_out = (T*)S->q_out.p;
     A.granules = P->d_granules.p;
     A.granule_rows = P->n_granule_rows;
     A.error = P->d_error.p;
diff --git a/viprs_amd/csrc/abi_plan.hip b/viprs_amd/csrc/abi_plan.hip
--- a/viprs_amd/csrc/abi_plan.hip
+++ b/viprs_amd/csrc/abi_plan.hip
@@ -230,7 +230,7 @@
         P->class_begin[2] = i;
         P->class_begin[3] = n;
         if (!sched_config().team_env && P->class_begin[1] > 0) {
-            P->team0 = std::min(16, std::max(8, 4 * (int)(((int64_t)P->dense_h[0].size * (int64_t)es + 5999) / 6000)));
+            P->team0 = std::min(16, std::max(es == 1 ? 4 : 8, 4 * (int)(((int64_t)P->dense_h[0].size * (int64_t)es + 4499) / 4500)));
             const int64_t room = (int64_t)P->n_cu * 2 * 5 / 8;
             while (P->team0 > 4 && (int64_t)P->class_begin[1] * P->team0 > room) P->team0 -= 4;
         }
diff --git a/viprs_amd/csrc/abi_state.hip b/viprs_amd/csrc/abi_state.hip
--- a/viprs_amd/csrc/abi_state.hip
+++ b/viprs_amd/csrc/abi_state.hip
@@ -306,10 +306,6 @@
     S->float_dtype = float_dtype;
     S->model_kind = model_kind;
     S->width = width;
-    if (plan->n_granule_rows > 0) {
-        HIP_TRY(S->eta_out.alloc(S->field_elems(VIPRS_FIELD_ETA) * float_size(float_dtype)));
-        HIP_TRY(S->q_out.alloc(S->field_elems(VIPRS_FIELD_ETA) * float_size(float_dtype)));
-    }
     for (int k = 0; k < VIPRS_FIELD_COUNT; ++k) {
         const size_t bytes = S->field_elems(k) * float_size(float_dtype);
         HIP_TRY(S->f[k].alloc(bytes));
diff --git a/viprs_amd/csrc/estep_band.h b/viprs_amd/csrc/estep_band.h
--- a/viprs_amd/csrc/estep_band.h
+++ b/viprs_amd/csrc/estep_band.h
@@ -185,7 +185,7 @@
                         if (SYM) qc = (me && upd) ? qc - d : qc;
                     }
                     bool skipped_lane;
-                    a_prev = MODEL::template finish<false>(A, j, in, qcap_v, tab, live, true, skipped_lane);
+                    a_prev = MODEL::finish(A, j, in, qcap_v, tab, live, true, skipped_lane);
                     my_skipped += __popcll(__ballot(skipped_lane));
                     la[(p & 1) * kPanel + lane] = a_prev;
                     *slot = qc;
diff --git a/viprs_amd/csrc/estep_panel.h b/viprs_amd/csrc/estep_panel.h
--- a/viprs_amd/csrc/estep_panel.h
+++ b/viprs_amd/csrc/estep_panel.h
@@ -111,22 +111,27 @@
         const U* __restrict__ base = ldd + bd.ld_off;
         const int np = (b + kPanel - 1) / kPanel;
         const int bpad = np * kPanel;
-        const int nstrips_all = (bpad + kSW - 1) / kSW;
-        const int n_own = TEAM ? (nstrips_all - member + TS - 1) / TS : nstrips_all;
-        auto own = [&](int c) { return !TEAM || ((c / kSW) % TS) == member; };
-        auto loc = [&](int c) { return TEAM ? ((c / kSW) / TS) * kSW + (c % kSW) : c; };
-        auto glob = [&](int li) { return TEAM ? ((li / kSW) * TS + member) * kSW + (li % kSW) : li; };
+        const int team_r = TEAM ? (np + TS - 1) / TS : np;
+        const int p_lo = TEAM ? min(member * team_r, np) : 0;
+        const int p_hi = TEAM ? min(p_lo + team_r, np) : np;
+        if (TEAM && p_lo == p_hi) continue;
+        const int c_lo = p_lo * kPanel, c_hi = p_hi * kPanel;
+        const int n_own = (c_hi - c_lo + kSW - 1) / kSW;
+        auto own_panel = [&](int p) { return !TEAM || (p >= p_lo && p < p_hi); };
+        auto loc = [&](int c) { return c - c_lo; };
 
         for (int li = tid; li < (TEAM ? n_own * kSW : bpad) + kStrip; li += NW * 64) {
-            const int c = glob(li);
-            const bool in = (!TEAM || li < n_own * kSW) && c < b;
+            const int c = c_lo + li;
+            const bool in = (!TEAM || c < c_hi) && c < b;
             lq[li] = in ? A.q[s0 + c] : 0.0f;
             if (SUMS) ls[li] = 0.0f;
         }
         if (tid == 0) { s_tdone = 0; s_ddone = 0; }
-        for (int i = tid; i < kPanel * kPanel / 4; i += NW * 64) {
-            const int row = i >> 4, tcol = (i & 15) * 4;
-            *reinterpret_cast<float4*>(lT + row * kPanel + tcol) = load4<U>(base + (int64_t)min(row, b - 1) * stride + tcol);
+        if (own_panel(0)) {
+            for (int i = tid; i < kPanel * kPanel / 4; i += NW * 64) {
+                const int row = i >> 4, tcol = (i & 15) * 4;
+                *reinterpret_cast<float4*>(lT + row * kPanel + tcol) = load4<U>(base + (int64_t)min(row, b - 1) * stride + tcol);
+            }
         }
         __syncthreads();
 
@@ -134,7 +139,7 @@
 
         typename MODEL::In nxt_in{};
         if (wave == 0) {
-            const bool live0 = lane < b;
+            const bool live0 = lane < b && own_panel(0);
             nxt_in = MODEL::load(A, s0 + (live0 ? lane : 0), live0);
         }
 
@@ -148,7 +153,7 @@
         for (int p = 0; p < np + 1; ++p) {
             PPROF(0, true);
             {
-                if (p < np) {
+                if (p < np && own_panel(p)) {
                     const int r0 = p * kPanel;
                     const int nrows = min(kPanel, b - r0);
                     const int64_t j = s0 + r0 + lane;
@@ -156,33 +161,14 @@
                     const typename MODEL::In in = nxt_in;
                     {
                         const int rn = r0 + kPanel + lane;
-                        const bool ln = rn < b;
+                        const bool ln = rn < b && (!TEAM || p + 1 < p_hi);
                         nxt_in = MODEL::load(A, s0 + (ln ? rn : 0), ln);
                     }
 
                     float qc;
                     float q_own = 0.0f;
-                    if (own(r0)) qc = lq[loc(r0 + lane)];
-                    else qc = (r0 + lane < b) ? A.q[s0 + r0 + lane] : 0.0f;
-                    if (TEAM && p >= 2 && (((p * kPanel) / kSW) % TS) != member) {
-                        unsigned long long g = 0;
-#ifdef PANEL_TIMING_NO_HANDOFF_WAIT
-                        if (false)
-#endif
-                        for (unsigned spins = 0;; ++spins) {
-                            g = __hip_atomic_load(gran + (int64_t)p * kPanel + lane, __ATOMIC_RELAXED,
-                                                  __HIP_MEMORY_SCOPE_AGENT);
-                            if (__all((unsigned)(g >> 32) == A.tag_base + (unsigned)(p + 1))) break;
-                            if (spins > (1u << 22)) {
-                                if (lane == 0) atomicExch(A.error, 1);
-                                break;
-                            }
-                            if ((spins & 1023u) == 1023u &&
-                                __hip_atomic_load(A.error, __ATOMIC_RELAXED, __HIP_MEMORY_SCOPE_AGENT) != 0) break;
-                            __builtin_amdgcn_s_sleep(8);
-                        }
-                        qc = __uint_as_float((unsigned)g);
-                    }
+                    qc = lq[loc(r0 + lane)];
+                    float pub = 0.0f;
                     PPROF(1, true);
                     if (p > 0) {
                         {
@@ -285,7 +271,7 @@
                             }
                             const bool livej = jj < nrows;
                             const float a = livej ? dq * d : 0.0f;
-                            if (comp && livej && member == 0) {
+                            if (comp && livej) {
                                 const int64_t o = (s0 + r0 + jj) * K + lane;
                                 A.var_mu[o] = mu;
                                 A.var_gamma[o] = gam;
@@ -301,11 +287,12 @@
                             if (!MIR) qc = (me && livej) ? qc - d : qc;
                         }
                         }
-                        if (member == 0 && live) {
+                        if (live) {
                             A.eta_diff[j] = dvec;
-                            if (TEAM) stage_store(A.eta_out + j, in.eta_old + dvec); else A.eta[j] = in.eta_old + dvec;
+                            A.eta[j] = in.eta_old + dvec;
                         }
                         a_prev = avec;
+                        pub = MIR ? (live ? dvec : 0.0f) : avec;
                         if (SUMS) led[(p & 1) * kPanel + lane] = live ? dvec : 0.0f;
                     } else if constexpr (MODEL::kLaneParallel) {
                         const int K = in.K;
@@ -406,7 +393,7 @@
                         else if (K < 4) run_panel(std::integral_constant<int, 4>{}, std::false_type{});
                         else run_panel(std::integral_constant<int, kPanelMaxK>{}, std::false_type{});
                         __builtin_amdgcn_wave_barrier();
-                        if (member == 0) {
+                        {
                             const int64_t o = (s0 + r0) * K;
                             for (int i = lane; i < nrows * K; i += 64) {
                                 A.var_mu[o + i] = Lmu[i];
@@ -414,10 +401,11 @@
                             }
                             if (live) {
                                 A.eta_diff[j] = dvec;
-                                if (TEAM) stage_store(A.eta_out + j, in.eta_old + dvec); else A.eta[j] = in.eta_old + dvec;
+                                A.eta[j] = in.eta_old + dvec;
                             }
                         }
                         a_prev = avec;
+                        pub = MIR ? (live ? dvec : 0.0f) : avec;
                         if (SUMS) led[(p & 1) * kPanel + lane] = live ? dvec : 0.0f;
                     } else {
                         float qcap_v = 0.0f;
@@ -442,13 +430,43 @@
                         PPROF(3, true);
                         bool skipped_lane;
                         float d_lane = 0.0f;
-                        a_prev = MODEL::template finish<TEAM>(A, j, in, qcap_v, tab, live, member == 0, skipped_lane, &d_lane);
+                        a_prev = MODEL::finish(A, j, in, qcap_v, tab, live, true, skipped_lane, &d_lane);
                         my_skipped += __popcll(__ballot(skipped_lane));
+                        pub = MIR ? d_lane : a_prev;
                         if (SUMS) led[(p & 1) * kPanel + lane] = d_lane;
                     }
+                    if (TEAM && TS > 1) {
+                        const unsigned long long g =
+                            ((unsigned long long)(A.tag_base + (unsigned)(p + 1)) << 32) | (unsigned long long)__float_as_uint(pub);
+                        __hip_atomic_store(gran + (int64_t)p * kPanel + lane, g, __ATOMIC_RELAXED, __HIP_MEMORY_SCOPE_AGENT);
+                    }
                     la[(p & 1) * kPanel + lane] = a_prev;
-                    if (own(r0)) lq[loc(r0 + lane)] = MIR ? q_own : qc;
+                    lq[loc(r0 + lane)] = MIR ? q_own : qc;
                     PPROF(4, true);
+                } else if (TEAM && p < np) {
+                    if (p + 1 == p_lo) {
+                        const int rn = (p + 1) * kPanel + lane;
+                        const bool ln = rn < b;
+                        nxt_in = MODEL::load(A, s0 + (ln ? rn : 0), ln);
+                    }
+                    if (lane == 0) *reinterpret_cast<volatile int*>(&s_tdone) = p + 1;
+                    unsigned long long g = 0;
+                    for (unsigned spins = 0;; ++spins) {
+                        g = __hip_atomic_load(gran + (int64_t)p * kPanel + lane, __ATOMIC_RELAXED, __HIP_MEMORY_SCOPE_AGENT);
+                        if (__all((unsigned)(g >> 32) == A.tag_base + (unsigned)(p + 1))) break;
+                        if (spins > (1u << 22)) {
+                            if (lane == 0) atomicExch(A.error, 1);
+                            break;
+                        }
+                        if ((spins & 1023u) == 1023u &&
+                            __hip_atomic_load(A.error, __ATOMIC_RELAXED, __HIP_MEMORY_SCOPE_AGENT) != 0) break;
+                        __builtin_amdgcn_s_sleep(8);
+                    }
+                    PPROF(1, true);
+                    const float v = __uint_as_float((unsigned)g);
+                    a_prev = MIR ? dq * v : v;
+                    if (SUMS) led[(p & 1) * kPanel + lane] = v;
+                    la[(p & 1) * kPanel + lane] = a_prev;
                 }
             }
             __syncthreads();
@@ -458,7 +476,7 @@
             {
                 const int uw = wave - 1;
                 auto stage_tiles = [&]() {
-                if (p + 1 < np) {
+                if (p + 1 < np && own_panel(p + 1)) {
                     float* __restrict__ T = lT + ((p + 1) & 1) * kPanel * kPanel;
                     const int trow = lane >> 4, tcol = (lane & 15) * 4;
                     const int row_base = (p + 1) * kPanel;
@@ -499,40 +517,22 @@
                 const int rr0 = pp * kPanel;
                 const int last_row = min(kPanel, b - rr0) - 1;
                 const float avec = p > 0 ? la[(pp & 1) * kPanel + lane] : 0.0f;
-                const int nstrips = (bpad + kSW - 1) / kSW;
                 const bool any_a = __ballot(avec != 0.0f) != 0;
                 const float edvec = (MIR && p > 0) ? led[(pp & 1) * kPanel + lane] : 0.0f;
                 const bool any_ed = MIR && __ballot(edvec != 0.0f) != 0;
-                const int s_pri = ((p + 1) * kPanel) / kSW;
-                const int n_mine = (nstrips - member + TS - 1) / TS;
                 auto do_strip = [&](int k) {
-                    int st = member + k * TS, kl = k;
-                    if (TEAM) {
-                        const int k_pri = (s_pri % TS == member) ? (s_pri - member) / TS : 0;
-                        kl = (k + k_pri) % n_mine;
-                        st = member + kl * TS;
-                    }
-                    const int c = st * kSW + CPL * lane;
-                    float* __restrict__ lq_c = lq + (TEAM ? kl * kSW + CPL * lane : c);
+                    const int li = k * kSW + CPL * lane;
+                    const int c = c_lo + li;
+                    float* __restrict__ lq_c = lq + li;
                     const int cp = c >> 6;
 #if defined(PANEL_TIMING_NO_SECOND_PASS) && PANEL_TIMING_NO_SECOND_PASS + 0 >= 2
-                    const bool active = (c < b) && cp > p;
+                    const bool active = (c < b) && (!TEAM || c < c_hi) && cp > p;
 #else
-                    const bool active = (c < b) && cp != pp && cp != p;
-#endif
-                    auto hand_off = [&]() {
-                        if (TEAM && st == s_pri && p + 1 < np && p + 1 >= 2) {
-                            __builtin_amdgcn_wave_barrier();
-                            const float v = lq[loc((p + 1) * kPanel + lane)];
-                            const unsigned long long g =
-                                ((unsigned long long)(A.tag_base + (unsigned)(p + 2)) << 32) | (unsigned long long)__float_as_uint(v);
-                            __hip_atomic_store(gran + (int64_t)(p + 1) * kPanel + lane, g, __ATOMIC_RELAXED,
-                                               __HIP_MEMORY_SCOPE_AGENT);
-                        }
-                    };
+                    const bool active = (c < b) && (!TEAM || c < c_hi) && cp != pp && cp != p;
+#endif
                     if constexpr (MIR) {
                         const bool left = cp < pp;
-                        float* __restrict__ tgt = left ? ls + (TEAM ? kl * kSW + CPL * lane : c) : lq_c;
+                        float* __restrict__ tgt = left ? ls + li : lq_c;
                         const bool any_l = __ballot(active && left) != 0, any_r = __ballot(active && !left) != 0;
                         if (any_l && any_r) {
                             const float fvec = left ? 1.0f : dq;
@@ -553,7 +553,6 @@
                             }
                         }
                         if (k == uw) PPROF(6, wave == 1);
-                        hand_off();
                     } else {
                         if (any_a && active) {
                             if (last_row == kPanel - 1)
@@ -562,14 +561,13 @@
                                 strip_update<U, CPL, false, kDepth>(base + (int64_t)rr0 * stride + c, stride, last_row, avec, lq_c);
                         }
                         if (k == uw) PPROF(6, wave == 1);
-                        hand_off();
                     }
                 };
                 if (MIR && p > 0 && uw == NW - 2) {
 #ifdef PANEL_TIMING_NO_SECOND_PASS
                     if (false) {
 #else
-                    if (any_ed && own(rr0)) {
+                    if (any_ed && own_panel(pp)) {
 #endif
                         float* __restrict__ sp = ls + loc(rr0 + lane);
                         *sp = diag_lower_update(lT + (pp & 1) * kPanel * kPanel, edvec, *sp, lane);
@@ -579,7 +577,7 @@
                 stage_tiles();
                 PPROF(5, wave == 1);
                 if (p > 0) {
-                    for (int k = uw; k < n_mine; k += NW - 1) do_strip(k);
+                    for (int k = uw; k < n_own; k += NW - 1) do_strip(k);
                 }
             }
             PPROF(7, wave == 1);
@@ -598,26 +596,12 @@
         }
 #endif
         {
-            for (int li = tid; li < (TEAM ? n_own * kSW : b); li += NW * 64) {
-                const int i = glob(li);
+            for (int li = tid; li < (TEAM ? c_hi - c_lo : b); li += NW * 64) {
+                const int i = c_lo + li;
                 if (i < b) {
                     const float v = SUMS ? lq[li] + A.dq * ls[li] : lq[li];
-                    if (TEAM) stage_store(A.q_out + s0 + i, v); else A.q[s0 + i] = v;
+                    A.q[s0 + i] = v;
                 }
-            }
-        }
-        if (TEAM) {
-            asm volatile("s_waitcnt vmcnt(0)" ::: "memory");
-            __syncthreads();
-            if (tid == 0) s_blk = (atomicAdd(A.arrive + item, 1) == TS - 1) ? 1 : 0;
-            __syncthreads();
-            const bool last = s_blk != 0;
-            if (last) {
-                for (int i = tid; i < b; i += NW * 64) {
-                    A.eta[s0 + i] = __hip_atomic_load(A.eta_out + s0 + i, __ATOMIC_RELAXED, __HIP_MEMORY_SCOPE_AGENT);
-                    A.q[s0 + i] = __hip_atomic_load(A.q_out + s0 + i, __ATOMIC_RELAXED, __HIP_MEMORY_SCOPE_AGENT);
-                }
-                if (tid == 0) atomicExch(A.arrive + item, 0);
             }
         }
         __syncthreads();
@@ -633,7 +617,7 @@
         }
 #endif
     }
-    if (lane == 0 && my_skipped && member == 0) atomicAdd(A0.skipped, my_skipped);
+    if (lane == 0 && my_skipped) atomicAdd(A0.skipped, my_skipped);
 }
 
 struct SweepArgs {
diff --git a/viprs_amd/csrc/internal.h b/viprs_amd/csrc/internal.h
--- a/viprs_amd/csrc/internal.h
+++ b/viprs_amd/csrc/internal.h
@@ -265,7 +265,6 @@
     int width = 1;
     viprs::DevBuf<char> f[VIPRS_FIELD_COUNT];
     viprs::DevBuf<int32_t> d_active;
-    viprs::DevBuf<char> eta_out, q_out;
     viprs::DevBuf<double> d_n, d_var_tau, d_partials, d_sums;
     viprs::DevBuf<double> d_weight;
     viprs::DevBuf<double> d_log_var_tau0;
diff --git a/viprs_amd/csrc/kernels_common.h b/viprs_amd/csrc/kernels_common.h
--- a/viprs_amd/csrc/kernels_common.h
+++ b/viprs_amd/csrc/kernels_common.h
@@ -142,7 +142,6 @@
     int32_t bottom_mod;
     unsigned long long* granules;
     uint32_t tag_base;
-    int32_t* arrive;
     int32_t* error;
     int32_t n_teams;
     int32_t team_size;
@@ -164,8 +163,6 @@
     T* eta;
     T* q;
     T* eta_diff;
-    T* eta_out;
-    T* q_out;
     T dq;
     int32_t low_memory;
     int32_t width;
@@ -185,7 +182,6 @@
         const int64_t off = (int64_t)A0.active[model_slot] * A0.m;
         A.var_gamma += off; A.var_mu += off; A.eta += off; A.q += off; A.eta_diff += off;
         A.u_logs += off; A.shvt += off; A.mu_mult += off;
-        if (A.eta_out) { A.eta_out += off; A.q_out += off; }
     }
     return A;
 }
diff --git a/viprs_amd/csrc/launch_panel.inc b/viprs_amd/csrc/launch_panel.inc
--- a/viprs_amd/csrc/launch_panel.inc
+++ b/viprs_amd/csrc/launch_panel.inc
@@ -4,6 +4,11 @@
 static viprs::BuildFlagsRegistrar viprs_tu_build_flags_(VIPRS_TU_BUILD_FLAGS);
 
 namespace viprs {
+
+static inline int team_member_cols(int n_panels, int team_size, int strip_cols) {
+    const int r = (n_panels + team_size - 1) / team_size;
+    return (r * kPanel + strip_cols - 1) / strip_cols * strip_cols;
+}
 
 template <typename U>
 int launch_panel_kernel(viprs_plan* P, EStepArgs<float> A, int model, const void* kfn, int nw, int math_bit) {
@@ -16,14 +21,13 @@
                                                                              : sched_config().class_team;
     P->math_used |= math_bit;
 
-    const int n_team_blocks = P->class_begin[2];
     const int64_t ng = P->n_granule_rows * kPanel * (int64_t)n_models;
     if (P->d_granules.n < (size_t)ng) {
         HIP_TRY(hipStreamSynchronize(P->stream));
         HIP_TRY(P->d_granules.alloc((size_t)ng));
         HIP_TRY(hipMemsetAsync(P->d_granules.p, 0, sizeof(unsigned long long) * (size_t)ng, P->stream));
     }
-    const size_t n_arrive = (size_t)n_team_blocks * (size_t)n_models + 1;
+    const size_t n_arrive = 1;
     if (P->d_arrive.n < n_arrive) {
         HIP_TRY(hipStreamSynchronize(P->stream));
         HIP_TRY(P->d_arrive.alloc(n_arrive));
@@ -49,7 +53,6 @@
         C.n_blocks = end - begin;
         if (A.blk_group) C.blk_group = A.blk_group + begin;
         C.counter = c < 2 ? P->d_counters.p + 4 + c : P->d_counters.p + 16;
-        C.arrive = P->d_arrive.p + (c == 1 ? (size_t)(P->class_begin[1] - P->class_begin[0]) * (size_t)n_models : 0);
         C.bottom_mod = 0;
         C.team_size = c < 2 ? team_of[c] : 1;
         if (c == 0 && P->team0 > 0 && team_of == sched_config().class_team) C.team_size = P->team0;
@@ -70,8 +73,7 @@
                     const bool narrow = upper && sizeof(U) < 4 && c == 0 && C.team_size >= 8 && model != kPanelMixture && model != kPanelMixtureWide;
                     if (c == 0) S.narrow0 = narrow ? 1 : 0;
                     const int kSW = kPanel * (narrow ? panel_team_cols<U>() : CPL);
-                    const int n_strips = ((max_b + kPanel - 1) / kPanel * kPanel + kSW - 1) / kSW;
-                    S.qcap[c] = (n_strips + C.team_size - 1) / C.team_size * kSW + kStrip;
+                    S.qcap[c] = team_member_cols((max_b + kPanel - 1) / kPanel, C.team_size, kSW) + kStrip;
                 }
                 if (c < 2 && lds_bytes(S.qcap[c]) > 160 * 1024 && C.team_size < 16) { ++C.team_size; continue; }
                 break;
@@ -90,7 +92,8 @@
     const int capacity = P->n_cu * per_cu;
 
     const int64_t n_small = (int64_t)S.cls[2].n_blocks * n_models;
-    const int team_budget = n_small > 0 ? capacity * 5 / 8 : capacity;
+    int team_budget = n_small > 0 ? capacity * 5 / 8 : capacity;
+    if (const char* f = getenv("VIPRS_TEAM_BUDGET")) { if (*f) team_budget = std::max(1, std::min(team_budget, atoi(f))); }
     int team_wgs = 0;
     {
         const double es = (double)sizeof(U);
diff --git a/viprs_amd/csrc/panel_enet.h b/viprs_amd/csrc/panel_enet.h
--- a/viprs_amd/csrc/panel_enet.h
+++ b/viprs_amd/csrc/panel_enet.h
@@ -33,7 +33,6 @@
         d = delta<LOOKUP>(in, q, tab, sel);
         return true;
     }
-    template <bool TEAM>
     static __device__ __forceinline__ float finish(const EStepArgs<float>& A, int64_t j, const In& in, float q,
                                                    const ExpTab&, bool live, bool writer, bool& skipped,
                                                    float* d_out = nullptr) {
@@ -44,7 +43,7 @@
             A.var_mu[j] = u;
             A.var_gamma[j] = b != 0.0f ? 1.0f : 0.0f;
             A.eta_diff[j] = d;
-            if (TEAM) stage_store(A.eta_out + j, in.eta_old + d); else A.eta[j] = in.eta_old + d;
+            A.eta[j] = in.eta_old + d;
         }
         skipped = false;
         return live ? A.dq * d : 0.0f;
diff --git a/viprs_amd/csrc/panel_loads.h b/viprs_amd/csrc/panel_loads.h
--- a/viprs_amd/csrc/panel_loads.h
+++ b/viprs_amd/csrc/panel_loads.h
@@ -39,10 +39,6 @@
     float r;
     asm("v_cndmask_b32_e64 %0, %1, %2, %3" : "=v"(r) : "v"(a), "v"(b), "s"(m));
     return r;
-}
-
-__device__ __forceinline__ void stage_store(float* p, float v) {
-    __hip_atomic_store(p, v, __ATOMIC_RELAXED, __HIP_MEMORY_SCOPE_AGENT);
 }
 
 __device__ __forceinline__ float rl(float v, int lane) {
diff --git a/viprs_amd/csrc/panel_models.h b/viprs_amd/csrc/panel_models.h
--- a/viprs_amd/csrc/panel_models.h
+++ b/viprs_amd/csrc/panel_models.h
@@ -32,7 +32,6 @@
         d = delta<LOOKUP>(in, q, tab, sel);
         return !(fabsf(d) < Eps<float>::value);
     }
-    template <bool TEAM>
     static __device__ __forceinline__ float finish(const EStepArgs<float>& A, int64_t j, const In& in, float q,
                                                    const ExpTab& tab, bool live, bool writer, bool& skipped,
                                                    float* d_out = nullptr) {
@@ -44,11 +43,10 @@
                 A.var_mu[j] = mu;
                 A.var_gamma[j] = gamma;
                 A.eta_diff[j] = d;
-                if (!TEAM) A.eta[j] = in.eta_old + d;
+                A.eta[j] = in.eta_old + d;
             } else {
                 A.eta_diff[j] = 0.0f;
             }
-            if (TEAM) stage_store(A.eta_out + j, skip ? in.eta_old : in.eta_old + d);
         }
         skipped = live && skip;
         if (d_out) *d_out = (live && !skip) ? d : 0.0f;
@@ -89,7 +87,6 @@
         d = delta<LOOKUP>(in, q, tab, sel);
         return true;
     }
-    template <bool TEAM>
     static __device__ __forceinline__ float finish(const EStepArgs<float>& A, int64_t j, const In& in, float q,
                                                    const ExpTab& tab, bool live, bool writer, bool& skipped,
                                                    float* d_out = nullptr) {
@@ -100,7 +97,7 @@
             A.var_mu[j] = mu;
             A.var_gamma[j] = gamma;
             A.eta_diff[j] = d;
-            if (TEAM) stage_store(A.eta_out + j, in.eta_old + d); else A.eta[j] = in.eta_old + d;
+            A.eta[j] = in.eta_old + d;
         }
         skipped = false;
         return live ? A.dq * d : 0.0f;
@@ -179,7 +176,6 @@
         core<LOOKUP>(in, q, tab, mu, gam, d, sel);
         return true;
     }
-    template <bool TEAM>
     static __device__ __forceinline__ float finish(const EStepArgs<float>& A, int64_t j, const In& in, float q,
                                                    const ExpTab& tab, bool live, bool writer, bool& skipped) {
         float mu[kPanelMaxK], gam[kPanelMaxK], d;
@@ -193,7 +189,7 @@
                 }
             }
             A.eta_diff[j] = d;
-            if (TEAM) stage_store(A.eta_out + j, in.eta_old + d); else A.eta[j] = in.eta_old + d;
+            A.eta[j] = in.eta_old + d;
         }
         skipped = false;
         return live ? A.dq * d : 0.0f;
```

After: 1.588 billion, median of 6. 1.01x the previous value.
